# CederGroupHub/chgnet

Hardware: NVIDIA H100
Metric: structures_per_sec_EFS (higher is better)
Workload: dtype f32

## Files before the change

chgnet_b200/_lib.py:

```python
from __future__ import annotations

import ctypes
import os
from ctypes import c_char_p, c_float, c_int32, c_int64, c_void_p

import torch
from torch import Tensor

_HERE = os.path.dirname(os.path.abspath(__file__))
LIB_PATH = os.path.join(_HERE, "libchgnet_b200.so")

P, I, F, I64 = c_void_p, c_int32, c_float, c_int64

SIGNATURES: dict[str, list] = {
    "chg_embed_atoms": [P, P, I, P, P],
    "chg_edge_geometry": [P, P, P, P, P, P, I, P, P, P, P],
    "chg_bond_basis_embed": [P, P, I, P, P, I, F, F, I, P, P, P, P, P, P],
    "chg_bond_basis_bwd": [P, P, I, P, P, I, F, F, I, P, P, P, P, P, P, P],
    "chg_angle_basis_embed": [P, P, P, I, P, I, P, P, P, P],
    "chg_angle_basis_bwd": [P, P, P, I, P, I, P, P, P, P, P],
    "chg_linear": [P, P, I, I, P, P, P, P, I, P, P],
    "chg_gather_rows": [P, P, I, I, P, P],
    "chg_scatter_rows": [P, P, I, I, P, P],
    "chg_atom_conv_fwd": [P, P, P, P, P, P, I, P, P, P, P, P, P, P],
    "chg_atom_conv_bwd": [P, P, P, P, P, P, I, P, P, P, P, P, P, P, P, P],
    "chg_segment_sum": [P, I, P, P, I, I, I, P, I, P],
    "chg_atom_conv_fused": [P, P, P, P, P, P, P, I, I, P, P, P, P, P, P, P],
    "chg_bond_conv_fused": [P, P, P, P, P, P, P, P, I, I, P, P, P, P, P, P, P, P],
    "chg_bond_conv_fwd": [P, P, P, P, P, P, P, I, P, P, P, P, P, P, P],
    "chg_bond_conv_bwd": [P, P, P, P, P, I, P, P, P, P, P, P, P, P, P],
    "chg_angle_update_fwd": [P, P, P, P, P, P, P, I, P, P, P, P],
    "chg_angle_update_bwd": [P, P, I, P, P, P, P],
    "chg_readout": [P, P, P, I, P, P, P, P, I, P, F, P, P, P, P, P, P, P],
    "chg_magmom": [P, I, P, F, P, P],
    "chg_force_virial": [P, P, P, P, P, P, P, P, P, P, I, P, P, P],
    "chg_wgrad": [P, P, I, P, I, P, I, P, I, I, P, I, P, P, P],
    "chg_colsum": [P, I, P, I, P, I, I, P, P],
    "chg_readout_bwd": [P, I, P, P, P, P, I, P, P, P, P, P, P, P, P],
    "chg_magmom_bwd": [P, I, P, F, P, P, P, P],
    "chg_loss_terms": [P, P, I, I, F, P, P, P],
    "chg_adam_step": [P, P, P, P, I64, F, F, F, F, F, I, P],
    "chg_edge_tangent": [P, P, P, P, P, P, P, P, I, P, P, P],
    "chg_bond_basis_tangent": [P, P, P, I, P, P, I, F, F, I, P, P, P, P, P, P],
    "chg_bond_basis_bwd2": [P, P, P, I, P, P, I, F, F, I, P, P, P, P, P, P],
    "chg_angle_basis_tangent": [P, P, P, P, I, P, I, P, P, P, P],
    "chg_angle_basis_bwd2": [P, P, P, P, I, P, I, P, P, P, P],
    "chg_atom_conv_tan": [P, P, P, P, P, P, P, I, P, P, P, P, P, P, P, P],
    "chg_atom_conv_bwd2": [P, P, P, P, P, P, P, P, P, I, P, P, P, P, P, P, P, P, P],
    "chg_bond_conv_tan": [P, P, P, P, P, P, P, P, I, P, P, P, P, P, P, P, P],
    "chg_bond_conv_bwd2": [P, P, P, P, P, P, P, P, P, I, P, P, P, P, P, P, P, P, P, P],
    "chg_angle_update_tan": [P, P, P, P, P, P, P, I, P, P, P, P, P],
    "chg_angle_update_bwd2": [P, P, P, P, I, P, P, P, P],
    "chg_readout_bwd2": [P, P, I, P, P, P, P, I, P, P, P, P, P, P, P, P, P, P, P, P],
    "chg_bond_basis_hvp": [P, P, P, I, P, P, I, F, F, I, P, P, P, P, P, P],
    "chg_angle_basis_hvp": [P, P, P, P, I, P, I, P, P, P, P],
    "chg_edge_tangent_bwd": [P, P, P, P, P, P, P, P, P, P, I, P, P],
    "chg_edge_tangent_bwd_virial": [P, P, P, P, P, P, P, P, P, P, P, P, I, P, P, P],
    "chg_dynamical_matrices": [P, P, P, P, P, I, I, P, I, P, P],
}

_lib = None


class ChgnetB200Error(RuntimeError):
    pass


def load_library(path: str | None = None) -> ctypes.CDLL:
    global _lib
    if _lib is not None and path is None:
        return _lib
    path = path or LIB_PATH
    if not os.path.exists(path):
        raise ChgnetB200Error(
            f"{path} not found: build it with `python -c 'import __graft_entry__ as g; g.build()'` "
            "(or `make -C chgnet_b200/csrc`). chgnet_b200 has no CPU or PyTorch fallback."
        )
    lib = ctypes.CDLL(path)
    lib.chg_last_error.restype = c_char_p
    lib.chg_last_error.argtypes = []
    lib.chg_abi_version.restype = c_int32
    lib.chg_abi_version.argtypes = []
    lib.chg_launch_count.restype = c_int64
    lib.chg_launch_count.argtypes = []
    lib.chg_set_option.restype = c_int32
    lib.chg_set_option.argtypes = [c_char_p, c_int32]
    lib.chg_wgrad_workspace_floats.restype = c_int64
    lib.chg_wgrad_workspace_floats.argtypes = [c_int32]
    lib.chg_gated_fused_workspace_floats.restype = c_int64
    lib.chg_gated_fused_workspace_floats.argtypes = [c_int32]
    for name, argtypes in SIGNATURES.items():
        fn = getattr(lib, name)
        fn.restype = c_int32
        fn.argtypes = argtypes
    _lib = lib
    return lib


def _p(t: Tensor | None):
    if t is None:
        return None
    return t.data_ptr()


class CudaKernels:

    name = "cuda"

    def __init__(self, device: torch.device | str | int | None = None) -> None:
        self.lib = load_library()
        if not torch.cuda.is_available():
            raise ChgnetB200Error("chgnet_b200 needs a CUDA device (H100 / sm_90a); none is visible")
        dev = torch.device("cuda", torch.cuda.current_device()) if device is None else torch.device(device)
        if dev.type != "cuda":
            raise ChgnetB200Error(f"chgnet_b200 kernels run on CUDA devices only (got {dev})")
        self.device_index = torch.cuda.current_device() if dev.index is None else dev.index

    def _stream(self):
        return torch.cuda.current_stream(self.device_index).cuda_stream

    def _call(self, name: str, *args) -> None:
        if torch.cuda.current_device() != self.device_index:
            with torch.cuda.device(self.device_index):
                return self._call(name, *args)
        rc = getattr(self.lib, name)(*args, self._stream())
        if rc != 0:
            raise ChgnetB200Error(f"{name} failed ({rc}): {self.lib.chg_last_error().decode()}")

    @staticmethod
    def _chk(*tensors: Tensor | None) -> None:
        for t in tensors:
            if t is not None and (not t.is_cuda or not t.is_contiguous()):
                raise ChgnetB200Error("kernel arguments must be contiguous CUDA tensors")

    def set_option(self, name: str, value: int) -> None:
        if self.lib.chg_set_option(name.encode(), int(value)) != 0:
            raise ChgnetB200Error(self.lib.chg_last_error().decode())

    @property
    def launches(self) -> int:
        return int(self.lib.chg_launch_count())

    def embed_atoms(self, z, emb, x):
        self._chk(z, emb, x)
        self._call("chg_embed_atoms", _p(z), _p(emb), z.shape[0], _p(x))

    def edge_geometry(self, frac, lattice, owner, center, nbr, image, rvec, dist, rhat):
        self._chk(frac, lattice, owner, center, nbr, image, rvec, dist, rhat)
        self._call("chg_edge_geometry", _p(frac), _p(lattice), _p(owner), _p(center), _p(nbr), _p(image),
                   center.shape[0], _p(rvec), _p(dist), _p(rhat))

    def bond_basis_embed(self, dist, u2d, freq_ag, freq_bg, rc_ag, rc_bg, p, w3t, e0, wag, wbg, basis_out=None):
        self._chk(dist, u2d, freq_ag, freq_bg, w3t, e0, wag, wbg, basis_out)
        self._call("chg_bond_basis_embed", _p(dist), _p(u2d), u2d.shape[0], _p(freq_ag), _p(freq_bg),
                   freq_ag.shape[0], float(rc_ag), float(rc_bg), int(p), _p(w3t), _p(e0), _p(wag), _p(wbg),
                   _p(basis_out))

    def bond_basis_bwd(self, dist, u2d, freq_ag, freq_bg, rc_ag, rc_bg, p, w3, g_e0, g_wag, g_wbg, g_dist,
                       g_freq=None):
        self._chk(dist, u2d, freq_ag, freq_bg, w3, g_e0, g_wag, g_wbg, g_dist, g_freq)
        self._call("chg_bond_basis_bwd", _p(dist), _p(u2d), u2d.shape[0], _p(freq_ag), _p(freq_bg),
                   freq_ag.shape[0], float(rc_ag), float(rc_bg), int(p), _p(w3), _p(g_e0), _p(g_wag), _p(g_wbg),
                   _p(g_dist), _p(g_freq))

    def angle_basis_embed(self, rhat, ang_di, ang_dj, freq, wt, a0, basis_out=None):
        self._chk(rhat, ang_di, ang_dj, freq, wt, a0, basis_out)
        self._call("chg_angle_basis_embed", _p(rhat), _p(ang_di), _p(ang_dj), ang_di.shape[0], _p(freq),
                   freq.shape[0], _p(wt), _p(a0), _p(basis_out))

    def angle_basis_bwd(self, rhat, ang_di, ang_dj, freq, w, g_a0, g_rhat, g_freq=None):
        self._chk(rhat, ang_di, ang_dj, freq, w, g_a0, g_rhat, g_freq)
        self._call("chg_angle_basis_bwd", _p(rhat), _p(ang_di), _p(ang_dj), ang_di.shape[0], _p(freq),
                   freq.shape[0], _p(w), _p(g_a0), _p(g_rhat), _p(g_freq))

    def linear(self, x, wt, bias, residual, y, x_rows=None, y_rows=None):
        self._chk(x, wt, bias, residual, y, x_rows, y_rows)
        m = x_rows.shape[0] if x_rows is not None else x.shape[0]
        self._call("chg_linear", _p(x), _p(x_rows), m, x.shape[1], _p(wt), _p(bias), _p(residual), _p(y_rows),
                   wt.shape[1], _p(y))

    def gather_rows(self, src, idx, dst):
        self._chk(src, idx, dst)
        self._call("chg_gather_rows", _p(src), _p(idx), idx.shape[0], src.shape[1], _p(dst))

    def scatter_rows(self, src, idx, dst):
        self._chk(src, idx, dst)
        self._call("chg_scatter_rows", _p(src), _p(idx), idx.shape[0], src.shape[1], _p(dst))

    def atom_conv_fwd(self, pcn, pe, wag, center, nbr, d2u, w2t, b2, ln, msg, save_p, save_pre=None):
        self._chk(pcn, pe, wag, center, nbr, d2u, w2t, b2, ln, msg, save_p, save_pre)
        self._call("chg_atom_conv_fwd", _p(pcn), _p(pe), _p(wag), _p(center), _p(nbr), _p(d2u), center.shape[0],
                   _p(w2t), _p(b2), _p(ln), _p(msg), _p(save_p), _p(save_pre))

    def atom_conv_bwd(self, pcn, pe, wag, center, nbr, d2u, save_p, g_agg, w2, ln, g_pre, g_w, g_p=None, g_ln=None):
        self._chk(pcn, pe, wag, center, nbr, d2u, save_p, g_agg, w2, ln, g_pre, g_w, g_p, g_ln)
        self._call("chg_atom_conv_bwd", _p(pcn), _p(pe), _p(wag), _p(center), _p(nbr), _p(d2u), center.shape[0],
                   _p(save_p), _p(g_agg), _p(w2), _p(ln), _p(g_pre), _p(g_w), _p(g_p), _p(g_ln))

    def _fused_work(self, n_rows: int, device) -> Tensor:
        need = int(self.lib.chg_gated_fused_workspace_floats(int(n_rows)))
        ws = getattr(self, "_fws", None)
        if ws is None or ws.device != device or ws.numel() < need:
            ws = torch.empty(need, dtype=torch.float32, device=device)
            self._fws = ws
        return ws

    def atom_conv_fused(self, pcn, pe, wag, center, nbr, d2u, ptr_c, w2t, b2, ln, agg, save_p):
        self._chk(pcn, pe, wag, center, nbr, d2u, ptr_c, w2t, b2, ln, agg, save_p)
        self._call("chg_atom_conv_fused", _p(pcn), _p(pe), _p(wag), _p(center), _p(nbr), _p(d2u), _p(ptr_c), center.shape[0],
                   agg.shape[0], _p(w2t), _p(b2), _p(ln), _p(agg), _p(save_p), _p(self._fused_work(center.shape[0], agg.device)))

    def bond_conv_fused(self, pij, px, pa, wbg, ang_atom, ang_i, ang_j, ptr_i, w2t, b2, ln, agg, save_pre, save_p):
        self._chk(pij, px, pa, wbg, ang_atom, ang_i, ang_j, ptr_i, w2t, b2, ln, agg, save_pre, save_p)
        self._call("chg_bond_conv_fused", _p(pij), _p(px), _p(pa), _p(wbg), _p(ang_atom), _p(ang_i), _p(ang_j), _p(ptr_i),
                   ang_i.shape[0], agg.shape[0], _p(w2t), _p(b2), _p(ln), _p(agg), _p(save_pre), _p(save_p),
                   _p(self._fused_work(ang_i.shape[0], agg.device)))

    def segment_sum(self, data, perm, ptr, accumulate, out):
        self._chk(data, perm, ptr)
        if not out.is_cuda or out.stride(1) != 1:
            raise ChgnetB200Error("segment_sum output must be a CUDA tensor with unit column stride")
        n_items = data.shape[0] if perm is None else perm.shape[0]
        self._call("chg_segment_sum", _p(data), data.shape[1], _p(perm), _p(ptr), ptr.shape[0] - 1, n_items,
                   int(accumulate), _p(out), out.stride(0))

    def bond_conv_fwd(self, pij, px, pa, wbg, ang_atom, ang_i, ang_j, w2t, b2, ln, upd, save_pre, save_p):
        self._chk(pij, px, pa, wbg, ang_atom, ang_i, ang_j, w2t, b2, ln, upd, save_pre, save_p)
        self._call("chg_bond_conv_fwd", _p(pij), _p(px), _p(pa), _p(wbg), _p(ang_atom), _p(ang_i), _p(ang_j),
                   ang_i.shape[0], _p(w2t), _p(b2), _p(ln), _p(upd), _p(save_pre), _p(save_p))

    def bond_conv_bwd(self, save_pre, save_p, wbg, ang_i, ang_j, g_agg, w2, ln, g_pre, gw_i, gw_j, g_p=None,
                      g_ln=None):
        self._chk(save_pre, save_p, wbg, ang_i, ang_j, g_agg, w2, ln, g_pre, gw_i, gw_j, g_p, g_ln)
        self._call("chg_bond_conv_bwd", _p(save_pre), _p(save_p), _p(wbg), _p(ang_i), _p(ang_j), ang_i.shape[0],
                   _p(g_agg), _p(w2), _p(ln), _p(g_pre), _p(gw_i), _p(gw_j), _p(g_p), _p(g_ln))

    def angle_update_fwd(self, pij, px, pa, ang, ang_atom, ang_i, ang_j, ln, ang_new, save_p):
        self._chk(pij, px, pa, ang, ang_atom, ang_i, ang_j, ln, ang_new, save_p)
        self._call("chg_angle_update_fwd", _p(pij), _p(px), _p(pa), _p(ang), _p(ang_atom), _p(ang_i), _p(ang_j),
                   ang_i.shape[0], _p(ln), _p(ang_new), _p(save_p))

    def angle_update_bwd(self, save_p, g_ang_in, ln, g_pre, g_ln=None):
        self._chk(save_p, g_ang_in, ln, g_pre, g_ln)
        self._call("chg_angle_update_bwd", _p(save_p), _p(g_ang_in), save_p.shape[0], _p(ln), _p(g_pre), _p(g_ln))

    @staticmethod
    def _chk_rows(*tensors: Tensor | None) -> None:
        for t in tensors:
            if t is not None and (not t.is_cuda or t.stride(-1) != 1):
                raise ChgnetB200Error("kernel arguments must be CUDA tensors with unit column stride")

    def _workspace(self, n_out: int, device) -> Tensor:
        ws = getattr(self, "_ws", None)
        if ws is None or ws.device != device:
            need = max(int(self.lib.chg_wgrad_workspace_floats(n)) for n in (64, 128, 256))
            ws = torch.empty(need, dtype=torch.float32, device=device)
            self._ws = ws
        return ws

    def wgrad(self, x, g, out, colsum=None, x_rows=None, g_rows=None, x_silu=False, x2=None):
        self._chk_rows(x, g, out, x2)
        self._chk(colsum, x_rows, g_rows)
        if x2 is not None and x2.stride(0) != x.stride(0):
            raise ChgnetB200Error("wgrad: x2 must have the row stride of x")
        m = x_rows.shape[0] if x_rows is not None else (g_rows.shape[0] if g_rows is not None else x.shape[0])
        self._call("chg_wgrad", _p(x), _p(x2), x.stride(0), _p(x_rows), int(bool(x_silu)), _p(g), g.stride(0), _p(g_rows), m,
                   out.shape[1], _p(out), out.stride(0), _p(colsum), _p(self._workspace(out.shape[1], x.device)))

    def colsum(self, a, out, b=None, rowscale=None):
        self._chk_rows(a, b)
        self._chk(out, rowscale)
        self._call("chg_colsum", _p(a), a.stride(0), _p(b), b.stride(0) if b is not None else 0, _p(rowscale),
                   a.shape[0], a.shape[1], _p(out))

    def readout_bwd(self, x, ln, mlp_wt, mlp_w, mlp_b, w_last, seed, g_x, h_all, gz_all, g_h0, xhat):
        self._chk(x, ln, mlp_wt, mlp_w, mlp_b, w_last, seed, g_x, h_all, gz_all, g_h0, xhat)
        self._call("chg_readout_bwd", _p(x), x.shape[0], _p(ln), _p(mlp_wt), _p(mlp_w), _p(mlp_b), mlp_wt.shape[0],
                   _p(w_last), _p(seed), _p(g_x), _p(h_all), _p(gz_all), _p(g_h0), _p(xhat))

    def magmom_bwd(self, x, w, b, g_m, g_x, g_lin):
        self._chk(x, w, g_m, g_x, g_lin)
        self._call("chg_magmom_bwd", _p(x), x.shape[0], _p(w), float(b), _p(g_m), _p(g_x), _p(g_lin))

    def loss_terms(self, pred, target, kind, delta, g_pred, sums):
        self._chk(pred, target, g_pred, sums)
        self._call("chg_loss_terms", _p(pred), _p(target), pred.numel(), int(kind), float(delta), _p(g_pred), _p(sums))

    def edge_tangent(self, rvec, dist, rhat, center, nbr, owner, u_atom, w_graph, ddist, drhat):
        self._chk(rvec, dist, rhat, center, nbr, owner, u_atom, w_graph, ddist, drhat)
        self._call("chg_edge_tangent", _p(rvec), _p(dist), _p(rhat), _p(center), _p(nbr), _p(owner), _p(u_atom),
                   _p(w_graph), center.shape[0], _p(ddist), _p(drhat))

    def bond_basis_tangent(self, dist, ddist, u2d, freq_ag, freq_bg, rc_ag, rc_bg, p, w3t, e0d, wagd, wbgd, tbasis):
        self._chk(dist, ddist, u2d, freq_ag, freq_bg, w3t, e0d, wagd, wbgd, tbasis)
        self._call("chg_bond_basis_tangent", _p(dist), _p(ddist), _p(u2d), u2d.shape[0], _p(freq_ag), _p(freq_bg),
                   freq_ag.shape[0], float(rc_ag), float(rc_bg), int(p), _p(w3t), _p(e0d), _p(wagd), _p(wbgd), _p(tbasis))

    def bond_basis_bwd2(self, dist, ddist, u2d, freq_ag, freq_bg, rc_ag, rc_bg, p, w3, lam_e0, lam_wag, lam_wbg, g_freq):
        self._chk(dist, ddist, u2d, freq_ag, freq_bg, w3, lam_e0, lam_wag, lam_wbg, g_freq)
        self._call("chg_bond_basis_bwd2", _p(dist), _p(ddist), _p(u2d), u2d.shape[0], _p(freq_ag), _p(freq_bg),
                   freq_ag.shape[0], float(rc_ag), float(rc_bg), int(p), _p(w3), _p(lam_e0), _p(lam_wag), _p(lam_wbg),
                   _p(g_freq))

    def angle_basis_tangent(self, rhat, drhat, ang_di, ang_dj, freq, wt, a0d, tbasis):
        self._chk(rhat, drhat, ang_di, ang_dj, freq, wt, a0d, tbasis)
        self._call("chg_angle_basis_tangent", _p(rhat), _p(drhat), _p(ang_di), _p(ang_dj), ang_di.shape[0], _p(freq),
                   freq.shape[0], _p(wt), _p(a0d), _p(tbasis))

    def angle_basis_bwd2(self, rhat, drhat, ang_di, ang_dj, freq, w, lam_a0, g_freq):
        self._chk(rhat, drhat, ang_di, ang_dj, freq, w, lam_a0, g_freq)
        self._call("chg_angle_basis_bwd2", _p(rhat), _p(drhat), _p(ang_di), _p(ang_dj), ang_di.shape[0], _p(freq),
                   freq.shape[0], _p(w), _p(lam_a0), _p(g_freq))

    def bond_basis_hvp(self, dist, ddist, u2d, freq_ag, freq_bg, rc_ag, rc_bg, p, w3, lam_e0, lam_wag, lam_wbg, g_dist):
        self._chk(dist, ddist, u2d, freq_ag, freq_bg, w3, lam_e0, lam_wag, lam_wbg, g_dist)
        self._call("chg_bond_basis_hvp", _p(dist), _p(ddist), _p(u2d), u2d.shape[0], _p(freq_ag), _p(freq_bg),
                   freq_ag.shape[0], float(rc_ag), float(rc_bg), int(p), _p(w3), _p(lam_e0), _p(lam_wag), _p(lam_wbg),
                   _p(g_dist))

    def angle_basis_hvp(self, rhat, drhat, ang_di, ang_dj, freq, w, lam_a0, g_rhat):
        self._chk(rhat, drhat, ang_di, ang_dj, freq, w, lam_a0, g_rhat)
        self._call("chg_angle_basis_hvp", _p(rhat), _p(drhat), _p(ang_di), _p(ang_dj), ang_di.shape[0], _p(freq),
                   freq.shape[0], _p(w), _p(lam_a0), _p(g_rhat))

    def edge_tangent_bwd(self, dist, rhat, ddist, drhat, lam_dist, lam_rhat, d2u, u2d, center, nbr, force):
        self._chk(dist, rhat, ddist, drhat, lam_dist, lam_rhat, d2u, u2d, center, nbr, force)
        self._call("chg_edge_tangent_bwd", _p(dist), _p(rhat), _p(ddist), _p(drhat), _p(lam_dist), _p(lam_rhat), _p(d2u),
                   _p(u2d), _p(center), _p(nbr), center.shape[0], _p(force))

    def edge_tangent_bwd_virial(self, rvec, dist, rhat, ddist, drhat, lam_dist, lam_rhat, d2u, u2d, center, nbr, owner,
                                force, virial):
        self._chk(rvec, dist, rhat, ddist, drhat, lam_dist, lam_rhat, d2u, u2d, center, nbr, owner, force, virial)
        self._call("chg_edge_tangent_bwd_virial", _p(rvec), _p(dist), _p(rhat), _p(ddist), _p(drhat), _p(lam_dist),
                   _p(lam_rhat), _p(d2u), _p(u2d), _p(center), _p(nbr), _p(owner), center.shape[0], _p(force), _p(virial))

    def dynamical_matrices(self, fc, img_ptr, img_vec, s2p, inv_sqrt_m, qpoints, dyn):
        self._chk(fc, img_ptr, img_vec, s2p, inv_sqrt_m, qpoints, dyn)
        if dyn.dtype != torch.complex128 or fc.dtype != torch.float64 or qpoints.dtype != torch.float64:
            raise ChgnetB200Error("dynamical_matrices: fc and qpoints must be float64, dyn complex128")
        self._call("chg_dynamical_matrices", _p(fc), _p(img_ptr), _p(img_vec), _p(s2p), _p(inv_sqrt_m), fc.shape[0],
                   fc.shape[1], _p(qpoints), qpoints.shape[0], _p(dyn))

    def atom_conv_tan(self, pcn_d, pe_d, wag, wag_d, center, nbr, d2u, save_pre, save_p, w2t, ln, msg_d, pre_d, p_d):
        self._chk(pcn_d, pe_d, wag, wag_d, center, nbr, d2u, save_pre, save_p, w2t, ln, msg_d, pre_d, p_d)
        self._call("chg_atom_conv_tan", _p(pcn_d), _p(pe_d), _p(wag), _p(wag_d), _p(center), _p(nbr), _p(d2u),
                   center.shape[0], _p(save_pre), _p(save_p), _p(w2t), _p(ln), _p(msg_d), _p(pre_d), _p(p_d))

    def atom_conv_bwd2(self, save_pre, save_p, pre_d, p_d, g_p_lam, wag, wag_d, center, d2u, lam_agg, bar_agg, w2, ln,
                       bar_pre, bar_w, u_out, g_ln):
        self._chk(save_pre, save_p, pre_d, p_d, g_p_lam, wag, wag_d, center, d2u, lam_agg, bar_agg, w2, ln, bar_pre,
                  bar_w, u_out, g_ln)
        self._call("chg_atom_conv_bwd2", _p(save_pre), _p(save_p), _p(pre_d), _p(p_d), _p(g_p_lam), _p(wag), _p(wag_d),
                   _p(center), _p(d2u), center.shape[0], _p(lam_agg), _p(bar_agg), _p(w2), _p(ln), _p(bar_pre), _p(bar_w),
                   _p(u_out), _p(g_ln))

    def bond_conv_tan(self, pij_d, px_d, pa_d, wbg, wbg_d, ang_atom, ang_i, ang_j, save_pre, save_p, w2t, ln, upd_d,
                      pre_d, p_d):
        self._chk(pij_d, px_d, pa_d, wbg, wbg_d, ang_atom, ang_i, ang_j, save_pre, save_p, w2t, ln, upd_d, pre_d, p_d)
        self._call("chg_bond_conv_tan", _p(pij_d), _p(px_d), _p(pa_d), _p(wbg), _p(wbg_d), _p(ang_atom), _p(ang_i),
                   _p(ang_j), ang_i.shape[0], _p(save_pre), _p(save_p), _p(w2t), _p(ln), _p(upd_d), _p(pre_d), _p(p_d))

    def bond_conv_bwd2(self, save_pre, save_p, pre_d, p_d, g_p_lam, wbg, wbg_d, ang_i, ang_j, lam_agg, bar_agg, w2, ln,
                       bar_pre, bar_wi, bar_wj, u_out, g_ln):
        self._chk(save_pre, save_p, pre_d, p_d, g_p_lam, wbg, wbg_d, ang_i, ang_j, lam_agg, bar_agg, w2, ln, bar_pre,
                  bar_wi, bar_wj, u_out, g_ln)
        self._call("chg_bond_conv_bwd2", _p(save_pre), _p(save_p), _p(pre_d), _p(p_d), _p(g_p_lam), _p(wbg), _p(wbg_d),
                   _p(ang_i), _p(ang_j), ang_i.shape[0], _p(lam_agg), _p(bar_agg), _p(w2), _p(ln), _p(bar_pre),
                   _p(bar_wi), _p(bar_wj), _p(u_out), _p(g_ln))

    def angle_update_tan(self, pij_d, px_d, pa_d, ang_d, ang_atom, ang_i, ang_j, save_p, ln, ang_new_d, p_d):
        self._chk(pij_d, px_d, pa_d, ang_d, ang_atom, ang_i, ang_j, save_p, ln, ang_new_d, p_d)
        self._call("chg_angle_update_tan", _p(pij_d), _p(px_d), _p(pa_d), _p(ang_d), _p(ang_atom), _p(ang_i), _p(ang_j),
                   ang_i.shape[0], _p(save_p), _p(ln), _p(ang_new_d), _p(p_d))

    def angle_update_bwd2(self, save_p, p_d, lam_ang, bar_ang, ln, bar_pre, g_ln):
        self._chk(save_p, p_d, lam_ang, bar_ang, ln, bar_pre, g_ln)
        self._call("chg_angle_update_bwd2", _p(save_p), _p(p_d), _p(lam_ang), _p(bar_ang), save_p.shape[0], _p(ln),
                   _p(bar_pre), _p(g_ln))

    def readout_bwd2(self, x, xd, ln, mlp_wt, mlp_w, mlp_b, w_last, seed, bar_x, h_all, hd_all, gz_all, zbar_all,
                     g_h0, hbar0, xhat, xhatd):
        self._chk(x, xd, ln, mlp_wt, mlp_w, mlp_b, w_last, seed, bar_x, h_all, hd_all, gz_all, zbar_all, g_h0, hbar0,
                  xhat, xhatd)
        self._call("chg_readout_bwd2", _p(x), _p(xd), x.shape[0], _p(ln), _p(mlp_wt), _p(mlp_w), _p(mlp_b),
                   mlp_wt.shape[0], _p(w_last), _p(seed), _p(bar_x), _p(h_all), _p(hd_all), _p(gz_all), _p(zbar_all),
                   _p(g_h0), _p(hbar0), _p(xhat), _p(xhatd))

    def adam_step(self, p, g, m, v, lr, beta1, beta2, eps, weight_decay, step):
        self._chk(p, g, m, v)
        self._call("chg_adam_step", _p(p), _p(g), _p(m), _p(v), p.numel(), float(lr), float(beta1), float(beta2),
                   float(eps), float(weight_decay), int(step))

    def readout(self, x, z, owner, ln, mlp_wt, mlp_w, mlp_b, w_last, b_last, atom_ref, site_e, h_out, e_graph,
                e_ref, g_x):
        self._chk(x, z, owner, ln, mlp_wt, mlp_w, mlp_b, w_last, atom_ref, site_e, h_out, e_graph, e_ref, g_x)
        self._call("chg_readout", _p(x), _p(z), _p(owner), x.shape[0], _p(ln), _p(mlp_wt), _p(mlp_w), _p(mlp_b),
                   mlp_wt.shape[0], _p(w_last), float(b_last), _p(atom_ref), _p(site_e), _p(h_out), _p(e_graph),
                   _p(e_ref), _p(g_x))

# ... 9 lines not shown
```

chgnet_b200/csrc/gated.cu:

```cuda
#include <cstdlib>

#include "gated_common.cuh"

namespace chg {
namespace {

using namespace gated;

template <int MODE>
struct FwdSmem {
  static constexpr bool HAS_W2 = MODE != ANGLE;
  static constexpr int W2_OFF = 0;
  static constexpr int TILE_OFF = W2_OFF + (HAS_W2 ? 64 * 128 : 0);
  static constexpr int TILE_FLOATS = HAS_W2 ? TM * HS : 0;
  static constexpr int B2_OFF = TILE_OFF + TILE_FLOATS;
  static constexpr int LN_OFF = B2_OFF + 128;
  static constexpr int IDX_OFF = LN_OFF + 256;
  static constexpr int TOTAL_BYTES = (IDX_OFF + 3 * TM) * 4;
};

template <int MODE>
__global__ void __launch_bounds__(NTHR, 2) gated_fwd_kernel(const FwdArgs a) {
  using L = FwdSmem<MODE>;
  extern __shared__ __align__(16) float smem[];
  float* s_w2t = smem + L::W2_OFF;
  float* s_tile = smem + L::TILE_OFF;
  float* s_b2 = smem + L::B2_OFF;
  float* s_ln = smem + L::LN_OFF;
  int* s_idx = reinterpret_cast<int*>(smem + L::IDX_OFF);

  const int tid = threadIdx.x;
  const int tx = tid & 15, ty = tid >> 4;
  const int r0 = ty * 4, c0 = tx * 4;
  const bool use_ln = a.ln != nullptr;

  if (L::HAS_W2) {
    copy_to_smem(s_w2t, a.w2t, 64 * 128, tid);
    if (tid < 128) s_b2[tid] = a.b2[tid];
  }
  if (use_ln) s_ln[tid] = a.ln[tid];

  const int n_tiles = (a.n_rows + TM - 1) / TM;
  for (int tile = blockIdx.x; tile < n_tiles; tile += gridDim.x) {
    const int base = tile * TM;
    __syncthreads();
    if (tid < TM) {
      const int r = min(base + tid, a.n_rows - 1);
      s_idx[tid] = a.idx0[r];
      s_idx[TM + tid] = a.idx1[r];
      s_idx[2 * TM + tid] = a.idx2[r];
    }
    __syncthreads();

    float acc[4][8];
#pragma unroll
    for (int i = 0; i < 4; ++i)
#pragma unroll
      for (int j = 0; j < 8; ++j) acc[i][j] = 0.f;
    gather_pre<TM>(acc, a.p_a, a.p_b, a.p_c, s_idx, base, a.n_rows, r0, c0);

    if (L::HAS_W2) {
      if (a.save_pre != nullptr) {
#pragma unroll
        for (int i = 0; i < 4; ++i) {
          const int g = base + r0 + i;
          if (g < a.n_rows) {
            stg4(a.save_pre + (size_t)g * 128 + c0, make_float4(acc[i][0], acc[i][1], acc[i][2], acc[i][3]));
            stg4(a.save_pre + (size_t)g * 128 + 64 + c0, make_float4(acc[i][4], acc[i][5], acc[i][6], acc[i][7]));
          }
        }
      }
#pragma unroll
      for (int i = 0; i < 4; ++i) {
        sts4(s_tile + (r0 + i) * HS + c0,
             make_float4(silu_f(acc[i][0]), silu_f(acc[i][1]), silu_f(acc[i][2]), silu_f(acc[i][3])));
        sts4(s_tile + (r0 + i) * HS + 64 + c0,
             make_float4(silu_f(acc[i][4]), silu_f(acc[i][5]), silu_f(acc[i][6]), silu_f(acc[i][7])));
      }
      __syncthreads();
      const float4 bc = lds4(s_b2 + c0), bg = lds4(s_b2 + 64 + c0);
#pragma unroll
      for (int i = 0; i < 4; ++i) {
        acc[i][0] = bc.x; acc[i][1] = bc.y; acc[i][2] = bc.z; acc[i][3] = bc.w;
        acc[i][4] = bg.x; acc[i][5] = bg.y; acc[i][6] = bg.z; acc[i][7] = bg.w;
      }
      gemm_blockdiag(acc, s_tile, s_w2t, s_w2t + 64, 128, r0, c0);
    }

    float4 g1, b1, g2, b2v;
    if (use_ln) {
      g1 = lds4(s_ln + c0);
      b1 = lds4(s_ln + 64 + c0);
      g2 = lds4(s_ln + 128 + c0);
      b2v = lds4(s_ln + 192 + c0);
    }
#pragma unroll
    for (int i = 0; i < 4; ++i) {
      const int row = r0 + i;
      const int g = base + row;
      const bool valid = g < a.n_rows;
      if (a.save_p != nullptr && valid) {
        stg4(a.save_p + (size_t)g * 128 + c0, make_float4(acc[i][0], acc[i][1], acc[i][2], acc[i][3]));
        stg4(a.save_p + (size_t)g * 128 + 64 + c0, make_float4(acc[i][4], acc[i][5], acc[i][6], acc[i][7]));
      }
      float y1[4] = {acc[i][0], acc[i][1], acc[i][2], acc[i][3]};
      float y2[4] = {acc[i][4], acc[i][5], acc[i][6], acc[i][7]};
      if (use_ln) {
        float xh[4], rstd;
        ln_stats(y1, xh, rstd);
#pragma unroll
        for (int j = 0; j < 4; ++j) y1[j] = fmaf(xh[j], f4at(g1, j), f4at(b1, j));
        ln_stats(y2, xh, rstd);
#pragma unroll
        for (int j = 0; j < 4; ++j) y2[j] = fmaf(xh[j], f4at(g2, j), f4at(b2v, j));
      }
      float4 o;
#pragma unroll
      for (int j = 0; j < 4; ++j) f4at(o, j) = silu_f(y1[j]) * sigmoid_f(y2[j]);
      if (MODE == ATOM) {
        o = o * ldg4(a.wgt + (size_t)s_idx[2 * TM + row] * 64 + c0);
      } else if (MODE == BOND) {
        o = o * ldg4(a.wgt + (size_t)s_idx[row] * 64 + c0) * ldg4(a.wgt + (size_t)s_idx[TM + row] * 64 + c0);
      } else {
        o = o + ldg4(a.feat + (size_t)min(g, a.n_rows - 1) * 64 + c0);
      }
      if (valid) stg4(a.out + (size_t)g * 64 + c0, o);
    }
  }
}

template <int MODE>
struct BwdSmem {
  static constexpr bool HAS_W2 = MODE != ANGLE;
  static constexpr int W2_OFF = 0;
  static constexpr int TILE_OFF = W2_OFF + (HAS_W2 ? 128 * 64 : 0);
  static constexpr int LN_OFF = TILE_OFF + (HAS_W2 ? TM * HS : 0);
  static constexpr int IDX_OFF = LN_OFF + 256;
  static constexpr int TOTAL_BYTES = (IDX_OFF + 3 * TM) * 4;
};

template <int MODE, bool TRAIN>
__global__ void __launch_bounds__(NTHR, 2) gated_bwd_kernel(const BwdArgs a) {
  using L = BwdSmem<MODE>;
  extern __shared__ __align__(16) float smem[];
  float* s_w2 = smem + L::W2_OFF;
  float* s_g = smem + L::TILE_OFF;
  float* s_ln = smem + L::LN_OFF;
  int* s_idx = reinterpret_cast<int*>(smem + L::IDX_OFF);

  const int tid = threadIdx.x;
  const int tx = tid & 15, ty = tid >> 4;
  const int r0 = ty * 4, c0 = tx * 4;
  const bool use_ln = a.ln != nullptr;

  if (L::HAS_W2) copy_to_smem(s_w2, a.w2, 128 * 64, tid);
  if (use_ln) s_ln[tid] = a.ln[tid];
  float ln_acc[16];
#pragma unroll
  for (int j = 0; j < 16; ++j) ln_acc[j] = 0.f;

  const int n_tiles = (a.n_rows + TM - 1) / TM;
  for (int tile = blockIdx.x; tile < n_tiles; tile += gridDim.x) {
    const int base = tile * TM;
    __syncthreads();
    if (MODE != ANGLE && tid < TM) {
      const int r = min(base + tid, a.n_rows - 1);
      s_idx[tid] = a.idx0[r];
      s_idx[TM + tid] = a.idx1[r];
      if (MODE == ATOM) s_idx[2 * TM + tid] = a.idx2[r];
    }
    __syncthreads();

    float4 g1, g2, b1, b2v;
    if (use_ln) {
      g1 = lds4(s_ln + c0);
      b1 = lds4(s_ln + 64 + c0);
      g2 = lds4(s_ln + 128 + c0);
      b2v = lds4(s_ln + 192 + c0);
    }
#pragma unroll
    for (int i = 0; i < 4; ++i) {
      const int row = r0 + i;
      const int g = base + row;
      const bool valid = g < a.n_rows;
      const int r = min(g, a.n_rows - 1);
      const float4 pc4 = ldg4(a.save_p + (size_t)r * 128 + c0);
      const float4 pg4 = ldg4(a.save_p + (size_t)r * 128 + 64 + c0);
      float y1[4] = {pc4.x, pc4.y, pc4.z, pc4.w};
      float y2[4] = {pg4.x, pg4.y, pg4.z, pg4.w};
      float xh1[4], xh2[4], rstd1 = 1.f, rstd2 = 1.f;
      if (use_ln) {
        ln_stats(y1, xh1, rstd1);
        ln_stats(y2, xh2, rstd2);
#pragma unroll
        for (int j = 0; j < 4; ++j) {
          y1[j] = fmaf(xh1[j], f4at(g1, j), f4at(b1, j));
          y2[j] = fmaf(xh2[j], f4at(g2, j), f4at(b2v, j));
        }
      }
      float s1[4], core[4], gate[4];
      float4 o;
#pragma unroll
      for (int j = 0; j < 4; ++j) {
        s1[j] = sigmoid_f(y1[j]);
        core[j] = y1[j] * s1[j];
        gate[j] = sigmoid_f(y2[j]);
        f4at(o, j) = core[j] * gate[j];
      }
      float4 go;
      if (MODE == ATOM) {
        const float4 gm = ldg4(a.g_in + (size_t)s_idx[row] * 64 + c0);
        const float4 w = ldg4(a.wgt + (size_t)s_idx[2 * TM + row] * 64 + c0);
        if (valid) stg4(a.g_w0 + (size_t)g * 64 + c0, gm * o);
        go = gm * w;
      } else if (MODE == BOND) {
        const float4 gm = ldg4(a.g_in + (size_t)s_idx[row] * 64 + c0);
        const float4 wi = ldg4(a.wgt + (size_t)s_idx[row] * 64 + c0);
        const float4 wj = ldg4(a.wgt + (size_t)s_idx[TM + row] * 64 + c0);
        const float4 gmo = gm * o;
        if (valid) {
          stg4(a.g_w0 + (size_t)g * 64 + c0, gmo * wj);
          stg4(a.g_w1 + (size_t)g * 64 + c0, gmo * wi);
        }
        go = gm * wi * wj;
      } else {
        go = a.g_in != nullptr ? ldg4(a.g_in + (size_t)r * 64 + c0) : make_float4(0.f, 0.f, 0.f, 0.f);
      }
      float gy1[4], gy2[4];
#pragma unroll
      for (int j = 0; j < 4; ++j) {
        const float gj = f4at(go, j);
        gy1[j] = gj * gate[j] * (s1[j] * fmaf(y1[j], 1.f - s1[j], 1.f));
        gy2[j] = gj * core[j] * gate[j] * (1.f - gate[j]);
      }
      if (use_ln) {
        if (TRAIN && valid) {
#pragma unroll
          for (int j = 0; j < 4; ++j) {
            ln_acc[j] = fmaf(gy1[j], xh1[j], ln_acc[j]);
            ln_acc[4 + j] += gy1[j];
            ln_acc[8 + j] = fmaf(gy2[j], xh2[j], ln_acc[8 + j]);
            ln_acc[12 + j] += gy2[j];
          }
        }
        float gx[4], sa = 0.f, sb = 0.f;
#pragma unroll
        for (int j = 0; j < 4; ++j) {
          gx[j] = gy1[j] * f4at(g1, j);
          sa += gx[j];
          sb = fmaf(gx[j], xh1[j], sb);
        }
        sa = sum16(sa) * (1.f / 64.f);
        sb = sum16(sb) * (1.f / 64.f);
#pragma unroll
        for (int j = 0; j < 4; ++j) gy1[j] = rstd1 * (gx[j] - sa - xh1[j] * sb);
        sa = 0.f, sb = 0.f;
#pragma unroll
        for (int j = 0; j < 4; ++j) {
          gx[j] = gy2[j] * f4at(g2, j);
          sa += gx[j];
          sb = fmaf(gx[j], xh2[j], sb);
        }
        sa = sum16(sa) * (1.f / 64.f);
        sb = sum16(sb) * (1.f / 64.f);
#pragma unroll
        for (int j = 0; j < 4; ++j) gy2[j] = rstd2 * (gx[j] - sa - xh2[j] * sb);
      }
      const float4 gpc = make_float4(gy1[0], gy1[1], gy1[2], gy1[3]);
      const float4 gpg = make_float4(gy2[0], gy2[1], gy2[2], gy2[3]);
      if (TRAIN && L::HAS_W2 && valid && a.g_p != nullptr) {
        stg4(a.g_p + (size_t)g * 128 + c0, gpc);
        stg4(a.g_p + (size_t)g * 128 + 64 + c0, gpg);
      }
      if (L::HAS_W2) {
        sts4(s_g + row * HS + c0, gpc);
        sts4(s_g + row * HS + 64 + c0, gpg);
      } else if (valid) {
        stg4(a.g_pre + (size_t)g * 128 + c0, gpc);
        stg4(a.g_pre + (size_t)g * 128 + 64 + c0, gpg);
      }
    }

    if (L::HAS_W2) {
      __syncthreads();
      float acc[4][8];
#pragma unroll
      for (int i = 0; i < 4; ++i)
#pragma unroll
        for (int j = 0; j < 8; ++j) acc[i][j] = 0.f;
      gemm_blockdiag(acc, s_g, s_w2, s_w2 + 64 * 64, 64, r0, c0);
      float pre[4][8];
      if (MODE == ATOM) {
#pragma unroll
        for (int i = 0; i < 4; ++i)
#pragma unroll
          for (int j = 0; j < 8; ++j) pre[i][j] = 0.f;
        gather_pre<TM>(pre, a.p_a, a.p_b, nullptr, s_idx, base, a.n_rows, r0, c0);
      } else {
#pragma unroll
        for (int i = 0; i < 4; ++i) {
          const int r = min(base + r0 + i, a.n_rows - 1);
          const float4 vc = ldg4(a.save_pre + (size_t)r * 128 + c0);
          const float4 vg = ldg4(a.save_pre + (size_t)r * 128 + 64 + c0);
          pre[i][0] = vc.x; pre[i][1] = vc.y; pre[i][2] = vc.z; pre[i][3] = vc.w;
          pre[i][4] = vg.x; pre[i][5] = vg.y; pre[i][6] = vg.z; pre[i][7] = vg.w;
        }
      }
#pragma unroll
      for (int i = 0; i < 4; ++i) {
        const int g = base + r0 + i;
#pragma unroll
        for (int j = 0; j < 8; ++j) acc[i][j] *= dsilu_f(pre[i][j]);
        if (g < a.n_rows) {
          stg4(a.g_pre + (size_t)g * 128 + c0, make_float4(acc[i][0], acc[i][1], acc[i][2], acc[i][3]));
          stg4(a.g_pre + (size_t)g * 128 + 64 + c0, make_float4(acc[i][4], acc[i][5], acc[i][6], acc[i][7]));
        }
      }
    }
  }
  if (TRAIN && use_ln && a.g_ln != nullptr) {
    __syncthreads();
    float* s_red = smem;
#pragma unroll
    for (int which = 0; which < 4; ++which)
#pragma unroll
      for (int j = 0; j < 4; ++j) s_red[ty * 256 + which * 64 + c0 + j] = ln_acc[which * 4 + j];
    __syncthreads();
    float tot = 0.f;
#pragma unroll
    for (int r = 0; r < 16; ++r) tot += s_red[r * 256 + tid];
    atomicAdd(a.g_ln + tid, (double)tot);
  }
}

constexpr int TM2 = 128;

struct Smem2 {
  static constexpr int W_OFF = 0;
  static constexpr int TILE_OFF = W_OFF + 64 * 128;
  static constexpr int B2_OFF = TILE_OFF + TM2 * HS;
  static constexpr int LN_OFF = B2_OFF + 128;
  static constexpr int IDX_OFF = LN_OFF + 256;
  static constexpr int TOTAL_BYTES = (IDX_OFF + 3 * TM2) * 4;
};

__device__ __forceinline__ void gemm_half_8x8(float (&acc)[8][8], const float* __restrict__ sT,
                                              const float* __restrict__ sB, int ldb, int row0, int cg) {
#pragma unroll
  for (int i = 0; i < 8; ++i)
#pragma unroll
    for (int j = 0; j < 8; ++j) acc[i][j] = 0.f;
#pragma unroll 2
  for (int k2 = 0; k2 < 32; ++k2) {
    float2 a[8];
#pragma unroll
    for (int i = 0; i < 8; ++i) a[i] = *reinterpret_cast<const float2*>(sT + (row0 + i) * HS + k2 * 2);
#pragma unroll
    for (int kk = 0; kk < 2; ++kk) {
      const float4 b0 = lds4(sB + (k2 * 2 + kk) * ldb + cg * 4);
      const float4 b1 = lds4(sB + (k2 * 2 + kk) * ldb + 32 + cg * 4);
#pragma unroll
      for (int i = 0; i < 8; ++i) {
        const float v = kk == 0 ? a[i].x : a[i].y;
        acc[i][0] = fmaf(v, b0.x, acc[i][0]);
        acc[i][1] = fmaf(v, b0.y, acc[i][1]);
        acc[i][2] = fmaf(v, b0.z, acc[i][2]);
        acc[i][3] = fmaf(v, b0.w, acc[i][3]);
        acc[i][4] = fmaf(v, b1.x, acc[i][4]);
        acc[i][5] = fmaf(v, b1.y, acc[i][5]);
        acc[i][6] = fmaf(v, b1.z, acc[i][6]);
        acc[i][7] = fmaf(v, b1.w, acc[i][7]);
      }
    }
  }
}

template <bool FWD>
__device__ __forceinline__ void tile_gemm_inplace(float* s_tile, const float* s_w, int tid) {
  const int half = tid >> 7, u = tid & 127;
  const int cg = u & 7, row0 = (u >> 3) * 8;
  const float* sB = FWD ? s_w + half * 64 : s_w + half * 64 * 64;
  float acc[8][8];
  gemm_half_8x8(acc, s_tile + half * 64, sB, FWD ? 128 : 64, row0, cg);
  __syncthreads();
#pragma unroll
  for (int i = 0; i < 8; ++i) {
    float* dst = s_tile + (row0 + i) * HS + half * 64 + cg * 4;
    sts4(dst, make_float4(acc[i][0], acc[i][1], acc[i][2], acc[i][3]));
    sts4(dst + 32, make_float4(acc[i][4], acc[i][5], acc[i][6], acc[i][7]));
  }
  __syncthreads();
}

template <int MODE>
__global__ void __launch_bounds__(NTHR, 2) gated2_fwd_kernel(const FwdArgs a) {
  extern __shared__ __align__(16) float smem[];
  float* s_w = smem + Smem2::W_OFF;
  float* s_tile = smem + Smem2::TILE_OFF;
  float* s_b2 = smem + Smem2::B2_OFF;
  float* s_ln = smem + Smem2::LN_OFF;
  int* s_idx = reinterpret_cast<int*>(smem + Smem2::IDX_OFF);

  const int tid = threadIdx.x;
  const int tx = tid & 15, ty = tid >> 4;
  const int c0 = tx * 4;
  const bool use_ln = a.ln != nullptr;
  copy_to_smem(s_w, a.w2t, 64 * 128, tid);
  if (tid < 128) s_b2[tid] = a.b2[tid];
  if (use_ln) s_ln[tid] = a.ln[tid];

  const int n_tiles = (a.n_rows + TM2 - 1) / TM2;
  for (int tile = blockIdx.x; tile < n_tiles; tile += gridDim.x) {
    const int base = tile * TM2;
    __syncthreads();
    if (tid < TM2) {
      const int r = min(base + tid, a.n_rows - 1);
      s_idx[tid] = a.idx0[r];
      s_idx[TM2 + tid] = a.idx1[r];
      s_idx[2 * TM2 + tid] = a.idx2[r];
    }
    __syncthreads();

#pragma unroll 1
    for (int it = 0; it < 2; ++it) {
      const int r0 = it * 64 + ty * 4;
      float acc[4][8];
#pragma unroll
      for (int i = 0; i < 4; ++i)
#pragma unroll
        for (int j = 0; j < 8; ++j) acc[i][j] = 0.f;
      gather_pre<TM2>(acc, a.p_a, a.p_b, a.p_c, s_idx, base, a.n_rows, r0, c0);
#pragma unroll
      for (int i = 0; i < 4; ++i) {
        const int g = base + r0 + i;
// ... 209 lines not shown
                           hc.w * dsilu_f(pre[i][3])));
          stg4(a.g_pre + (size_t)g * 128 + 64 + c0,
               make_float4(hg.x * dsilu_f(pre[i][4]), hg.y * dsilu_f(pre[i][5]), hg.z * dsilu_f(pre[i][6]),
                           hg.w * dsilu_f(pre[i][7])));
        }
      }
    }
  }
}

template <int MODE>
int launch_fwd(const FwdArgs& a, cudaStream_t stream) {
  if (a.n_rows == 0) return CHG_OK;
  constexpr int smem = FwdSmem<MODE>::TOTAL_BYTES;
  static int slots = 0;
  if (slots == 0) {
    CHG_CUDA(cudaFuncSetAttribute(gated_fwd_kernel<MODE>, cudaFuncAttributeMaxDynamicSharedMemorySize, smem));
    slots = resident_ctas(gated_fwd_kernel<MODE>, smem);
  }
  const int n_tiles = (a.n_rows + TM - 1) / TM;
  gated_fwd_kernel<MODE><<<min(n_tiles, slots), NTHR, smem, stream>>>(a);
  CHG_LAUNCH_END();
}

template <int MODE, bool TRAIN>
int launch_bwd_t(const BwdArgs& a, cudaStream_t stream) {
  if (a.n_rows == 0) return CHG_OK;
  constexpr int smem = TRAIN ? (BwdSmem<MODE>::TOTAL_BYTES > 16 * 256 * 4 ? BwdSmem<MODE>::TOTAL_BYTES : 16 * 256 * 4)
                             : BwdSmem<MODE>::TOTAL_BYTES;
  static int slots = 0;
  if (slots == 0) {
    CHG_CUDA(cudaFuncSetAttribute(gated_bwd_kernel<MODE, TRAIN>, cudaFuncAttributeMaxDynamicSharedMemorySize, smem));
    slots = resident_ctas(gated_bwd_kernel<MODE, TRAIN>, smem);
  }
  const int n_tiles = (a.n_rows + TM - 1) / TM;
  gated_bwd_kernel<MODE, TRAIN><<<min(n_tiles, slots), NTHR, smem, stream>>>(a);
  CHG_LAUNCH_END();
}

template <int MODE>
int launch_bwd(const BwdArgs& a, cudaStream_t stream) {
  if (a.g_p != nullptr || a.g_ln != nullptr) return launch_bwd_t<MODE, true>(a, stream);
  return launch_bwd_t<MODE, false>(a, stream);
}

template <typename KernelT, typename ArgsT>
int launch2(KernelT kernel, const ArgsT& a, int& slots, cudaStream_t stream) {
  if (a.n_rows == 0) return CHG_OK;
  if (slots == 0) {
    CHG_CUDA(cudaFuncSetAttribute(kernel, cudaFuncAttributeMaxDynamicSharedMemorySize, Smem2::TOTAL_BYTES));
    slots = resident_ctas(kernel, Smem2::TOTAL_BYTES);
  }
  const int n_tiles = (a.n_rows + TM2 - 1) / TM2;
  kernel<<<min(n_tiles, slots), NTHR, Smem2::TOTAL_BYTES, stream>>>(a);
  CHG_LAUNCH_END();
}

}
}

using namespace chg;
using namespace chg::gated;

extern "C" int chg_atom_conv_fwd(const float* pcn, const float* pe, const float* wag, const int32_t* center,
                                 const int32_t* nbr, const int32_t* d2u, int32_t n_edges, const float* w2t,
                                 const float* b2, const float* ln, float* msg, float* save_p, float* save_pre,
                                 void* stream) {
  CHG_CHECK_ARG(n_edges >= 0, "negative size");
  if (n_edges == 0) return CHG_OK;
  CHG_CHECK_ARG(pcn && pe && wag && center && nbr && d2u && w2t && b2 && msg, "null pointer");
  FwdArgs a{pcn, pe, nullptr, nullptr, wag, center, nbr, d2u, n_edges, w2t, b2, ln, msg, save_pre, save_p};
  const bool train = save_pre != nullptr;
  if (gated_impl() == 1 && !train) return atom_conv_fwd_tc(a, as_stream(stream));
  if (gated_impl() == 2 && !train) {
    static int slots = 0;
    return launch2(gated2_fwd_kernel<ATOM>, a, slots, as_stream(stream));
  }
  return launch_fwd<ATOM>(a, as_stream(stream));
}

extern "C" int chg_atom_conv_bwd(const float* pcn, const float* pe, const float* wag, const int32_t* center,
                                 const int32_t* nbr, const int32_t* d2u, int32_t n_edges, const float* save_p,
                                 const float* g_agg, const float* w2, const float* ln, float* g_pre, float* g_w,
                                 float* g_p, double* g_ln, void* stream) {
  CHG_CHECK_ARG(n_edges >= 0, "negative size");
  if (n_edges == 0) return CHG_OK;
  CHG_CHECK_ARG(pcn && pe && wag && center && nbr && d2u && save_p && g_agg && w2 && g_pre && g_w, "null pointer");
  BwdArgs a{pcn, pe, wag, center, nbr, d2u, n_edges, nullptr, save_p, g_agg, w2, ln, g_pre, g_w, nullptr, g_p, g_ln};
  const bool train = g_p != nullptr || g_ln != nullptr;
  if (gated_impl() == 3 && !train && n_edges >= ws_min_rows()) return atom_conv_bwd_ws(a, as_stream(stream));
  if (gated_impl() == 1 && !train) return atom_conv_bwd_tc(a, as_stream(stream));
  if (gated_impl() == 2 && !train) {
    static int slots = 0;
    return launch2(gated2_bwd_kernel<ATOM>, a, slots, as_stream(stream));
  }
  return launch_bwd<ATOM>(a, as_stream(stream));
}

extern "C" int chg_bond_conv_fwd(const float* pij, const float* px, const float* pa, const float* wbg,
                                 const int32_t* ang_atom, const int32_t* ang_i, const int32_t* ang_j,
                                 int32_t n_angles, const float* w2t, const float* b2, const float* ln, float* upd,
                                 float* save_pre, float* save_p, void* stream) {
  CHG_CHECK_ARG(n_angles >= 0, "negative size");
  if (n_angles == 0) return CHG_OK;
  CHG_CHECK_ARG(pij && px && pa && wbg && ang_atom && ang_i && ang_j && w2t && b2 && upd, "null pointer");
  FwdArgs a{pij, px, pa, nullptr, wbg, ang_i, ang_j, ang_atom, n_angles, w2t, b2, ln, upd, save_pre, save_p};
  if (gated_impl() == 1) return bond_conv_fwd_tc(a, as_stream(stream));
  if (gated_impl() == 2) {
    static int slots = 0;
    return launch2(gated2_fwd_kernel<BOND>, a, slots, as_stream(stream));
  }
  return launch_fwd<BOND>(a, as_stream(stream));
}

extern "C" int chg_bond_conv_bwd(const float* save_pre, const float* save_p, const float* wbg, const int32_t* ang_i,
                                 const int32_t* ang_j, int32_t n_angles, const float* g_agg, const float* w2,
                                 const float* ln, float* g_pre, float* gw_i, float* gw_j, float* g_p, double* g_ln,
                                 void* stream) {
  CHG_CHECK_ARG(n_angles >= 0, "negative size");
  if (n_angles == 0) return CHG_OK;
  CHG_CHECK_ARG(save_pre && save_p && wbg && ang_i && ang_j && g_agg && w2 && g_pre && gw_i && gw_j, "null pointer");
  BwdArgs a{nullptr, nullptr, wbg, ang_i, ang_j, nullptr, n_angles, save_pre, save_p, g_agg, w2, ln,
            g_pre, gw_i, gw_j, g_p, g_ln};
  const bool train = g_p != nullptr || g_ln != nullptr;
  if (gated_impl() == 3 && !train && n_angles >= ws_min_rows()) return bond_conv_bwd_ws(a, as_stream(stream));
  if (gated_impl() == 1 && !train) return bond_conv_bwd_tc(a, as_stream(stream));
  if (gated_impl() == 2 && !train) {
    static int slots = 0;
    return launch2(gated2_bwd_kernel<BOND>, a, slots, as_stream(stream));
  }
  return launch_bwd<BOND>(a, as_stream(stream));
}

extern "C" int chg_angle_update_fwd(const float* pij, const float* px, const float* pa, const float* ang,
                                    const int32_t* ang_atom, const int32_t* ang_i, const int32_t* ang_j,
                                    int32_t n_angles, const float* ln, float* ang_new, float* save_p, void* stream) {
  CHG_CHECK_ARG(n_angles >= 0, "negative size");
  if (n_angles == 0) return CHG_OK;
  CHG_CHECK_ARG(pij && px && pa && ang && ang_atom && ang_i && ang_j && ang_new, "null pointer");
  FwdArgs a{pij, px, pa, ang, nullptr, ang_i, ang_j, ang_atom, n_angles, nullptr, nullptr, ln, ang_new,
            nullptr, save_p};
  return launch_fwd<ANGLE>(a, as_stream(stream));
}

extern "C" int chg_angle_update_bwd(const float* save_p, const float* g_ang_in, int32_t n_angles, const float* ln,
                                    float* g_pre, double* g_ln, void* stream) {
  CHG_CHECK_ARG(n_angles >= 0, "negative size");
  if (n_angles == 0) return CHG_OK;
  CHG_CHECK_ARG(save_p && g_pre, "null pointer");
  BwdArgs a{nullptr, nullptr, nullptr, nullptr, nullptr, nullptr, n_angles, nullptr, save_p, g_ang_in,
            nullptr, ln, g_pre, nullptr, nullptr, nullptr, g_ln};
  return launch_bwd<ANGLE>(a, as_stream(stream));
}
```

chgnet_b200/csrc/gated_common.cuh:

```cuda
#pragma once
#include "common.cuh"

namespace chg {
namespace gated {

constexpr int HS = 132;
constexpr float LN_EPS = 1e-5f;
}
int ws_min_rows();
namespace gated {

enum Mode { ATOM = 0, BOND = 1, ANGLE = 2 };

struct FwdArgs {
  const float* p_a;
  const float* p_b;
  const float* p_c;
  const float* feat;
  const float* wgt;
  const int32_t* idx0;
  const int32_t* idx1;
  const int32_t* idx2;
  int32_t n_rows;
  const float* w2t;
  const float* b2;
  const float* ln;
  float* out;
  float* save_pre;
  float* save_p;
};

struct BwdArgs {
  const float* p_a;
  const float* p_b;
  const float* wgt;
  const int32_t* idx0;
  const int32_t* idx1;
  const int32_t* idx2;
  int32_t n_rows;
  const float* save_pre;
  const float* save_p;
  const float* g_in;
  const float* w2;
  const float* ln;
  float* g_pre;
  float* g_w0;
  float* g_w1;
  float* g_p;
  double* g_ln;
};

__device__ __forceinline__ void ln_stats(const float (&v)[4], float (&xhat)[4], float& rstd) {
  const float mean = sum16(v[0] + v[1] + v[2] + v[3]) * (1.f / 64.f);
  float d[4], ss = 0.f;
#pragma unroll
  for (int j = 0; j < 4; ++j) {
    d[j] = v[j] - mean;
    ss = fmaf(d[j], d[j], ss);
  }
  const float var = sum16(ss) * (1.f / 64.f);
  rstd = 1.f / sqrtf(var + LN_EPS);
#pragma unroll
  for (int j = 0; j < 4; ++j) xhat[j] = d[j] * rstd;
}

template <int TMV>
__device__ __forceinline__ void gather_pre(float (&acc)[4][8], const float* __restrict__ p_a,
                                           const float* __restrict__ p_b, const float* __restrict__ p_c,
                                           const int* s_idx, int base, int n_rows, int r0, int c0) {
#pragma unroll
  for (int i = 0; i < 4; ++i) {
    const int row = r0 + i;
    const float* s0 = p_a + (size_t)s_idx[row] * 256 + c0;
    const float* s1 = p_a + (size_t)s_idx[TMV + row] * 256 + 128 + c0;
    const float* s2 = p_b + (size_t)s_idx[2 * TMV + row] * 128 + c0;
    float4 vc = ldg4(s0) + ldg4(s1) + ldg4(s2);
    float4 vg = ldg4(s0 + 64) + ldg4(s1 + 64) + ldg4(s2 + 64);
    if (p_c != nullptr) {
      const float* s3 = p_c + (size_t)min(base + row, n_rows - 1) * 128 + c0;
      vc = vc + ldg4(s3);
      vg = vg + ldg4(s3 + 64);
    }
    acc[i][0] += vc.x; acc[i][1] += vc.y; acc[i][2] += vc.z; acc[i][3] += vc.w;
    acc[i][4] += vg.x; acc[i][5] += vg.y; acc[i][6] += vg.z; acc[i][7] += vg.w;
  }
}


#ifdef __CUDACC__
constexpr int TM = 64;
constexpr int NTHR = 256;

__device__ __forceinline__ void copy_to_smem(float* dst, const float* src, int n_floats, int tid) {
  for (int i = tid * 4; i < n_floats; i += NTHR * 4) sts4(dst + i, ldg4(src + i));
}

__device__ __forceinline__ void gemm_blockdiag(float (&acc)[4][8], const float* __restrict__ sT,
                                               const float* __restrict__ sBc, const float* __restrict__ sBg,
                                               int ldb, int r0, int c0) {
#pragma unroll 2
  for (int k4 = 0; k4 < 16; ++k4) {
    float4 hc[4], hg[4];
#pragma unroll
    for (int i = 0; i < 4; ++i) {
      hc[i] = lds4(sT + (r0 + i) * HS + k4 * 4);
      hg[i] = lds4(sT + (r0 + i) * HS + 64 + k4 * 4);
    }
#pragma unroll
    for (int kk = 0; kk < 4; ++kk) {
      const float4 wc = lds4(sBc + (k4 * 4 + kk) * ldb + c0);
      const float4 wg = lds4(sBg + (k4 * 4 + kk) * ldb + c0);
#pragma unroll
      for (int i = 0; i < 4; ++i) {
        const float a = f4at(hc[i], kk);
        const float g = f4at(hg[i], kk);
        acc[i][0] = fmaf(a, wc.x, acc[i][0]);
        acc[i][1] = fmaf(a, wc.y, acc[i][1]);
        acc[i][2] = fmaf(a, wc.z, acc[i][2]);
        acc[i][3] = fmaf(a, wc.w, acc[i][3]);
        acc[i][4] = fmaf(g, wg.x, acc[i][4]);
        acc[i][5] = fmaf(g, wg.y, acc[i][5]);
        acc[i][6] = fmaf(g, wg.z, acc[i][6]);
        acc[i][7] = fmaf(g, wg.w, acc[i][7]);
      }
    }
  }
}


template <typename KernelT>
inline int resident_ctas(KernelT kernel, int smem_bytes) {
  int per_sm = 0;
  if (cudaOccupancyMaxActiveBlocksPerMultiprocessor(&per_sm, kernel, NTHR, smem_bytes) != cudaSuccess || per_sm < 1)
    per_sm = 1;
  return per_sm * sm_count();
}

#endif

int atom_conv_fwd_tc(const FwdArgs& a, cudaStream_t stream);
int bond_conv_fwd_tc(const FwdArgs& a, cudaStream_t stream);
int atom_conv_bwd_tc(const BwdArgs& a, cudaStream_t stream);
int bond_conv_bwd_tc(const BwdArgs& a, cudaStream_t stream);

int atom_conv_bwd_ws(const BwdArgs& a, cudaStream_t stream);
int bond_conv_bwd_ws(const BwdArgs& a, cudaStream_t stream);

int atom_conv_fused_ws(const float* pcn, const float* pe, const float* wag, const int32_t* center, const int32_t* nbr,
                       const int32_t* d2u, const int32_t* ptr_c, int n_edges, int n_atoms, const float* w2t, const float* b2,
                       const float* ln, float* agg, float* save_p, float* parts, cudaStream_t stream);
int bond_conv_fused_ws(const float* pij, const float* px, const float* pa, const float* wbg, const int32_t* ang_atom,
                       const int32_t* ang_i, const int32_t* ang_j, const int32_t* ptr_i, int n_angles, int n_slots,
                       const float* w2t, const float* b2, const float* ln, float* agg, float* save_pre, float* save_p,
                       float* parts, cudaStream_t stream);

}
}
```

chgnet_b200/csrc/gated_ws.cu:

```cuda
#include "gated_common.cuh"
#include "tc.cuh"

namespace chg {
namespace gated {
namespace {

constexpr int WS_THREADS = 512;
constexpr int TR = 128;
constexpr int HALF_BYTES = TR * 64 * 4;
constexpr int IMG_BYTES = 64 * 64 * 4;
constexpr int STRIP = 16;

struct WsSmem {
  static constexpr int IMG_OFF = 0;
  static constexpr int HS_OFF = 4 * IMG_BYTES;
  static constexpr int O_OFF = HS_OFF + 2 * HALF_BYTES;
  static constexpr int GIDX_OFF = O_OFF + HALF_BYTES;
  static constexpr int EIDX_OFF = GIDX_OFF + 2 * 3 * TR * 4;
  static constexpr int B2_OFF = EIDX_OFF + 4 * TR * 4;
  static constexpr int LN_OFF = B2_OFF + 128 * 4;
  static constexpr int TOTAL = LN_OFF + 256 * 4;
};

struct WsBars {
  uint64_t a_full[2], a_empty[2];
};

struct FusedArgs {
  const float* p_a;
  const float* p_b;
  const float* p_c;
  const float* wgt;
  const int32_t* idx0;
  const int32_t* idx1;
  const int32_t* idx2;
  const int32_t* ptr;
  int32_t n_rows, n_seg;
  const float* w2t;
  const float* b2;
  const float* ln;
  float* out;
  float* parts;
  float* save_pre;
  float* save_p;
};

__device__ __forceinline__ void prefetch_l2(const void* p) { asm volatile("prefetch.global.L2 [%0];" ::"l"(p)); }
__device__ __forceinline__ int swz(int r, int c) { return r * 256 + ((c ^ (r & 7)) << 4); }

__device__ __forceinline__ void build_image_ws(uint8_t* hi, uint8_t* lo, const float* __restrict__ src, int ld, int col0,
                                               int tid) {
  for (int i = tid; i < 4096; i += (int)blockDim.x) {
    const int kk = i >> 6, n = i & 63;
    uint32_t h, l;
    tc::split_tf32(__ldg(src + (size_t)kk * ld + col0 + n), h, l);
    const uint32_t off = tc::kmajor_offset(n, kk, 64);
    *reinterpret_cast<uint32_t*>(hi + off) = h;
    *reinterpret_cast<uint32_t*>(lo + off) = l;
  }
}

__device__ __forceinline__ float quad_sum(float v) {
  v += __shfl_xor_sync(0xffffffffu, v, 1);
  v += __shfl_xor_sync(0xffffffffu, v, 2);
  return v;
}
__device__ __forceinline__ void bias_ln_frag(float (&d)[32], const float* s_b2, const float* s_gamma, const float* s_beta,
                                             bool use_ln, float* save_rows, int row0, int n_rows) {
#pragma unroll
  for (int i = 0; i < 32; ++i) d[i] += s_b2[tc::frag_col(i)];
  if (save_rows != nullptr) {
#pragma unroll
    for (int i = 0; i < 32; i += 2) {
      const int g = row0 + tc::frag_row(i);
      if (g < n_rows) *reinterpret_cast<float2*>(save_rows + (size_t)g * 128 + tc::frag_col(i)) = make_float2(d[i], d[i + 1]);
    }
  }
  if (!use_ln) return;
#pragma unroll
  for (int h = 0; h < 2; ++h) {
    float s1 = 0.f;
#pragma unroll
    for (int i = 0; i < 32; ++i)
      if (((i >> 1) & 1) == h) s1 += d[i];
    const float mean = quad_sum(s1) * (1.f / 64.f);
    float s2 = 0.f;
#pragma unroll
    for (int i = 0; i < 32; ++i)
      if (((i >> 1) & 1) == h) s2 = fmaf(d[i] - mean, d[i] - mean, s2);
    const float rstd = 1.f / sqrtf(quad_sum(s2) * (1.f / 64.f) + LN_EPS);
#pragma unroll
    for (int i = 0; i < 32; ++i)
      if (((i >> 1) & 1) == h) d[i] = fmaf((d[i] - mean) * rstd, s_gamma[tc::frag_col(i)], s_beta[tc::frag_col(i)]);
  }
}

template <int MODE>
__global__ void __launch_bounds__(WS_THREADS, 1) gated_ws_fwd_kernel(const FusedArgs a) {
  extern __shared__ __align__(1024) uint8_t smem_raw[];
  uint8_t* s_img = smem_raw + WsSmem::IMG_OFF;
  uint8_t* s_hs = smem_raw + WsSmem::HS_OFF;
  uint8_t* s_o = smem_raw + WsSmem::O_OFF;
  int* s_gidx = reinterpret_cast<int*>(smem_raw + WsSmem::GIDX_OFF);
  int* s_eidx = reinterpret_cast<int*>(smem_raw + WsSmem::EIDX_OFF);
  float* s_b2 = reinterpret_cast<float*>(smem_raw + WsSmem::B2_OFF);
  float* s_ln = reinterpret_cast<float*>(smem_raw + WsSmem::LN_OFF);
  __shared__ __align__(8) WsBars bars;

  const int tid = threadIdx.x, warp = tid >> 5, lane = tid & 31;
  const bool use_ln = a.ln != nullptr;
  const int n_tiles = (a.n_rows + TR - 1) / TR;

  build_image_ws(s_img, s_img + IMG_BYTES, a.w2t, 128, 0, tid);
  build_image_ws(s_img + 2 * IMG_BYTES, s_img + 3 * IMG_BYTES, a.w2t, 128, 64, tid);
  if (tid < 128) s_b2[tid] = a.b2[tid];
  if (tid < 256) s_ln[tid] = use_ln ? a.ln[tid] : 0.f;
  if (tid == 0) {
    for (int i = 0; i < 2; ++i) {
      tc::mbar_init(&bars.a_full[i], 128);
      tc::mbar_init(&bars.a_empty[i], 256);
    }
    tc::mbar_fence_init();
  }
  tc::fence_async_smem();
  __syncthreads();

  if (warp >= 8) {
    const int half = (warp - 8) >> 2;
    const int gt = tid - 256 - half * 128;
    const int tx = gt & 15, ty = gt >> 4;
    int* gi = s_gidx + half * 3 * TR;
    uint8_t* stage = s_hs + half * HALF_BYTES;
    const int col = half * 64 + tx * 4;
    constexpr int PB = 4;
    int tl = 0;
    for (int tile = blockIdx.x; tile < n_tiles; tile += gridDim.x, ++tl) {
      const int base = tile * TR;
      {
        const int r = min(base + gt, a.n_rows - 1);
        gi[gt] = a.idx0[r];
        gi[TR + gt] = a.idx1[r];
        gi[2 * TR + gt] = a.idx2[r];
      }
      tc::wg_barrier(1 + half, 128);
      {
        const int nt = tile + gridDim.x;
        if (nt < n_tiles) {
          const int r = min(nt * TR + gt, a.n_rows - 1);
          const float* row = MODE == BOND ? a.p_c + (size_t)r * 128 + half * 64 : a.p_b + (size_t)__ldg(a.idx2 + r) * 128 + half * 64;
          prefetch_l2(row);
          prefetch_l2(row + 32);
        }
      }
#pragma unroll 1
      for (int b = 0; b < 16 / PB; ++b) {
        float4 v[PB];
#pragma unroll
        for (int i = 0; i < PB; ++i) {
          const int row = ty + 8 * (b * PB + i);
          const float* s0 = a.p_a + (size_t)gi[row] * 256 + col;
          const float* s1 = a.p_a + (size_t)gi[TR + row] * 256 + 128 + col;
          const float* s2 = a.p_b + (size_t)gi[2 * TR + row] * 128 + col;
          v[i] = ldg4(s0) + ldg4(s1) + ldg4(s2);
          if (MODE == BOND) v[i] = v[i] + ldg4(a.p_c + (size_t)min(base + row, a.n_rows - 1) * 128 + col);
        }
        if (b == 0) tc::mbar_wait(&bars.a_empty[half], (tl & 1) ^ 1);
#pragma unroll
        for (int i = 0; i < PB; ++i) {
          const int row = ty + 8 * (b * PB + i);
          if (a.save_pre != nullptr && base + row < a.n_rows) stg4(a.save_pre + (size_t)(base + row) * 128 + col, v[i]);
          *reinterpret_cast<float4*>(stage + swz(row, tx)) =
              make_float4(silu_f(v[i].x), silu_f(v[i].y), silu_f(v[i].z), silu_f(v[i].w));
        }
      }
      tc::wg_barrier(1 + half, 128);
      tc::mbar_arrive(&bars.a_full[half]);
    }
  } else {
    const int cw = warp >> 2;
    const int t = tid & 127;
    const int row0 = cw * 64;
    int* s_seg = s_eidx;
    int* s_wrow = s_eidx + TR;
    int* s_sa = s_eidx + 2 * TR;
    int* s_sb = s_eidx + 3 * TR;
    const uint32_t img = tc::smem_u32(s_img);
    int tl = 0;
    for (int tile = blockIdx.x; tile < n_tiles; tile += gridDim.x, ++tl) {
      const int base = tile * TR;
      {
        const int r = min(base + t, a.n_rows - 1);
        if (cw == 0) {
          const int seg = a.idx0[r];
          s_seg[t] = seg;
          s_sa[t] = __ldg(a.ptr + seg);
          s_sb[t] = __ldg(a.ptr + seg + 1);
        } else {
          const int wr = MODE == BOND ? a.idx1[r] : a.idx2[r];
          s_wrow[t] = wr;
          prefetch_l2(a.wgt + (size_t)wr * 64);
          prefetch_l2(a.wgt + (size_t)wr * 64 + 32);
        }
      }
      float dc[32], dg[32];
#pragma unroll
      for (int i = 0; i < 32; ++i) dc[i] = dg[i] = 0.f;
      tc::mbar_wait(&bars.a_full[0], tl & 1);
      tc::wg_gemm_k64<64>(dc, [&](int r, int k) { return *reinterpret_cast<const float*>(s_hs + swz(row0 + r, k >> 2) + (k & 3) * 4); },
                          img, img + IMG_BYTES, 2048);
      tc::mbar_arrive(&bars.a_empty[0]);
      tc::mbar_wait(&bars.a_full[1], tl & 1);
      tc::wg_gemm_k64<64>(dg, [&](int r, int k) { return *reinterpret_cast<const float*>(s_hs + HALF_BYTES + swz(row0 + r, k >> 2) + (k & 3) * 4); },
                          img + 2 * IMG_BYTES, img + 3 * IMG_BYTES, 2048);
      tc::mbar_arrive(&bars.a_empty[1]);
      float* save = a.save_p != nullptr ? a.save_p + (size_t)base * 128 : nullptr;
      bias_ln_frag(dc, s_b2, s_ln, s_ln + 64, use_ln, save, row0, a.n_rows - base);
      bias_ln_frag(dg, s_b2 + 64, s_ln + 128, s_ln + 192, use_ln, save != nullptr ? save + 64 : nullptr, row0, a.n_rows - base);
#pragma unroll
      for (int i = 0; i < 32; i += 2) {
        const int r = row0 + tc::frag_row(i), c = tc::frag_col(i);
        *reinterpret_cast<float2*>(s_o + swz(r, c >> 2) + (c & 3) * 4) =
            make_float2(silu_f(dc[i]) * sigmoid_f(dg[i]), silu_f(dc[i + 1]) * sigmoid_f(dg[i + 1]));
      }
      tc::wg_barrier(3, 256);

      const int strip_lo = base + warp * STRIP;
      const int strip_hi = min(strip_lo + STRIP, a.n_rows);
      if (strip_lo < a.n_rows) {
        float2 w[STRIP];
#pragma unroll
        for (int i = 0; i < STRIP; ++i) {
          const int rr = warp * STRIP + i;
          const float2 w0 = __ldg(reinterpret_cast<const float2*>(a.wgt + (size_t)s_wrow[rr] * 64) + lane);
          if (MODE == ATOM) {
            w[i] = w0;
          } else {
            const float2 wi = __ldg(reinterpret_cast<const float2*>(a.wgt + (size_t)s_seg[rr] * 64) + lane);
            w[i] = make_float2(wi.x * w0.x, wi.y * w0.y);
          }
        }
        float2 acc = make_float2(0.f, 0.f);
        int cur_row = warp * STRIP;
        auto emit = [&](int row0_, const float2& v) {
          const int seg = s_seg[row0_], sa = s_sa[row0_], sb = s_sb[row0_];
          float* dst;
          if (sa >= strip_lo && sb <= strip_hi) {
            dst = a.out + (size_t)seg * 64;
          } else {
            dst = a.parts + ((size_t)(strip_lo / STRIP) * 2 + (sa < strip_lo ? 0 : 1)) * 64;
          }
          *reinterpret_cast<float2*>(dst + lane * 2) = v;
        };
#pragma unroll
        for (int i = 0; i < STRIP; ++i) {
          const int rr = warp * STRIP + i;
          if (strip_lo + i < strip_hi) {
            if (s_seg[rr] != s_seg[cur_row]) {
              emit(cur_row, acc);
              cur_row = rr;
              acc = make_float2(0.f, 0.f);
            }
            const float2 o = *reinterpret_cast<const float2*>(s_o + swz(rr, lane >> 1) + (lane & 1) * 8);
            acc.x = fmaf(o.x, w[i].x, acc.x);
            acc.y = fmaf(o.y, w[i].y, acc.y);
          }
        }
        emit(cur_row, acc);
      }
      tc::wg_barrier(3, 256);
    }
  }
}

__global__ void seg_stitch_kernel(const int32_t* __restrict__ ptr, int n_seg, const float* __restrict__ parts,
                                  float* __restrict__ out) {
  const int idx = blockIdx.x * blockDim.x + threadIdx.x;
  const int s = idx >> 4, l = idx & 15;
  if (s >= n_seg) return;
  const int a = ptr[s], b = ptr[s + 1];
  if (a >= b) {
    stg4(out + (size_t)s * 64 + l * 4, make_float4(0.f, 0.f, 0.f, 0.f));
    return;
  }
  const int k0 = a / STRIP, k1 = (b - 1) / STRIP;
  if (k0 == k1) return;
  float4 acc = ldg4(parts + ((size_t)k0 * 2 + 1) * 64 + l * 4);
  for (int k = k0 + 1; k <= k1; ++k) acc = acc + ldg4(parts + ((size_t)k * 2) * 64 + l * 4);
  stg4(out + (size_t)s * 64 + l * 4, acc);
}

template <int MODE>
int launch_fused(const FusedArgs& a, cudaStream_t stream) {
  if (a.n_seg == 0) return CHG_OK;
  if (a.n_rows > 0) {
    static bool attr_set = false;
    if (!attr_set) {
      CHG_CUDA(cudaFuncSetAttribute(gated_ws_fwd_kernel<MODE>, cudaFuncAttributeMaxDynamicSharedMemorySize, WsSmem::TOTAL));
      attr_set = true;
    }
    const int n_tiles = (a.n_rows + TR - 1) / TR;
    gated_ws_fwd_kernel<MODE><<<min(n_tiles, sm_count()), WS_THREADS, WsSmem::TOTAL, stream>>>(a);
    cudaError_t e = cudaGetLastError();
    if (e != cudaSuccess) {
      set_error("gated_ws_fwd_kernel: launch failed: %s", cudaGetErrorString(e));
      return CHG_ERR_CUDA;
    }
    count_launch();
  }
  seg_stitch_kernel<<<(a.n_seg * 16 + 255) / 256, 256, 0, stream>>>(a.ptr, a.n_seg, a.parts, a.out);
  CHG_LAUNCH_END();
}

}

int atom_conv_fused_ws(const float* pcn, const float* pe, const float* wag, const int32_t* center, const int32_t* nbr,
                       const int32_t* d2u, const int32_t* ptr_c, int n_edges, int n_atoms, const float* w2t, const float* b2,
                       const float* ln, float* agg, float* save_p, float* parts, cudaStream_t stream) {
  FusedArgs a{pcn, pe, nullptr, wag, center, nbr, d2u, ptr_c, n_edges, n_atoms, w2t, b2, ln, agg, parts, nullptr, save_p};
  return launch_fused<ATOM>(a, stream);
}

int bond_conv_fused_ws(const float* pij, const float* px, const float* pa, const float* wbg, const int32_t* ang_atom,
                       const int32_t* ang_i, const int32_t* ang_j, const int32_t* ptr_i, int n_angles, int n_slots,
                       const float* w2t, const float* b2, const float* ln, float* agg, float* save_pre, float* save_p,
                       float* parts, cudaStream_t stream) {
  FusedArgs a{pij, px, pa, wbg, ang_i, ang_j, ang_atom, ptr_i, n_angles, n_slots, w2t, b2, ln, agg, parts, save_pre, save_p};
  return launch_fused<BOND>(a, stream);
}

}
}

using namespace chg;

extern "C" int64_t chg_gated_fused_workspace_floats(int32_t n_rows) {
  if (n_rows < 0) return -1;
  const int64_t msg = (int64_t)n_rows * 64, parts = ((int64_t)n_rows + 15) / 16 * 128;
  return (msg > parts ? msg : parts) + 64;
}

extern "C" int chg_atom_conv_fused(const float* pcn, const float* pe, const float* wag, const int32_t* center,
                                   const int32_t* nbr, const int32_t* d2u, const int32_t* ptr_c, int32_t n_edges,
                                   int32_t n_atoms, const float* w2t, const float* b2, const float* ln, float* agg,
                                   float* save_p, float* work, void* stream) {
  CHG_CHECK_ARG(n_edges >= 0 && n_atoms >= 0, "negative size");
  if (n_atoms == 0) return CHG_OK;
  CHG_CHECK_ARG(ptr_c && agg, "null pointer");
  CHG_CHECK_ARG(n_edges == 0 || (pcn && pe && wag && center && nbr && d2u && w2t && b2 && work), "null pointer");
  if (gated_impl() == 3 && n_edges >= ws_min_rows())
    return gated::atom_conv_fused_ws(pcn, pe, wag, center, nbr, d2u, ptr_c, n_edges, n_atoms, w2t, b2, ln, agg, save_p, work,
                                     as_stream(stream));
  const int rc = chg_atom_conv_fwd(pcn, pe, wag, center, nbr, d2u, n_edges, w2t, b2, ln, work, save_p, nullptr, stream);
  if (rc != CHG_OK) return rc;
  return chg_segment_sum(work, 64, nullptr, ptr_c, n_atoms, n_edges, 0, agg, 64, stream);
}

extern "C" int chg_bond_conv_fused(const float* pij, const float* px, const float* pa, const float* wbg,
                                   const int32_t* ang_atom, const int32_t* ang_i, const int32_t* ang_j,
                                   const int32_t* ptr_i, int32_t n_angles, int32_t n_slots, const float* w2t,
                                   const float* b2, const float* ln, float* agg, float* save_pre, float* save_p,
                                   float* work, void* stream) {
  CHG_CHECK_ARG(n_angles >= 0 && n_slots >= 0, "negative size");
  if (n_slots == 0) return CHG_OK;
  CHG_CHECK_ARG(ptr_i && agg, "null pointer");
  CHG_CHECK_ARG(n_angles == 0 || (pij && px && pa && wbg && ang_atom && ang_i && ang_j && w2t && b2 && work), "null pointer");
  if (gated_impl() == 3 && n_angles >= ws_min_rows())
    return gated::bond_conv_fused_ws(pij, px, pa, wbg, ang_atom, ang_i, ang_j, ptr_i, n_angles, n_slots, w2t, b2, ln, agg,
                                     save_pre, save_p, work, as_stream(stream));
  const int rc = chg_bond_conv_fwd(pij, px, pa, wbg, ang_atom, ang_i, ang_j, n_angles, w2t, b2, ln, work, save_pre, save_p, stream);
  if (rc != CHG_OK) return rc;
  return chg_segment_sum(work, 64, nullptr, ptr_i, n_slots, n_angles, 0, agg, 64, stream);
}

namespace chg {
namespace gated {
namespace {

struct WsBwdSmem {
  static constexpr int IMG_OFF = 0;
  static constexpr int T1_OFF = 4 * IMG_BYTES;
  static constexpr int T2_OFF = T1_OFF + 2 * HALF_BYTES;
  static constexpr int PIDX_OFF = T2_OFF + 2 * HALF_BYTES;
  static constexpr int FIDX_OFF = PIDX_OFF + 3 * TR * 4;
  static constexpr int LN_OFF = FIDX_OFF + 3 * TR * 4;
  static constexpr int TOTAL = LN_OFF + 256 * 4;
};

struct WsBwdBars {
  uint64_t a_full, a_empty;
};

template <int MODE>
__global__ void __launch_bounds__(WS_THREADS, 1) gated_ws_bwd_kernel(const BwdArgs a) {
  extern __shared__ __align__(1024) uint8_t smem_raw[];
  uint8_t* s_img = smem_raw + WsBwdSmem::IMG_OFF;
  uint8_t* s_t1 = smem_raw + WsBwdSmem::T1_OFF;
  uint8_t* s_t2 = smem_raw + WsBwdSmem::T2_OFF;
  int* s_pidx = reinterpret_cast<int*>(smem_raw + WsBwdSmem::PIDX_OFF);
  int* s_fidx = reinterpret_cast<int*>(smem_raw + WsBwdSmem::FIDX_OFF);
  float* s_ln = reinterpret_cast<float*>(smem_raw + WsBwdSmem::LN_OFF);
  __shared__ __align__(8) WsBwdBars bars;

  const int tid = threadIdx.x, warp = tid >> 5;
  const bool use_ln = a.ln != nullptr;
  const int n_tiles = (a.n_rows + TR - 1) / TR;

  build_image_ws(s_img, s_img + IMG_BYTES, a.w2, 64, 0, tid);
  build_image_ws(s_img + 2 * IMG_BYTES, s_img + 3 * IMG_BYTES, a.w2 + 64 * 64, 64, 0, tid);
  if (tid < 256) s_ln[tid] = use_ln ? a.ln[tid] : 0.f;
  if (tid == 0) {
    tc::mbar_init(&bars.a_full, 256);
    tc::mbar_init(&bars.a_empty, 256);
    tc::mbar_fence_init();
  }
  tc::fence_async_smem();
  __syncthreads();

  if (warp < 8) {
    const int t = tid;
    const int tx = t & 15, ty = t >> 4;
    const int c0 = tx * 4;
    int tl = 0;
    for (int tile = blockIdx.x; tile < n_tiles; tile += gridDim.x, ++tl) {
      const int base = tile * TR;
      if (t < TR) {
        const int r = min(base + t, a.n_rows - 1);
        s_pidx[t] = a.idx0[r];
        s_pidx[TR + t] = a.idx1[r];
        if (MODE == ATOM) s_pidx[2 * TR + t] = a.idx2[r];
      }
      tc::wg_barrier(1, 256);
      {
        const int nt = tile + gridDim.x;
        if (nt < n_tiles) {
          const int r = min(nt * TR + (t & 127), a.n_rows - 1);
          const float* row = a.save_p + (size_t)r * 128 + (t >> 7) * 64;
          prefetch_l2(row);
          prefetch_l2(row + 32);
        }
      }
      float4 g1, g2, b1, b2v;
      if (use_ln) {
        g1 = lds4(s_ln + c0);
        b1 = lds4(s_ln + 64 + c0);
        g2 = lds4(s_ln + 128 + c0);
        b2v = lds4(s_ln + 192 + c0);
      }
      tc::mbar_wait(&bars.a_empty, (tl & 1) ^ 1);
#pragma unroll 2
      for (int pass = 0; pass < 8; ++pass) {
        const int row = pass * 16 + ty;
        const int g = base + row;
        const bool valid = g < a.n_rows;
        const int r = min(g, a.n_rows - 1);
        const float4 pc4 = ldg4(a.save_p + (size_t)r * 128 + c0);
        const float4 pg4 = ldg4(a.save_p + (size_t)r * 128 + 64 + c0);
        float4 gm, wv;
        if (MODE == ATOM) {
          gm = ldg4(a.g_in + (size_t)s_pidx[row] * 64 + c0);
          wv = ldg4(a.wgt + (size_t)s_pidx[2 * TR + row] * 64 + c0);
        } else {
          gm = ldg4(a.g_in + (size_t)s_pidx[row] * 64 + c0);
          wv = ldg4(a.wgt + (size_t)s_pidx[row] * 64 + c0);
        }
        float y1[4] = {pc4.x, pc4.y, pc4.z, pc4.w};
        float y2[4] = {pg4.x, pg4.y, pg4.z, pg4.w};
        float xh1[4], xh2[4], rstd1 = 1.f, rstd2 = 1.f;
        if (use_ln) {
          ln_stats(y1, xh1, rstd1);
          ln_stats(y2, xh2, rstd2);
#pragma unroll
          for (int j = 0; j < 4; ++j) {
            y1[j] = fmaf(xh1[j], f4at(g1, j), f4at(b1, j));
            y2[j] = fmaf(xh2[j], f4at(g2, j), f4at(b2v, j));
          }
        }
        float s1[4], core[4], gate[4];
        float4 o;
#pragma unroll
        for (int j = 0; j < 4; ++j) {
          s1[j] = sigmoid_f(y1[j]);
          core[j] = y1[j] * s1[j];
          gate[j] = sigmoid_f(y2[j]);
          f4at(o, j) = core[j] * gate[j];
        }
        float4 go;
        if (MODE == ATOM) {
          if (valid) stg4(a.g_w0 + (size_t)g * 64 + c0, gm * o);
          go = gm * wv;
        } else {
          const float4 wj = ldg4(a.wgt + (size_t)s_pidx[TR + row] * 64 + c0);
          const float4 gmo = gm * o;
          if (valid) {
            stg4(a.g_w0 + (size_t)g * 64 + c0, gmo * wj);
            stg4(a.g_w1 + (size_t)g * 64 + c0, gmo * wv);
          }
          go = gm * wv * wj;
        }
        float gy1[4], gy2[4];
#pragma unroll
        for (int j = 0; j < 4; ++j) {
          const float gj = f4at(go, j);
          gy1[j] = gj * gate[j] * (s1[j] * fmaf(y1[j], 1.f - s1[j], 1.f));
          gy2[j] = gj * core[j] * gate[j] * (1.f - gate[j]);
        }
        if (use_ln) {
          float gx[4], sa = 0.f, sb = 0.f;
#pragma unroll
          for (int j = 0; j < 4; ++j) {
            gx[j] = gy1[j] * f4at(g1, j);
            sa += gx[j];
            sb = fmaf(gx[j], xh1[j], sb);
          }
          sa = sum16(sa) * (1.f / 64.f);
          sb = sum16(sb) * (1.f / 64.f);
#pragma unroll
          for (int j = 0; j < 4; ++j) gy1[j] = rstd1 * (gx[j] - sa - xh1[j] * sb);
          sa = 0.f, sb = 0.f;
#pragma unroll
          for (int j = 0; j < 4; ++j) {
            gx[j] = gy2[j] * f4at(g2, j);
            sa += gx[j];
            sb = fmaf(gx[j], xh2[j], sb);
          }
          sa = sum16(sa) * (1.f / 64.f);
          sb = sum16(sb) * (1.f / 64.f);
#pragma unroll
          for (int j = 0; j < 4; ++j) gy2[j] = rstd2 * (gx[j] - sa - xh2[j] * sb);
        }
        *reinterpret_cast<float4*>(s_t1 + swz(row, tx)) = make_float4(gy1[0], gy1[1], gy1[2], gy1[3]);
        *reinterpret_cast<float4*>(s_t1 + HALF_BYTES + swz(row, tx)) = make_float4(gy2[0], gy2[1], gy2[2], gy2[3]);
      }
      tc::wg_barrier(1, 256);
      tc::mbar_arrive(&bars.a_full);
    }
  } else {
    const int t = tid - 256;
    const int tx = t & 15, ty = t >> 4;
    const int c0 = tx * 4;
    const int crow = t & 127, chalf = t >> 7;
    const int row0 = ((warp - 8) >> 2) * 64;
    const uint32_t img = tc::smem_u32(s_img);
    int tl = 0;
    for (int tile = blockIdx.x; tile < n_tiles; tile += gridDim.x, ++tl) {
      const int base = tile * TR;
      if (MODE == ATOM && t < TR) {
        const int r = min(base + t, a.n_rows - 1);
        s_fidx[t] = a.idx0[r];
        s_fidx[TR + t] = a.idx1[r];
        s_fidx[2 * TR + t] = a.idx2[r];
      }
      {
        const int r = min(base + crow, a.n_rows - 1);
        const float* row = MODE == ATOM ? a.p_b + (size_t)__ldg(a.idx2 + r) * 128 + chalf * 64 : a.save_pre + (size_t)r * 128 + chalf * 64;
        prefetch_l2(row);
        prefetch_l2(row + 32);
      }
      tc::mbar_wait(&bars.a_full, tl & 1);
#pragma unroll 1
      for (int half = 0; half < 2; ++half) {
        float d[32];
#pragma unroll
        for (int i = 0; i < 32; ++i) d[i] = 0.f;
        const uint8_t* src = s_t1 + half * HALF_BYTES;
        tc::wg_gemm_k64<64>(d, [&](int r, int k) { return *reinterpret_cast<const float*>(src + swz(row0 + r, k >> 2) + (k & 3) * 4); },
                            img + half * 2 * IMG_BYTES, img + (half * 2 + 1) * IMG_BYTES, 2048);
        uint8_t* dst = s_t2 + half * HALF_BYTES;
#pragma unroll
        for (int i = 0; i < 32; i += 2) {
          const int r = row0 + tc::frag_row(i), c = tc::frag_col(i);
          *reinterpret_cast<float2*>(dst + swz(r, c >> 2) + (c & 3) * 4) = make_float2(d[i], d[i + 1]);
        }
      }
      tc::mbar_arrive(&bars.a_empty);
      tc::wg_barrier(2, 256);
#pragma unroll 2
      for (int pass = 0; pass < 8; ++pass) {
        const int row = pass * 16 + ty;
        const int g = base + row;
        float4 vc, vg;
        if (MODE == ATOM) {
          const float* s0 = a.p_a + (size_t)s_fidx[row] * 256 + c0;
          const float* s1 = a.p_a + (size_t)s_fidx[TR + row] * 256 + 128 + c0;
          const float* s2 = a.p_b + (size_t)s_fidx[2 * TR + row] * 128 + c0;
          vc = ldg4(s0) + ldg4(s1) + ldg4(s2);
          vg = ldg4(s0 + 64) + ldg4(s1 + 64) + ldg4(s2 + 64);
        } else {
          const int r = min(g, a.n_rows - 1);
          vc = ldg4(a.save_pre + (size_t)r * 128 + c0);
          vg = ldg4(a.save_pre + (size_t)r * 128 + 64 + c0);
        }
        const float4 hc = *reinterpret_cast<const float4*>(s_t2 + swz(row, tx));
        const float4 hg = *reinterpret_cast<const float4*>(s_t2 + HALF_BYTES + swz(row, tx));
        if (g < a.n_rows) {
          stg4(a.g_pre + (size_t)g * 128 + c0,
               make_float4(hc.x * dsilu_f(vc.x), hc.y * dsilu_f(vc.y), hc.z * dsilu_f(vc.z), hc.w * dsilu_f(vc.w)));
          stg4(a.g_pre + (size_t)g * 128 + 64 + c0,
               make_float4(hg.x * dsilu_f(vg.x), hg.y * dsilu_f(vg.y), hg.z * dsilu_f(vg.z), hg.w * dsilu_f(vg.w)));
        }
      }
      tc::wg_barrier(2, 256);
    }
  }
}

template <int MODE>
int launch_ws_bwd(const BwdArgs& a, cudaStream_t stream) {
  if (a.n_rows == 0) return CHG_OK;
  static bool attr_set = false;
  if (!attr_set) {
    CHG_CUDA(cudaFuncSetAttribute(gated_ws_bwd_kernel<MODE>, cudaFuncAttributeMaxDynamicSharedMemorySize, WsBwdSmem::TOTAL));
    attr_set = true;
  }
  const int n_tiles = (a.n_rows + TR - 1) / TR;
  gated_ws_bwd_kernel<MODE><<<min(n_tiles, sm_count()), WS_THREADS, WsBwdSmem::TOTAL, stream>>>(a);
  CHG_LAUNCH_END();
}

}

int atom_conv_bwd_ws(const BwdArgs& a, cudaStream_t stream) { return launch_ws_bwd<ATOM>(a, stream); }
int bond_conv_bwd_ws(const BwdArgs& a, cudaStream_t stream) { return launch_ws_bwd<BOND>(a, stream); }

}
}
```

chgnet_b200/csrc/native_engine.cu:

```cuda
#include <cstdarg>
#include <cstdio>
#include <cstring>
#include <string>

#include "common.cuh"

namespace chg {
namespace {

constexpr size_t ALIGN = 256;
constexpr int64_t PAD = 16;

struct GatedW {
  const float *w2t = nullptr, *w2 = nullptr, *b2 = nullptr, *ln = nullptr;
  const float *a_t = nullptr, *b_t = nullptr, *c_t = nullptr, *bias1 = nullptr;
  const float *a_b = nullptr, *b_b = nullptr, *c_b = nullptr;
  const float *wo_t = nullptr, *wo = nullptr, *bo = nullptr;
};
struct Weights {
  const float *emb, *freq_ag, *freq_bg, *freq_ang, *w3t, *w3, *wang_t, *wang;
  GatedW atom[CHG_MAX_CONV], bond[CHG_MAX_CONV], angle[CHG_MAX_CONV];
  const float *readout_ln, *mlp_wt, *mlp_w, *mlp_b, *w_last, *w_mag, *atom_ref;
};

// ... 128 lines not shown
  void reset_tmp() { top_used = 0; }
};

struct Ctx {
  Arena ar;
  cudaStream_t stream = nullptr;
  std::string* trace = nullptr;
  int rc = CHG_OK;
  float* f(bool keep, size_t n) { return static_cast<float*>(keep ? ar.keep(n * 4) : ar.tmp(n * 4)); }
  bool go(const char* name) {
    if (trace != nullptr) {
      trace->append(name);
      trace->push_back('\n');
    }
    return !ar.dry && !ar.overflow && rc == CHG_OK;
  }
  void zero(void* p, size_t bytes) {
    if (!ar.dry && !ar.overflow && rc == CHG_OK && bytes > 0 && cudaMemsetAsync(p, 0, bytes, stream) != cudaSuccess) {
      set_error("chg_forward: cudaMemsetAsync failed");
      rc = CHG_ERR_CUDA;
    }
  }
};

#define RUN(c, name, call) \
  do {                     \
    if ((c).go(name)) (c).rc = (call); \
  } while (0)

int run_schedule(const chg_hparams& hp, const Weights& W, const chg_batch& b, const chg_outputs& o, Ctx& c) {
  const int N = b.n_atoms, Ed = b.n_edges, Eu = b.n_bonds, A = b.n_angles, B = b.n_graphs, Es = b.n_short;
  const bool has_ang = A > 0;
  const bool grad = o.force != nullptr || o.virial != nullptr;
  const int n_conv = hp.n_conv;
  void* st = c.stream;
  auto lin = [&](const float* x, const int32_t* xr, int m, int k, const float* wt, const float* bias, const float* res,
                 const int32_t* yr, int n, float* y) { RUN(c, "linear", chg_linear(x, xr, m, k, wt, bias, res, yr, n, y, st)); };
  auto seg = [&](const float* data, int width, const int32_t* perm, const int32_t* ptr, int rows, int items, int acc,
                 float* out, int ld) { RUN(c, "segment_sum", chg_segment_sum(data, width, perm, ptr, rows, items, acc, out, ld, st)); };

  float* x = c.f(true, (size_t)N * 64);
  RUN(c, "embed_atoms", chg_embed_atoms(b.z, W.emb, N, x, st));
  float *rvec = c.f(true, (size_t)Ed * 3), *dist = c.f(true, Ed), *rhat = c.f(true, (size_t)Ed * 3);
  RUN(c, "edge_geometry", chg_edge_geometry(b.frac, b.lattice, b.owner, b.center, b.nbr, b.image, Ed, rvec, dist, rhat, st));
  float *e = c.f(true, (size_t)Eu * 64), *wag = c.f(true, (size_t)Eu * 64), *wbg = c.f(true, (size_t)Eu * 64);
  RUN(c, "bond_basis_embed", chg_bond_basis_embed(dist, b.u2d, Eu, W.freq_ag, W.freq_bg, hp.num_radial, hp.atom_graph_cutoff,
                                                  hp.bond_graph_cutoff, hp.cutoff_coeff, W.w3t, e, wag, wbg, nullptr, st));
  float *ang = nullptr, *ang_alt = nullptr, *wbg_s = nullptr;
  if (has_ang) {
    ang = c.f(true, (size_t)A * 64);
    ang_alt = c.f(true, (size_t)A * 64);
    RUN(c, "angle_basis_embed", chg_angle_basis_embed(rhat, b.ang_di, b.ang_dj, A, W.freq_ang, (hp.num_angular - 1) / 2,
                                                      W.wang_t, ang, nullptr, st));
    wbg_s = c.f(true, (size_t)Es * 64);
    RUN(c, "gather_rows", chg_gather_rows(wbg, b.short_ids, Es, 64, wbg_s, st));
  }
  struct SavedAtom { float *pcn, *pe, *p; } sa[CHG_MAX_CONV];
  struct SavedBond { float *pre, *p; } sb[CHG_MAX_CONV];
  float* sang[CHG_MAX_CONV];

  auto atom_conv = [&](int t, const float* xin, float* xout) {
    const GatedW& g = W.atom[t];
    float* pcn = c.f(grad, (size_t)N * 256);
    float* pe = c.f(grad, (size_t)Eu * 128);
    lin(xin, nullptr, N, 64, g.a_t, nullptr, nullptr, nullptr, 256, pcn);
    lin(e, nullptr, Eu, 64, g.b_t, g.bias1, nullptr, nullptr, 128, pe);
    float* save_p = grad ? c.f(true, (size_t)Ed * 128) : nullptr;
    float* agg = c.f(false, (size_t)N * 64);
    float* work = c.f(false, (size_t)chg_gated_fused_workspace_floats(Ed));
    RUN(c, "atom_conv_fused", chg_atom_conv_fused(pcn, pe, wag, b.center, b.nbr, b.d2u, b.ptr_c, Ed, N, g.w2t, g.b2, g.ln, agg, save_p,
                                                  work, st));
    sa[t] = SavedAtom{pcn, pe, save_p};
    lin(agg, nullptr, N, 64, g.wo_t, g.bo, xin, nullptr, 64, xout);
    c.ar.reset_tmp();
  };

  float* x_mag = nullptr;
  for (int t = 0; t < n_conv - 1; ++t) {
    float* xn = (t == n_conv - 2 && o.atom_fea != nullptr) ? o.atom_fea : c.f(true, (size_t)N * 64);
    atom_conv(t, x, xn);
    x = xn;
    if (has_ang) {
      const GatedW& g = W.bond[t];
      float* pij = c.f(false, (size_t)Es * 256);
      float* px = c.f(false, (size_t)N * 128);
      float* pa = c.f(false, (size_t)A * 128);
      lin(e, b.short_ids, Es, 64, g.a_t, g.bias1, nullptr, nullptr, 256, pij);
      lin(x, nullptr, N, 64, g.b_t, nullptr, nullptr, nullptr, 128, px);
      lin(ang, nullptr, A, 64, g.c_t, nullptr, nullptr, nullptr, 128, pa);
      float* s_pre = grad ? c.f(true, (size_t)A * 128) : nullptr;
      float* s_p = grad ? c.f(true, (size_t)A * 128) : nullptr;
      float* agg = c.f(false, (size_t)Es * 64);
      float* work = c.f(false, (size_t)chg_gated_fused_workspace_floats(A));
      RUN(c, "bond_conv_fused", chg_bond_conv_fused(pij, px, pa, wbg_s, b.ang_atom, b.ang_is, b.ang_js, b.ptr_is, A, Es, g.w2t, g.b2,
                                                    g.ln, agg, s_pre, s_p, work, st));
      lin(agg, nullptr, Es, 64, g.wo_t, g.bo, e, b.short_ids, 64, e);
      sb[t] = SavedBond{s_pre, s_p};
      c.ar.reset_tmp();
      if (t < n_conv - 2) {
        const GatedW& ga = W.angle[t];
        pij = c.f(false, (size_t)Es * 256);
        px = c.f(false, (size_t)N * 128);
        pa = c.f(false, (size_t)A * 128);
        lin(e, b.short_ids, Es, 64, ga.a_t, ga.bias1, nullptr, nullptr, 256, pij);
        lin(x, nullptr, N, 64, ga.b_t, nullptr, nullptr, nullptr, 128, px);
        lin(ang, nullptr, A, 64, ga.c_t, nullptr, nullptr, nullptr, 128, pa);
        float* s_pa = grad ? c.f(true, (size_t)A * 128) : nullptr;
        RUN(c, "angle_update_fwd", chg_angle_update_fwd(pij, px, pa, ang, b.ang_atom, b.ang_is, b.ang_js, A, ga.ln, ang_alt, s_pa, st));
        sang[t] = s_pa;
        float* sw = ang;
        ang = ang_alt;
        ang_alt = sw;
        c.ar.reset_tmp();
      }
    }
    if (t == n_conv - 2) {
      x_mag = x;
      if (o.magmom != nullptr) RUN(c, "magmom", chg_magmom(x, N, W.w_mag, hp.b_mag, o.magmom, st));
    }
  }
  if (n_conv == 1 && o.magmom != nullptr) c.zero(o.magmom, (size_t)N * 4);
  (void)x_mag;
  {
    float* xn = c.f(true, (size_t)N * 64);
    atom_conv(n_conv - 1, x, xn);
    x = xn;
  }

  float* h_out = o.crystal_fea != nullptr ? c.f(false, (size_t)N * 64) : nullptr;
  float* g_x = grad ? c.f(true, (size_t)N * 64) : nullptr;
  c.zero(o.energy, (size_t)B * 8);
  c.zero(o.e_ref, (size_t)B * 8);
  RUN(c, "readout", chg_readout(x, b.z, b.owner, N, W.readout_ln, W.mlp_wt, W.mlp_w, W.mlp_b, hp.n_readout_hidden, W.w_last,
                                hp.b_last, W.atom_ref, o.site_e, h_out, o.energy, o.e_ref, g_x, st));
  if (o.crystal_fea != nullptr) seg(h_out, 64, nullptr, b.graph_ptr, B, N, 0, o.crystal_fea, 64);
  c.ar.reset_tmp();
  if (!grad) return c.rc;

  float* g_e = c.f(true, (size_t)Eu * 64);
  bool g_e_live = false;
  float* g_wag = c.f(true, (size_t)Eu * 64);
  c.zero(g_wag, (size_t)Eu * 256);
  float* g_wbg = has_ang ? c.f(true, (size_t)Es * 64) : nullptr;
  if (has_ang) c.zero(g_wbg, (size_t)Es * 256);
  float* g_a = has_ang ? c.f(true, (size_t)A * 64) : nullptr;
  bool g_a_live = false;

  auto atom_bwd = [&](int t) {
    const GatedW& g = W.atom[t];
    float* g_agg = c.f(false, (size_t)N * 64);
    lin(g_x, nullptr, N, 64, g.wo, nullptr, nullptr, nullptr, 64, g_agg);
    float* g_pre = c.f(false, (size_t)Ed * 128);
    float* g_w = c.f(false, (size_t)Ed * 64);
    RUN(c, "atom_conv_bwd", chg_atom_conv_bwd(sa[t].pcn, sa[t].pe, wag, b.center, b.nbr, b.d2u, Ed, sa[t].p, g_agg, g.w2, g.ln,
                                              g_pre, g_w, nullptr, nullptr, st));
    float* sp = c.f(false, (size_t)N * 256);
    seg(g_pre, 128, nullptr, b.ptr_c, N, Ed, 0, sp, 256);
    seg(g_pre, 128, b.perm_n, b.ptr_n, N, Ed, 0, sp + 128, 256);
    lin(sp, nullptr, N, 256, g.a_b, nullptr, g_x, nullptr, 64, g_x);
    float* spe = c.f(false, (size_t)Eu * 128);
    seg(g_pre, 128, b.perm_u, b.ptr_u, Eu, Ed, 0, spe, 128);
    lin(spe, nullptr, Eu, 128, g.b_b, nullptr, g_e_live ? g_e : nullptr, nullptr, 64, g_e);
    g_e_live = true;
    seg(g_w, 64, b.perm_u, b.ptr_u, Eu, Ed, 1, g_wag, 64);
    c.ar.reset_tmp();
  };
  auto angle_scatter = [&](const float* g_pre, const GatedW& g) {
    float* sp = c.f(false, (size_t)Es * 256);
    seg(g_pre, 128, nullptr, b.ptr_is, Es, A, 0, sp, 256);
    seg(g_pre, 128, b.perm_js, b.ptr_js, Es, A, 0, sp + 128, 256);
    lin(sp, nullptr, Es, 256, g.a_b, nullptr, g_e, b.short_ids, 64, g_e);
    float* spx = c.f(false, (size_t)N * 128);
    seg(g_pre, 128, b.perm_x, b.ptr_x, N, A, 0, spx, 128);
    lin(spx, nullptr, N, 128, g.b_b, nullptr, g_x, nullptr, 64, g_x);
  };

  atom_bwd(n_conv - 1);
  for (int t = n_conv - 2; t >= 0; --t) {
    if (has_ang) {
      if (t < n_conv - 2) {
        const GatedW& ga = W.angle[t];
        float* g_pre = c.f(false, (size_t)A * 128);
        RUN(c, "angle_update_bwd", chg_angle_update_bwd(sang[t], g_a_live ? g_a : nullptr, A, ga.ln, g_pre, nullptr, st));
        lin(g_pre, nullptr, A, 128, ga.c_b, nullptr, g_a_live ? g_a : nullptr, nullptr, 64, g_a);
        g_a_live = true;
        angle_scatter(g_pre, ga);
        c.ar.reset_tmp();
      }
      const GatedW& g = W.bond[t];
      float* g_agg = c.f(false, (size_t)Es * 64);
      lin(g_e, b.short_ids, Es, 64, g.wo, nullptr, nullptr, nullptr, 64, g_agg);
      float* g_pre = c.f(false, (size_t)A * 128);
      float *gw_i = c.f(false, (size_t)A * 64), *gw_j = c.f(false, (size_t)A * 64);
      RUN(c, "bond_conv_bwd", chg_bond_conv_bwd(sb[t].pre, sb[t].p, wbg_s, b.ang_is, b.ang_js, A, g_agg, g.w2, g.ln, g_pre, gw_i,
                                                gw_j, nullptr, nullptr, st));
      lin(g_pre, nullptr, A, 128, g.c_b, nullptr, g_a_live ? g_a : nullptr, nullptr, 64, g_a);
      g_a_live = true;
      angle_scatter(g_pre, g);
      seg(gw_i, 64, nullptr, b.ptr_is, Es, A, 1, g_wbg, 64);
      seg(gw_j, 64, b.perm_js, b.ptr_js, Es, A, 1, g_wbg, 64);
      c.ar.reset_tmp();
    }
    atom_bwd(t);
  }

  float* g_dist = c.f(false, Eu);
  float* g_wbg_full = c.f(false, (size_t)Eu * 64);
  c.zero(g_wbg_full, (size_t)Eu * 256);
  if (has_ang) RUN(c, "scatter_rows", chg_scatter_rows(g_wbg, b.short_ids, Es, 64, g_wbg_full, st));
  RUN(c, "bond_basis_bwd", chg_bond_basis_bwd(dist, b.u2d, Eu, W.freq_ag, W.freq_bg, hp.num_radial, hp.atom_graph_cutoff,
                                              hp.bond_graph_cutoff, hp.cutoff_coeff, W.w3, g_e, g_wag, g_wbg_full, g_dist, nullptr, st));
  double* g_rhat = static_cast<double*>(c.ar.tmp((size_t)Ed * 3 * 8));
  c.zero(g_rhat, (size_t)Ed * 24);
  if (has_ang)
    RUN(c, "angle_basis_bwd", chg_angle_basis_bwd(rhat, b.ang_di, b.ang_dj, A, W.freq_ang, (hp.num_angular - 1) / 2, W.wang, g_a,
                                                  g_rhat, nullptr, st));
  c.zero(o.force, (size_t)N * 24);
  c.zero(o.virial, (size_t)B * 72);
  RUN(c, "force_virial", chg_force_virial(rvec, dist, rhat, g_rhat, g_dist, b.d2u, b.u2d, b.center, b.nbr, b.owner, Ed, o.force,
                                          o.virial, st));
  c.ar.reset_tmp();
  return c.rc;
}

}
}

using namespace chg;

extern "C" int64_t chg_packed_floats(const chg_hparams* hp) {
  if (!hp_ok(hp)) return -1;
  Weights w;
  return walk(*hp, nullptr, w);
}

extern "C" int chg_pack_weights_host(chg_hparams* hp, const chg_state_dict* sd, float* packed) {
  CHG_CHECK_ARG(hp_ok(hp), "bad hyper-parameters");
  CHG_CHECK_ARG(sd != nullptr && packed != nullptr, "null pointer");
  Weights w;
  const int64_t total = walk(*hp, packed, w);
  std::memset(packed, 0, sizeof(float) * total);
  const int R = hp->num_radial, NA = hp->num_angular, F = (NA - 1) / 2, L = hp->n_readout_hidden;
  copy_n(w.emb, sd->atom_embedding, 94 * 64);
  copy_n(w.freq_ag, sd->freq_ag, R);
  copy_n(w.freq_bg, sd->freq_bg, R);
  copy_n(w.freq_ang, sd->freq_ang, F);
  const float* three[3] = {sd->bond_embedding, sd->bond_weights_ag, sd->bond_weights_bg};
  for (int m = 0; m < 3; ++m) {
    copy_n(w.w3 + (size_t)m * 64 * R, three[m], 64 * R);
    for (int o = 0; o < 64; ++o)
      for (int k = 0; k < R; ++k) mut(w.w3t)[((size_t)m * R + k) * 64 + o] = three[m][(size_t)o * R + k];
  }
  copy_n(w.wang, sd->angle_embedding, 64 * NA);
  for (int o = 0; o < 64; ++o)
    for (int k = 0; k < NA; ++k) mut(w.wang_t)[(size_t)k * 64 + o] = sd->angle_embedding[(size_t)o * NA + k];
  for (int t = 0; t < hp->n_conv; ++t) {
    const GatedW& g = w.atom[t];
    const chg_gated_sd& s = sd->atom[t];
    pack_second(g, s);
    pack_ln(g, s);
    put_t(g.a_t, 256, 0, s.core_w1, 192, 0);
    put_t(g.a_t, 256, 64, s.gate_w1, 192, 0);
    put_t(g.a_t, 256, 128, s.core_w1, 192, 128);
    put_t(g.a_t, 256, 192, s.gate_w1, 192, 128);
    put_t(g.b_t, 128, 0, s.core_w1, 192, 64);
    put_t(g.b_t, 128, 64, s.gate_w1, 192, 64);
    copy_n(g.bias1, s.core_b1, 64);
    copy_n(g.bias1 + 64, s.gate_b1, 64);
    put_rows(g.a_b, 0, s.core_w1, 192, 0);
    put_rows(g.a_b, 1, s.gate_w1, 192, 0);
    put_rows(g.a_b, 2, s.core_w1, 192, 128);
    put_rows(g.a_b, 3, s.gate_w1, 192, 128);
    put_rows(g.b_b, 0, s.core_w1, 192, 64);
    put_rows(g.b_b, 1, s.gate_w1, 192, 64);
    pack_out(g, s);
  }
  for (int t = 0; t < hp->n_conv - 1; ++t) {
    for (int kind = 0; kind < 2; ++kind) {
      const GatedW& g = kind == 0 ? w.bond[t] : w.angle[t];
      const chg_gated_sd& s = kind == 0 ? sd->bond[t] : sd->angle[t];
      if (kind == 0) pack_second(g, s);
      pack_ln(g, s);
      put_t(g.a_t, 256, 0, s.core_w1, 256, 0);
      put_t(g.a_t, 256, 64, s.gate_w1, 256, 0);
      put_t(g.a_t, 256, 128, s.core_w1, 256, 64);
      put_t(g.a_t, 256, 192, s.gate_w1, 256, 64);
      copy_n(g.bias1, s.core_b1, 64);
      copy_n(g.bias1 + 64, s.gate_b1, 64);
      put_t(g.b_t, 128, 0, s.core_w1, 256, 192);
      put_t(g.b_t, 128, 64, s.gate_w1, 256, 192);
      put_t(g.c_t, 128, 0, s.core_w1, 256, 128);
      put_t(g.c_t, 128, 64, s.gate_w1, 256, 128);
      put_rows(g.a_b, 0, s.core_w1, 256, 0);
      put_rows(g.a_b, 1, s.gate_w1, 256, 0);
      put_rows(g.a_b, 2, s.core_w1, 256, 64);
      put_rows(g.a_b, 3, s.gate_w1, 256, 64);
      put_rows(g.b_b, 0, s.core_w1, 256, 192);
      put_rows(g.b_b, 1, s.gate_w1, 256, 192);
      put_rows(g.c_b, 0, s.core_w1, 256, 128);
      put_rows(g.c_b, 1, s.gate_w1, 256, 128);
      if (kind == 0) pack_out(g, s);
    }
  }
  if (w.readout_ln != nullptr) {
    copy_n(w.readout_ln, sd->readout_ln_w, 64);
    copy_n(w.readout_ln + 64, sd->readout_ln_b, 64);
  }
  for (int l = 0; l < L; ++l) {
    copy_n(w.mlp_w + (size_t)l * 4096, sd->mlp_w[l], 4096);
    put_t(w.mlp_wt + (size_t)l * 4096, 64, 0, sd->mlp_w[l], 64, 0);
    copy_n(w.mlp_b + (size_t)l * 64, sd->mlp_b[l], 64);
  }
  copy_n(w.w_last, sd->mlp_last_w, 64);
  copy_n(w.w_mag, sd->site_wise_w, 64);
  if (sd->atom_ref != nullptr) copy_n(w.atom_ref, sd->atom_ref, 94);
  hp->b_last = sd->mlp_last_b;
  hp->b_mag = sd->site_wise_b;
  return CHG_OK;
}

static int forward_impl(const chg_hparams* hp, const float* packed, const chg_batch* b, const chg_outputs* o, void* workspace,
                        size_t workspace_bytes, bool dry, std::string* trace, size_t* need, void* stream) {
  CHG_CHECK_ARG(hp_ok(hp), "bad hyper-parameters");
  CHG_CHECK_ARG(b != nullptr && o != nullptr, "null pointer");
  CHG_CHECK_ARG(b->n_atoms >= 0 && b->n_edges >= 0 && b->n_bonds >= 0 && b->n_angles >= 0 && b->n_graphs >= 1 && b->n_short >= 0,
                "negative size");
  Weights w;
  walk(*hp, const_cast<float*>(packed), w);
  Ctx c;
  c.ar.base = static_cast<char*>(workspace);
  c.ar.cap = dry ? (size_t)-1 / 4 : workspace_bytes / ALIGN * ALIGN;
  c.ar.dry = dry;
  c.stream = as_stream(stream);
  c.trace = trace;
  const int rc = run_schedule(*hp, w, *b, *o, c);
  if (need != nullptr) *need = c.ar.peak + ALIGN;
  if (!dry && c.ar.overflow) {
    set_error("chg_forward: workspace too small (%zu bytes given, %zu needed; ask chg_forward_plan)", workspace_bytes,
              c.ar.peak + ALIGN);
    return CHG_ERR_ARG;
  }
  return rc;
}

extern "C" int chg_forward_plan(const chg_hparams* hp, const chg_batch* sizes, const chg_outputs* wanted,
                                size_t* workspace_bytes, char* trace, size_t trace_cap) {
  std::string tr;
  const int rc = forward_impl(hp, nullptr, sizes, wanted, nullptr, 0, true, trace != nullptr ? &tr : nullptr, workspace_bytes, nullptr);
  if (trace != nullptr && trace_cap > 0) {
    const size_t n = tr.size() < trace_cap - 1 ? tr.size() : trace_cap - 1;
    std::memcpy(trace, tr.data(), n);
    trace[n] = 0;
// ... 13 lines not shown
```

chgnet_b200/engine.py:

```python
from __future__ import annotations

from dataclasses import dataclass, field

import torch
from torch import Tensor

from chgnet_b200.batch import DeviceBatch
from chgnet_b200.weights import PackedWeights

EV_A3_TO_GPA = 160.21766208


@dataclass
class EngineOutput:
    energy: Tensor
    e_ref: Tensor
    site_e: Tensor
    magmom: Tensor | None = None
    atom_fea: Tensor | None = None
    crystal_fea: Tensor | None = None
    force: Tensor | None = None
    virial: Tensor | None = None
    extras: dict = field(default_factory=dict)

# ... 331 lines not shown

        def atom_bwd2(t, bar_xout, bar_e):
            gp, sv, la, tt = pw.atom[t], saved_atom[t], rec["atom"][t], t_atom[t]
            if G is not None:
                G[f"atom.{t}.wo_t"] = wsum(sv["agg"], bar_xout, 64, tt["agg_d"], la["g_xout"])
                if gp.extra["bo"] is not None:
                    G[f"atom.{t}.bo"] = self._colsum(b, bar_xout)
            bar_agg = self._lin(b, bar_xout, gp.extra["wo"])
            bar_pre, bar_w, u, g_ln = self._new(b, Ed, 128), self._new(b, Ed, 64), self._new(b, Ed, 128), ln_acc()
            K.atom_conv_bwd2(sv["pre"], sv["p"], tt["pre_d"], tt["p_d"], la["g_p"], wag, wag_d, b.center, b.d2u,
                             la["g_agg"], bar_agg, gp.w2, gp.ln, bar_pre, bar_w, u, g_ln)
            w2_grads(f"atom.{t}", sv["pre"], u, tt["pre_d"], la["g_p"], g_ln)
            sp = self._new(b, N, 256)
            K.segment_sum(bar_pre, None, b.ptr_c, 0, sp[:, :128])
            K.segment_sum(bar_pre, b.perm_n, b.ptr_n, 0, sp[:, 128:])
            spe = self._seg(b, bar_pre, b.perm_u, b.ptr_u, Eu)
            if G is not None:
                G[f"atom.{t}.wcn_t"] = wsum(sv["x"], sp, 256, tt["x_d"], la["sp"])
                we_bar, G[f"atom.{t}.b1"] = self._wgrad(b, sv["e"], spe, 128, colsum=True)
                G[f"atom.{t}.we_t"] = we_bar + self._wgrad(b, tt["e_d"], la["spe"], 128)
            K.segment_sum(bar_w, b.perm_u, b.ptr_u, 1, bar_wag)
            return acc(bar_xout, sp, gp.extra["wcn_b"]), acc(bar_e, spe, gp.extra["we_b"])

        def angle_scatter2(bar_pre, bar_x, bar_e, ex, key, sv, la, tt):
            sp = self._new(b, Es, 256)
            K.segment_sum(bar_pre, None, b.ptr_is, 0, sp[:, :128])
            K.segment_sum(bar_pre, b.perm_js, b.ptr_js, 0, sp[:, 128:])
            if bar_e is None:
                bar_e = self._zeros(b, Eu, 64)
            K.linear(sp, ex["wij_b"], None, bar_e, bar_e, None, sid)
            spx = self._seg(b, bar_pre, b.perm_x, b.ptr_x, N)
            if G is not None:
                G[f"{key}.wij_t"] = wsum(sv["e"], sp, 256, tt["e_d"], la["sp"], x_rows=sid)
                G[f"{key}.wx_t"] = wsum(sv["x"], spx, 128, tt["x_d"], la["spx"])
                w1a_bar, G[f"{key}.b1"] = self._wgrad(b, sv["ang"], bar_pre, 128, colsum=True)
                G[f"{key}.w1a_t"] = w1a_bar + self._wgrad(b, tt["ang_d"], la["g_pre"], 128)
            return acc(bar_x, spx, ex["wx_b"]), bar_e

        bar_x, bar_e = atom_bwd2(n_conv - 1, bar_x, None)
        if train["seed_magmom"] is not None:
            g_lin = self._new(b, N)
            K.magmom_bwd(tr["x_mag"], pw.w_mag, pw.b_mag, train["seed_magmom"].to(dt).contiguous(), bar_x, g_lin)
            G["w_mag"] = self._colsum(b, tr["x_mag"], rowscale=g_lin)
            G["b_mag"] = g_lin.sum()
        for t in reversed(range(n_conv - 1)):
            if has_ang:
                if t < n_conv - 2:
                    ga, sva, la, tt = pw.angle[t], saved_angle[t], rec["angle"][t], t_angle[t]
                    bar_pre, g_ln = self._new(b, A, 128), ln_acc()
                    K.angle_update_bwd2(sva["p"], tt["p_d"], la["g_ang_in"], bar_a, ga.ln, bar_pre, g_ln)
                    if g_ln is not None:
                        G[f"angle.{t}.ln"] = g_ln.to(dt).view(4, 64)
                    bar_a = acc(bar_a, bar_pre, ga.extra["w1a_b"])
                    bar_x, bar_e = angle_scatter2(bar_pre, bar_x, bar_e, ga.extra, f"angle.{t}", sva, la, tt)
                gp, sv, la, tt = pw.bond[t], saved_bond[t], rec["bond"][t], t_bond[t]
                if bar_e is None:
                    bar_e = self._zeros(b, Eu, 64)
                if G is not None:
                    G[f"bond.{t}.wo_t"] = (self._wgrad(b, sv["agg"], bar_e, 64, g_rows=sid)
                                           + self._wgrad(b, tt["agg_d"], la["g_eout"], 64, g_rows=sid))
                    if gp.extra["bo"] is not None:
                        G[f"bond.{t}.bo"] = self._colsum(b, bar_e)
                bar_agg = self._lin(b, bar_e, gp.extra["wo"], x_rows=sid)
                bar_pre, u, g_ln = self._new(b, A, 128), self._new(b, A, 128), ln_acc()
                bw_i, bw_j = self._new(b, A, 64), self._new(b, A, 64)
                K.bond_conv_bwd2(sv["pre"], sv["p"], tt["pre_d"], tt["p_d"], la["g_p"], wbg_s, wbg_s_d, b.ang_is, b.ang_js,
                                 la["g_agg"], bar_agg, gp.w2, gp.ln, bar_pre, bw_i, bw_j, u, g_ln)
                w2_grads(f"bond.{t}", sv["pre"], u, tt["pre_d"], la["g_p"], g_ln)
                bar_a = acc(bar_a, bar_pre, gp.extra["w1a_b"])
                bar_x, bar_e = angle_scatter2(bar_pre, bar_x, bar_e, gp.extra, f"bond.{t}", sv, la, tt)
                K.segment_sum(bw_i, None, b.ptr_is, 1, bar_wbg)
                K.segment_sum(bw_j, b.perm_js, b.ptr_js, 1, bar_wbg)
            bar_x, bar_e = atom_bwd2(t, bar_x, bar_e)

        bar_wbg_full = self._zeros(b, Eu, 64)
        if has_ang:
            K.scatter_rows(bar_wbg, sid, bar_wbg_full)
        if G is None:
            return self._geometry_tail(st, ddist, drhat, bar_e, bar_wag, bar_wbg_full, bar_a, per_graph)

        R, NA = pw.freq_ag.shape[0], pw.wang.shape[1]
        order = torch.argsort(b.z.long(), stable=True).int()
        zptr = torch.zeros(95, dtype=torch.int32, device=b.z.device)
        zptr[1:] = torch.cumsum(torch.bincount(b.z.long() - 1, minlength=94), 0)
        G["emb"] = self._new(b, 94, 64)
        K.segment_sum(bar_x, order, zptr, 0, G["emb"])
        bb = tr["bb"]
        G["w3t"] = torch.stack([wsum(bb, bar_e, 64, tb, rec["g_e0"])[:R], wsum(bb, bar_wag, 64, tb, rec["g_wag"])[:R],
                                wsum(bb, bar_wbg_full, 64, tb, rec["g_wbg_full"])[32 : 32 + R]])
        g_freq = self._zeros(b, 2, R, dtype=torch.float64)
        K.bond_basis_bwd(dist, b.u2d, pw.freq_ag, pw.freq_bg, hp.atom_graph_cutoff, hp.bond_graph_cutoff,
                         hp.cutoff_coeff, pw.w3, bar_e, bar_wag, bar_wbg_full, self._new(b, Eu), g_freq)
        K.bond_basis_bwd2(dist, ddist, b.u2d, pw.freq_ag, pw.freq_bg, hp.atom_graph_cutoff, hp.bond_graph_cutoff,
                          hp.cutoff_coeff, pw.w3, rec["g_e0"], rec["g_wag"], rec["g_wbg_full"], g_freq)
        G["freq_ag"], G["freq_bg"] = g_freq[0].to(dt), g_freq[1].to(dt)
        if has_ang:
            G["wang_t"] = wsum(tr["fb"], bar_a, 64, tfb, rec["g_a0"])[:NA]
            g_fa = self._zeros(b, pw.freq_ang.shape[0], dtype=torch.float64)
            K.angle_basis_bwd(rhat, b.ang_di, b.ang_dj, pw.freq_ang, pw.wang, bar_a, None, g_fa)
            K.angle_basis_bwd2(rhat, drhat, b.ang_di, b.ang_dj, pw.freq_ang, pw.wang, rec["g_a0"], g_fa)
            G["freq_ang"] = g_fa.to(dt)

    def _geometry_tail(self, st, ddist, drhat, bar_e, bar_wag, bar_wbg_full, bar_a,
                       per_graph: bool = False) -> tuple[Tensor, Tensor]:
        pw, K, hp = self.pw, self.K, self.pw.hp
        b: DeviceBatch = st["b"]
        rec, dist, rvec, rhat = st["rec"], st["dist"], st["rvec"], st["rhat"]
        g_dist = self._new(b, b.n_bonds)
        K.bond_basis_bwd(dist, b.u2d, pw.freq_ag, pw.freq_bg, hp.atom_graph_cutoff, hp.bond_graph_cutoff,
                         hp.cutoff_coeff, pw.w3, bar_e, bar_wag, bar_wbg_full, g_dist)
        K.bond_basis_hvp(dist, ddist, b.u2d, pw.freq_ag, pw.freq_bg, hp.atom_graph_cutoff, hp.bond_graph_cutoff,
                         hp.cutoff_coeff, pw.w3, rec["g_e0"], rec["g_wag"], rec["g_wbg_full"], g_dist)
        g_rhat = self._zeros(b, b.n_edges, 3, dtype=torch.float64)
        if b.n_angles > 0:
            K.angle_basis_bwd(rhat, b.ang_di, b.ang_dj, pw.freq_ang, pw.wang, bar_a, g_rhat)
            K.angle_basis_hvp(rhat, drhat, b.ang_di, b.ang_dj, pw.freq_ang, pw.wang, rec["g_a0"], g_rhat)
        neg_hv = self._zeros(b, b.n_atoms, 3, dtype=torch.float64)
        virial = self._zeros(b, b.n_graphs, 9, dtype=torch.float64)
        K.force_virial(rvec, dist, rhat, g_rhat, g_dist, b.d2u, b.u2d, b.center, b.nbr, b.owner, neg_hv, virial)
        if per_graph:
            K.edge_tangent_bwd_virial(rvec, dist, rhat, ddist, drhat, rec["g_dist"], rec["g_rhat"], b.d2u, b.u2d,
                                      b.center, b.nbr, b.owner, neg_hv, virial)
        else:
            K.edge_tangent_bwd(dist, rhat, ddist, drhat, rec["g_dist"], rec["g_rhat"], b.d2u, b.u2d, b.center, b.nbr,
                               neg_hv)
        return neg_hv.neg_(), virial

    def _wgrad(self, b, x, g, n, *, x_rows=None, g_rows=None, x_silu=False, colsum=False):
        out = self._new(b, 64, n)
        cs = self._new(b, n) if colsum else None
        self.K.wgrad(x, g, out, cs, x_rows, g_rows, x_silu)
        return (out, cs) if colsum else out

    def _colsum(self, b, a, bmul=None, rowscale=None) -> Tensor:
        out = self._zeros(b, a.shape[1], dtype=torch.float64)
        self.K.colsum(a, out, bmul, rowscale)
        return out.to(self.pw.emb.dtype)

    def _reverse(self, st: dict, out: EngineOutput, train: dict | None, rec: dict | None = None) -> None:
        pw, K, hp = self.pw, self.K, self.pw.hp
        b: DeviceBatch = st["b"]
        N, Ed, Eu, A, B = b.n_atoms, b.n_edges, b.n_bonds, b.n_angles, b.n_graphs
        has_ang = A > 0
        n_conv = hp.n_conv
        Es, sid = b.n_short, b.short_ids
        wag, wbg_s, dist, rvec, rhat, tr = st["wag"], st["wbg_s"], st["dist"], st["rvec"], st["rhat"], st["tr"]
        saved_atom, saved_bond, saved_angle = st["saved_atom"], st["saved_bond"], st["saved_angle"]
        G = train["grads"] if train is not None else None
        use_ln = pw.atom[0].ln is not None

        def ln_acc():
            return self._zeros(b, 256, dtype=torch.float64) if (G is not None and use_ln) else None

        g_x = st["g_x"]
        if train is not None:
            L = pw.mlp_wt.shape[0]
            seed_atom = train["seed_energy"].to(pw.emb.dtype)[b.owner.long()].contiguous()
            g_x = self._new(b, N, 64)
            h_all, gz_all = self._new(b, L + 1, N, 64), self._new(b, L, N, 64)
            g_h0, xhat = self._new(b, N, 64), self._new(b, N, 64)
            K.readout_bwd(st["x_last"], pw.readout_ln, pw.mlp_wt, pw.mlp_w, pw.mlp_b, pw.w_last, seed_atom, g_x,
                          h_all, gz_all, g_h0, xhat)
            G["mlp_wt"] = torch.stack([self._wgrad(b, h_all[l], gz_all[l], 64) for l in range(L)])
            G["mlp_b"] = torch.stack([self._colsum(b, gz_all[l]) for l in range(L)])
            G["w_last"] = self._colsum(b, h_all[L], rowscale=seed_atom)
            G["b_last"] = seed_atom.sum()
            if pw.readout_ln is not None:
                G["readout_ln"] = torch.stack([self._colsum(b, g_h0, xhat), self._colsum(b, g_h0)])

        g_e = None
        g_wag = self._zeros(b, Eu, 64)
        g_wbg = self._zeros(b, Es, 64) if has_ang else None
        g_a = None

        def acc(dst: Tensor | None, x_in: Tensor, wt: Tensor) -> Tensor:
            return self._lin(b, x_in, wt, residual=dst)

        def w2_grads(key: str, pre: Tensor, g_p: Tensor, g_ln: Tensor | None) -> None:
            w2t, b2 = self._new(b, 64, 128), self._new(b, 128)
            K.wgrad(pre[:, :64], g_p[:, :64], w2t[:, :64], b2[:64], None, None, True)
            K.wgrad(pre[:, 64:], g_p[:, 64:], w2t[:, 64:], b2[64:], None, None, True)
            G[f"{key}.w2t"], G[f"{key}.b2"] = w2t, b2
            if g_ln is not None:
                G[f"{key}.ln"] = g_ln.to(w2t.dtype).view(4, 64)

        def atom_conv_bwd(t: int, g_xout: Tensor, g_e: Tensor | None) -> tuple[Tensor, Tensor]:
            gp, sv = pw.atom[t], saved_atom[t]
            g_agg = self._lin(b, g_xout, gp.extra["wo"])
            g_pre, g_w = self._new(b, Ed, 128), self._new(b, Ed, 64)
            if rec is not None:
                g_p = self._new(b, Ed, 128)
                K.atom_conv_bwd(sv["pcn"], sv["pe"], wag, b.center, b.nbr, b.d2u, sv["p"], g_agg, gp.w2, gp.ln,
                                g_pre, g_w, g_p, None)
                rec["atom"][t] = dict(g_xout=g_xout, g_agg=g_agg, g_p=g_p)
            elif G is None:
                K.atom_conv_bwd(sv["pcn"], sv["pe"], wag, b.center, b.nbr, b.d2u, sv["p"], g_agg, gp.w2, gp.ln,
                                g_pre, g_w)
            else:
                g_p, g_ln = self._new(b, Ed, 128), ln_acc()
                K.atom_conv_bwd(sv["pcn"], sv["pe"], wag, b.center, b.nbr, b.d2u, sv["p"], g_agg, gp.w2, gp.ln,
                                g_pre, g_w, g_p, g_ln)
                w2_grads(f"atom.{t}", sv["pre"], g_p, g_ln)
                G[f"atom.{t}.wo_t"] = self._wgrad(b, sv["agg"], g_xout, 64)
                if gp.extra["bo"] is not None:
                    G[f"atom.{t}.bo"] = self._colsum(b, g_xout)
            sp = self._new(b, N, 256)
            K.segment_sum(g_pre, None, b.ptr_c, 0, sp[:, :128])
            K.segment_sum(g_pre, b.perm_n, b.ptr_n, 0, sp[:, 128:])
            g_xin = acc(g_xout, sp, gp.extra["wcn_b"])
            spe = self._seg(b, g_pre, b.perm_u, b.ptr_u, Eu)
            if rec is not None:
                rec["atom"][t].update(sp=sp, spe=spe)
            if G is not None:
                G[f"atom.{t}.wcn_t"] = self._wgrad(b, sv["x"], sp, 256)
                G[f"atom.{t}.we_t"], G[f"atom.{t}.b1"] = self._wgrad(b, sv["e"], spe, 128, colsum=True)
            g_e = acc(g_e, spe, gp.extra["we_b"])
            K.segment_sum(g_w, b.perm_u, b.ptr_u, 1, g_wag)
            return g_xin, g_e

        def angle_scatter(g_pre: Tensor, g_x: Tensor, g_e: Tensor | None, ex: dict, key: str = "",
                          sv: dict | None = None) -> tuple[Tensor, Tensor]:
            sp = self._new(b, Es, 256)
            K.segment_sum(g_pre, None, b.ptr_is, 0, sp[:, :128])
            K.segment_sum(g_pre, b.perm_js, b.ptr_js, 0, sp[:, 128:])
            K.linear(sp, ex["wij_b"], None, g_e, g_e, None, sid)
            spx = self._seg(b, g_pre, b.perm_x, b.ptr_x, N)
            if rec is not None:
                rec[key.split(".")[0]][int(key.split(".")[1])].update(sp=sp, spx=spx, g_pre=g_pre)
            if G is not None:
                G[f"{key}.wij_t"] = self._wgrad(b, sv["e"], sp, 256, x_rows=sid)
                G[f"{key}.wx_t"] = self._wgrad(b, sv["x"], spx, 128)
                G[f"{key}.w1a_t"], G[f"{key}.b1"] = self._wgrad(b, sv["ang"], g_pre, 128, colsum=True)
            g_x = acc(g_x, spx, ex["wx_b"])
            return g_x, g_e

        g_x, g_e = atom_conv_bwd(n_conv - 1, g_x, None)
        if train is not None and train["seed_magmom"] is not None:
            g_lin = self._new(b, N)
            K.magmom_bwd(tr["x_mag"], pw.w_mag, pw.b_mag, train["seed_magmom"].to(pw.emb.dtype).contiguous(), g_x, g_lin)
            G["w_mag"] = self._colsum(b, tr["x_mag"], rowscale=g_lin)
            G["b_mag"] = g_lin.sum()
        for t in reversed(range(n_conv - 1)):
            if has_ang:
                if t < n_conv - 2:
                    ga = pw.angle[t]
                    g_pre = self._new(b, A, 128)
                    if rec is not None:
                        rec["angle"][t] = dict(g_ang_in=g_a)
                    if G is None:
                        K.angle_update_bwd(saved_angle[t]["p"], g_a, ga.ln, g_pre)
                    else:
                        g_ln = ln_acc()
                        K.angle_update_bwd(saved_angle[t]["p"], g_a, ga.ln, g_pre, g_ln)
                        if g_ln is not None:
                            G[f"angle.{t}.ln"] = g_ln.to(g_pre.dtype).view(4, 64)
                    g_a = acc(g_a, g_pre, ga.extra["w1a_b"])
                    g_x, g_e = angle_scatter(g_pre, g_x, g_e, ga.extra, f"angle.{t}", saved_angle[t])
                gp, sv = pw.bond[t], saved_bond[t]
                g_agg = self._lin(b, g_e, gp.extra["wo"], x_rows=sid)
                g_pre = self._new(b, A, 128)
                gw_i, gw_j = self._new(b, A, 64), self._new(b, A, 64)
                if rec is not None:
                    g_p = self._new(b, A, 128)
                    K.bond_conv_bwd(sv["pre"], sv["p"], wbg_s, b.ang_is, b.ang_js, g_agg, gp.w2, gp.ln, g_pre,
                                    gw_i, gw_j, g_p, None)
                    rec["bond"][t] = dict(g_eout=g_e.clone(), g_agg=g_agg, g_p=g_p)
                elif G is None:
                    K.bond_conv_bwd(sv["pre"], sv["p"], wbg_s, b.ang_is, b.ang_js, g_agg, gp.w2, gp.ln, g_pre,
                                    gw_i, gw_j)
                else:
                    g_p, g_ln = self._new(b, A, 128), ln_acc()
                    K.bond_conv_bwd(sv["pre"], sv["p"], wbg_s, b.ang_is, b.ang_js, g_agg, gp.w2, gp.ln, g_pre,
                                    gw_i, gw_j, g_p, g_ln)
                    w2_grads(f"bond.{t}", sv["pre"], g_p, g_ln)
                    G[f"bond.{t}.wo_t"] = self._wgrad(b, sv["agg"], g_e, 64, g_rows=sid)
                    if gp.extra["bo"] is not None:
                        G[f"bond.{t}.bo"] = self._colsum(b, g_e)
                g_a = acc(g_a, g_pre, gp.extra["w1a_b"])
                g_x, g_e = angle_scatter(g_pre, g_x, g_e, gp.extra, f"bond.{t}", sv)
                K.segment_sum(gw_i, None, b.ptr_is, 1, g_wbg)
                K.segment_sum(gw_j, b.perm_js, b.ptr_js, 1, g_wbg)
            g_x, g_e = atom_conv_bwd(t, g_x, g_e)

        g_dist = self._new(b, Eu)
        g_wbg_full = self._zeros(b, Eu, 64)
        if has_ang:
            K.scatter_rows(g_wbg, sid, g_wbg_full)
        if G is not None:
            R, NA = pw.freq_ag.shape[0], pw.wang.shape[1]
            order = torch.argsort(b.z.long(), stable=True).int()
            zptr = torch.zeros(95, dtype=torch.int32, device=b.z.device)
            zptr[1:] = torch.cumsum(torch.bincount(b.z.long() - 1, minlength=94), 0)
            G["emb"] = self._new(b, 94, 64)
            K.segment_sum(g_x, order, zptr, 0, G["emb"])
            G["w3t"] = torch.stack([self._wgrad(b, tr["bb"], g_e, 64)[:R], self._wgrad(b, tr["bb"], g_wag, 64)[:R],
                                    self._wgrad(b, tr["bb"], g_wbg_full, 64)[32 : 32 + R]])
            g_freq = self._zeros(b, 2, R, dtype=torch.float64)
            K.bond_basis_bwd(dist, b.u2d, pw.freq_ag, pw.freq_bg, hp.atom_graph_cutoff, hp.bond_graph_cutoff,
                             hp.cutoff_coeff, pw.w3, g_e, g_wag, g_wbg_full, g_dist, g_freq)
            G["freq_ag"], G["freq_bg"] = g_freq[0].to(g_e.dtype), g_freq[1].to(g_e.dtype)
            if has_ang:
                G["wang_t"] = self._wgrad(b, tr["fb"], g_a, 64)[:NA]
                g_fa = self._zeros(b, pw.freq_ang.shape[0], dtype=torch.float64)
                K.angle_basis_bwd(rhat, b.ang_di, b.ang_dj, pw.freq_ang, pw.wang, g_a, None, g_fa)
                G["freq_ang"] = g_fa.to(g_e.dtype)
            return
        if rec is not None:
            rec.update(g_e0=g_e, g_wag=g_wag, g_wbg_full=g_wbg_full, g_a0=g_a)
        K.bond_basis_bwd(dist, b.u2d, pw.freq_ag, pw.freq_bg, hp.atom_graph_cutoff, hp.bond_graph_cutoff,
                         hp.cutoff_coeff, pw.w3, g_e, g_wag, g_wbg_full, g_dist)
        g_rhat = self._zeros(b, Ed, 3, dtype=torch.float64)
        if has_ang:
            K.angle_basis_bwd(rhat, b.ang_di, b.ang_dj, pw.freq_ang, pw.wang, g_a, g_rhat)
        if rec is not None:
            rec.update(g_dist=g_dist, g_rhat=g_rhat)
        force = self._zeros(b, N, 3, dtype=torch.float64)
        virial = self._zeros(b, B, 9, dtype=torch.float64)
        K.force_virial(rvec, dist, rhat, g_rhat, g_dist, b.d2u, b.u2d, b.center, b.nbr, b.owner, force, virial)
        out.force, out.virial = force, virial
```

include/chgnet_b200.h:

```cpp
#ifndef CHGNET_B200_H
#define CHGNET_B200_H

#include <stdint.h>

#ifdef __cplusplus
extern "C" {
#endif

#define CHG_FEA 64
#define CHG_MAX_CONV 8
#define CHG_MAX_Z 94
#define CHG_OK 0
#define CHG_ERR_ARG (-1)
#define CHG_ERR_CUDA (-2)

const char* chg_last_error(void);
int chg_abi_version(void);
int64_t chg_launch_count(void);
int chg_set_option(const char* name, int32_t value);

int chg_embed_atoms(const int32_t* z, const float* emb, int32_t n_atoms, float* x, void* stream);

int chg_edge_geometry(const float* frac, const float* lattice, const int32_t* atom_owner,
                      const int32_t* center, const int32_t* nbr, const float* image,
                      int32_t n_edges, float* rvec, float* dist, float* rhat, void* stream);

int chg_bond_basis_embed(const float* dist, const int32_t* u2d, int32_t n_bonds,
                         const float* freq_ag, const float* freq_bg, int32_t n_radial,
                         float rc_ag, float rc_bg, int32_t p, const float* w3t,
                         float* e0, float* wag, float* wbg,
                         float* basis_out ,
                         void* stream);
int chg_bond_basis_bwd(const float* dist, const int32_t* u2d, int32_t n_bonds,
                       const float* freq_ag, const float* freq_bg, int32_t n_radial,
                       float rc_ag, float rc_bg, int32_t p, const float* w3,
                       const float* g_e0, const float* g_wag, const float* g_wbg,
                       float* g_dist,
                       double* g_freq ,
                       void* stream);

int chg_angle_basis_embed(const float* rhat, const int32_t* ang_di, const int32_t* ang_dj,
                          int32_t n_angles, const float* freq, int32_t n_freq,
                          const float* wt, float* a0,
                          float* basis_out ,
                          void* stream);
int chg_angle_basis_bwd(const float* rhat, const int32_t* ang_di, const int32_t* ang_dj,
                        int32_t n_angles, const float* freq, int32_t n_freq,
                        const float* w, const float* g_a0, double* g_rhat ,
                        double* g_freq , void* stream);

int chg_linear(const float* x, const int32_t* x_rows, int32_t m, int32_t k, const float* wt,
               const float* bias, const float* residual, const int32_t* y_rows, int32_t n_out,
               float* y, void* stream);
int chg_gather_rows(const float* src, const int32_t* idx, int32_t n, int32_t width, float* dst,
                    void* stream);
int chg_scatter_rows(const float* src, const int32_t* idx, int32_t n, int32_t width, float* dst,
                     void* stream);

int chg_atom_conv_fwd(const float* pcn, const float* pe, const float* wag,
                      const int32_t* center, const int32_t* nbr, const int32_t* d2u,
                      int32_t n_edges, const float* w2t, const float* b2, const float* ln,
                      float* msg, float* save_p, float* save_pre ,
                      void* stream);
int chg_atom_conv_bwd(const float* pcn, const float* pe, const float* wag,
                      const int32_t* center, const int32_t* nbr, const int32_t* d2u,
                      int32_t n_edges, const float* save_p, const float* g_agg,
                      const float* w2, const float* ln, float* g_pre, float* g_w,
                      float* g_p ,
                      double* g_ln , void* stream);

int chg_segment_sum(const float* data, int32_t width, const int32_t* perm,
                    const int32_t* ptr, int32_t n_rows,
                    int32_t n_items , int32_t accumulate,
                    float* out, int32_t out_ld , void* stream);

int64_t chg_gated_fused_workspace_floats(int32_t n_rows);
int chg_atom_conv_fused(const float* pcn, const float* pe, const float* wag, const int32_t* center,
                        const int32_t* nbr, const int32_t* d2u, const int32_t* ptr_c, int32_t n_edges,
                        int32_t n_atoms, const float* w2t, const float* b2, const float* ln, float* agg,
                        float* save_p, float* work, void* stream);
int chg_bond_conv_fused(const float* pij, const float* px, const float* pa, const float* wbg,
                        const int32_t* ang_atom, const int32_t* ang_i, const int32_t* ang_j,
                        const int32_t* ptr_i, int32_t n_angles, int32_t n_slots, const float* w2t,
                        const float* b2, const float* ln, float* agg, float* save_pre, float* save_p,
                        float* work, void* stream);

int chg_bond_conv_fwd(const float* pij, const float* px, const float* pa, const float* wbg,
                      const int32_t* ang_atom, const int32_t* ang_i, const int32_t* ang_j,
                      int32_t n_angles, const float* w2t, const float* b2, const float* ln,
                      float* upd, float* save_pre, float* save_p, void* stream);
int chg_bond_conv_bwd(const float* save_pre, const float* save_p, const float* wbg,
                      const int32_t* ang_i, const int32_t* ang_j, int32_t n_angles,
                      const float* g_agg, const float* w2, const float* ln, float* g_pre,
                      float* gw_i, float* gw_j, float* g_p ,
                      double* g_ln , void* stream);

int chg_angle_update_fwd(const float* pij, const float* px, const float* pa, const float* ang,
                         const int32_t* ang_atom, const int32_t* ang_i, const int32_t* ang_j,
                         int32_t n_angles, const float* ln, float* ang_new, float* save_p,
                         void* stream);
int chg_angle_update_bwd(const float* save_p, const float* g_ang_in, int32_t n_angles,
                         const float* ln, float* g_pre, double* g_ln ,
                         void* stream);

int chg_readout(const float* x, const int32_t* z, const int32_t* atom_owner, int32_t n_atoms,
                const float* ln, const float* mlp_wt, const float* mlp_w, const float* mlp_b,
                int32_t n_hidden, const float* w_last, float b_last, const float* atom_ref,
                float* site_e, float* h_out, double* e_graph, double* e_ref, float* g_x,
                void* stream);
int chg_magmom(const float* x, int32_t n_atoms, const float* w, float b, float* m, void* stream);

int chg_force_virial(const float* rvec, const float* dist, const float* rhat,
                     const double* g_rhat, const float* g_dist, const int32_t* d2u,
                     const int32_t* u2d, const int32_t* center, const int32_t* nbr,
                     const int32_t* atom_owner, int32_t n_edges, double* force,
                     double* virial, void* stream);

typedef struct {
  int32_t num_radial;
  int32_t num_angular;
  int32_t n_conv;
  int32_t cutoff_coeff;
  int32_t n_readout_hidden;
  int32_t use_ln;
  int32_t readout_ln;
  int32_t has_mlp_out_bias;
  float atom_graph_cutoff;
  float bond_graph_cutoff;
  float b_last;
  float b_mag;
} chg_hparams;

typedef struct {
  const float* core_w1; const float* core_b1; const float* gate_w1; const float* gate_b1;
  const float* core_w2; const float* core_b2; const float* gate_w2; const float* gate_b2;
  const float* ln1_w; const float* ln1_b; const float* ln2_w; const float* ln2_b;
  const float* out_w; const float* out_b;
} chg_gated_sd;
typedef struct {
  const float* atom_embedding;
  const float* freq_ag; const float* freq_bg; const float* freq_ang;
  const float* bond_embedding; const float* bond_weights_ag; const float* bond_weights_bg;
  const float* angle_embedding;
  chg_gated_sd atom[CHG_MAX_CONV];
  chg_gated_sd bond[CHG_MAX_CONV];
  chg_gated_sd angle[CHG_MAX_CONV];
  const float* readout_ln_w; const float* readout_ln_b;
  const float* mlp_w[4]; const float* mlp_b[4];
  const float* mlp_last_w; float mlp_last_b;
  const float* site_wise_w; float site_wise_b;
  const float* atom_ref;
} chg_state_dict;
int64_t chg_packed_floats(const chg_hparams* hp);
int chg_pack_weights_host(chg_hparams* hp, const chg_state_dict* sd, float* packed_host);

typedef struct {
  int32_t n_atoms, n_edges, n_bonds, n_angles, n_graphs, n_short;
  const int32_t* z; const float* frac; const int32_t* owner; const float* lattice;
  const int32_t* center; const int32_t* nbr; const float* image;
  const int32_t* d2u; const int32_t* u2d;
  const int32_t* ptr_c; const int32_t* perm_n; const int32_t* ptr_n; const int32_t* perm_u; const int32_t* ptr_u;
  const int32_t* ang_atom; const int32_t* ang_di; const int32_t* ang_dj; const int32_t* ang_is; const int32_t* ang_js;
  const int32_t* ptr_is; const int32_t* perm_js; const int32_t* ptr_js; const int32_t* perm_x; const int32_t* ptr_x;
  const int32_t* short_ids;
  const int32_t* graph_ptr;
} chg_batch;
typedef struct {
  double* energy; double* e_ref; float* site_e;
  float* magmom; float* atom_fea; float* crystal_fea;
  double* force; double* virial;
} chg_outputs;
int chg_forward_plan(const chg_hparams* hp, const chg_batch* sizes, const chg_outputs* wanted,
                     size_t* workspace_bytes, char* trace, size_t trace_cap);
int chg_forward(const chg_hparams* hp, const float* packed_weights, const chg_batch* batch,
                const chg_outputs* out, void* workspace , size_t workspace_bytes,
                void* stream);

typedef struct chg_graph chg_graph;
int chg_graph_build(const double* frac, const double* lattice, int32_t n_atoms, double r_atom, double r_bond,
                    chg_graph** out);
void chg_graph_sizes(const chg_graph* g, int64_t* n_edges, int64_t* n_bonds, int64_t* n_angles);
int chg_graph_export(const chg_graph* g, int32_t* atom_graph, float* image, int32_t* d2u, int32_t* u2d,
                     int32_t* bond_graph);
void chg_graph_free(chg_graph* g);

int chg_graph_build_many(int32_t n, const double* const* frac, const double* const* lattice, const int32_t* n_atoms,
                         double r_atom, double r_bond, chg_graph** out);
int chg_graph_views(int32_t n, chg_graph* const* graphs, int64_t* counts, uint64_t* ptrs, int32_t* n_isolated);
void chg_graph_free_many(int32_t n, chg_graph** graphs);

int64_t chg_graph_device_scratch_bytes(int32_t n_atoms, int32_t cap_edges);
int chg_graph_build_device(const double* frac, const double* lattice, int32_t n_atoms, double r_atom, double r_bond,
                           int32_t cap_edges, int32_t cap_angles, int32_t* center, int32_t* nbr, float* image,
                           int32_t* d2u, int32_t* u2d, int32_t* ptr_c, int32_t* ang_atom, int32_t* ang_i,
                           int32_t* ang_di, int32_t* ang_j, int32_t* ang_dj, void* scratch, int32_t* sizes_out,
                           void* stream);

int chg_md_kick_drift(double* x, double* v, const double* f, const double* inv_mass, int32_t n_atoms, double dt,
                      const double* inv_lattice, double* frac64, float* frac32, const double* x_ref,
                      double* max_disp2, void* stream);
int chg_md_kick(double* v, const double* f, const double* inv_mass, int32_t n_atoms, double dt, double* e_kin,
                void* stream);
int chg_fire_step(double* x, double* v, const double* f, int32_t n_atoms, double* state, const double* inv_lattice,
                  double* frac64, float* frac32, double dt_max, double max_step, void* stream);

typedef struct chg_csr_in {
  int32_t n_atoms, n_edges, n_bonds, n_angles, n_short, with_reverse;
  const int32_t *center, *nbr, *d2u, *ang_atom, *ang_i, *ang_j;
} chg_csr_in;
typedef struct chg_csr_out {
  int32_t *ptr_c, *perm_n, *ptr_n, *perm_u, *ptr_u, *ptr_i, *perm_j, *ptr_j, *perm_x, *ptr_x;
  int32_t *short_ids, *ang_is, *ang_js, *ptr_is, *ptr_js;
} chg_csr_out;
int64_t chg_build_csr_scratch_ints(int32_t n_atoms, int32_t n_edges, int32_t n_bonds, int32_t n_angles);
int chg_build_csr(const chg_csr_in* in, const chg_csr_out* out, int32_t* scratch, void* stream);
int chg_bond_graph_count(const int32_t* ang_i, const int32_t* ang_j, int32_t n_angles, int32_t n_bonds,
                         int32_t* scratch, int32_t* count_out, void* stream);

int chg_pack_batch_host(int32_t n_graphs, const int64_t* counts, const void* const* ptrs, int32_t* ibuf,
                        float* fbuf, int32_t* flags_out);

int chg_host_alloc(int64_t bytes, int32_t write_combined, void** out);
int chg_host_free(void* p);

int chg_pack_batch_wire(int32_t n_graphs, const int64_t* counts, const void* const* ptrs, int32_t* ibuf_host,
                        float* fbuf_host, int8_t* img_host, int32_t* ibuf_dev, float* fbuf_dev, int8_t* img_dev,
                        int32_t* flags_out, void* stream);


int64_t chg_wgrad_workspace_floats(int32_t n_out);
int chg_wgrad(const float* x, const float* x2 ,
              int32_t ldx, const int32_t* x_rows, int32_t x_silu, const float* g,
              int32_t ldg, const int32_t* g_rows, int32_t m, int32_t n_out, float* out, int32_t ldo,
              float* colsum, float* workspace, void* stream);
int chg_colsum(const float* a, int32_t lda, const float* bmul, int32_t ldb, const float* rowscale,
               int32_t m, int32_t n, double* out, void* stream);
int chg_readout_bwd(const float* x, int32_t n_atoms, const float* ln, const float* mlp_wt,
                    const float* mlp_w, const float* mlp_b, int32_t n_hidden, const float* w_last,
                    const float* seed, float* g_x, float* h_all, float* gz_all, float* g_h0,
                    float* xhat, void* stream);
int chg_magmom_bwd(const float* x, int32_t n_atoms, const float* w, float b, const float* g_m,
                   float* g_x, float* g_lin, void* stream);
int chg_loss_terms(const float* pred, const float* target, int32_t n, int32_t kind, float delta,
                   float* g_pred, double* sums, void* stream);
int chg_adam_step(float* p, const float* g, float* m, float* v, int64_t n, float lr, float beta1,
                  float beta2, float eps, float weight_decay, int32_t step, void* stream);

int chg_edge_tangent(const float* rvec, const float* dist, const float* rhat, const int32_t* center,
                     const int32_t* nbr, const int32_t* atom_owner, const float* u_atom ,
                     const float* w_graph , int32_t n_edges, float* ddist, float* drhat,
                     void* stream);
int chg_bond_basis_tangent(const float* dist, const float* ddist, const int32_t* u2d, int32_t n_bonds,
                           const float* freq_ag, const float* freq_bg, int32_t n_radial, float rc_ag,
                           float rc_bg, int32_t p, const float* w3t, float* e0d, float* wagd, float* wbgd,
                           float* tbasis, void* stream);
int chg_bond_basis_bwd2(const float* dist, const float* ddist, const int32_t* u2d, int32_t n_bonds,
// ... 64 lines not shown
```

Baseline: 10950.

## Fuse sorted-index segment sums into gated backward kernels' epilogues

Adds fused backward entry points for atom conv, bond conv and angle update that reduce g_pre (and gw_i for bond) into per-segment sums inside the kernel epilogue. They exploit that the first index array is sorted, writing partial sums at strip boundaries to a workspace. A small stitch kernel then combines those partials. This removes separate segment_sum launches and the re-read of the g_pre and gw_i buffers, and for bond conv it skips materializing gw_i. The cost is extra per-strip work and shared-memory traffic, plus a row-to-thread mapping change (contiguous strips of 8 rows) in the warp-specialized kernel that may alter its memory access pattern.

```diff
diff --git a/chgnet_b200/_lib.py b/chgnet_b200/_lib.py
--- a/chgnet_b200/_lib.py
+++ b/chgnet_b200/_lib.py
@@ -31,6 +31,9 @@
     "chg_bond_conv_bwd": [P, P, P, P, P, I, P, P, P, P, P, P, P, P, P],
     "chg_angle_update_fwd": [P, P, P, P, P, P, P, I, P, P, P, P],
     "chg_angle_update_bwd": [P, P, I, P, P, P, P],
+    "chg_atom_conv_bwd_fused": [P, P, P, P, P, P, P, I, I, P, P, P, P, P, P, P, I, P, P],
+    "chg_bond_conv_bwd_fused": [P, P, P, P, P, P, I, I, P, P, P, P, P, P, I, P, P, P],
+    "chg_angle_update_bwd_fused": [P, P, P, P, I, I, P, P, P, I, P, P],
     "chg_readout": [P, P, P, I, P, P, P, P, I, P, F, P, P, P, P, P, P, P],
     "chg_magmom": [P, I, P, F, P, P],
     "chg_force_virial": [P, P, P, P, P, P, P, P, P, P, I, P, P, P],
@@ -245,6 +248,31 @@
         self._call("chg_angle_update_bwd", _p(save_p), _p(g_ang_in), save_p.shape[0], _p(ln), _p(g_pre), _p(g_ln))
 
     @staticmethod
+    def _chk_sp(sp):
+        if not sp.is_cuda or sp.stride(1) != 1:
+            raise ChgnetB200Error("the segment-sum output must be a CUDA tensor with unit column stride")
+
+    def atom_conv_bwd_fused(self, pcn, pe, wag, center, nbr, d2u, ptr_c, save_p, g_agg, w2, ln, g_pre, g_w, sp):
+        self._chk(pcn, pe, wag, center, nbr, d2u, ptr_c, save_p, g_agg, w2, ln, g_pre, g_w)
+        self._chk_sp(sp)
+        self._call("chg_atom_conv_bwd_fused", _p(pcn), _p(pe), _p(wag), _p(center), _p(nbr), _p(d2u), _p(ptr_c),
+                   center.shape[0], sp.shape[0], _p(save_p), _p(g_agg), _p(w2), _p(ln), _p(g_pre), _p(g_w), _p(sp),
+                   sp.stride(0), _p(self._fused_work(center.shape[0], sp.device)))
+
+    def bond_conv_bwd_fused(self, save_pre, save_p, wbg, ang_i, ang_j, ptr_i, g_agg, w2, ln, g_pre, gw_j, sp, g_wbg):
+        self._chk(save_pre, save_p, wbg, ang_i, ang_j, ptr_i, g_agg, w2, ln, g_pre, gw_j, g_wbg)
+        self._chk_sp(sp)
+        self._call("chg_bond_conv_bwd_fused", _p(save_pre), _p(save_p), _p(wbg), _p(ang_i), _p(ang_j), _p(ptr_i),
+                   ang_i.shape[0], sp.shape[0], _p(g_agg), _p(w2), _p(ln), _p(g_pre), _p(gw_j), _p(sp), sp.stride(0),
+                   _p(g_wbg), _p(self._fused_work(ang_i.shape[0], sp.device)))
+
+    def angle_update_bwd_fused(self, save_p, g_ang_in, ang_i, ptr_i, ln, g_pre, sp):
+        self._chk(save_p, g_ang_in, ang_i, ptr_i, ln, g_pre)
+        self._chk_sp(sp)
+        self._call("chg_angle_update_bwd_fused", _p(save_p), _p(g_ang_in), _p(ang_i), _p(ptr_i), save_p.shape[0],
+                   sp.shape[0], _p(ln), _p(g_pre), _p(sp), sp.stride(0), _p(self._fused_work(save_p.shape[0], sp.device)))
+
+    @staticmethod
     def _chk_rows(*tensors: Tensor | None) -> None:
         for t in tensors:
             if t is not None and (not t.is_cuda or t.stride(-1) != 1):
diff --git a/chgnet_b200/csrc/gated.cu b/chgnet_b200/csrc/gated.cu
--- a/chgnet_b200/csrc/gated.cu
+++ b/chgnet_b200/csrc/gated.cu
@@ -159,17 +159,21 @@
 #pragma unroll
   for (int j = 0; j < 16; ++j) ln_acc[j] = 0.f;
 
+  const bool fuse = MODE == ANGLE && a.sum_pre.out != nullptr;
   const int n_tiles = (a.n_rows + TM - 1) / TM;
   for (int tile = blockIdx.x; tile < n_tiles; tile += gridDim.x) {
     const int base = tile * TM;
     __syncthreads();
-    if (MODE != ANGLE && tid < TM) {
+    if ((MODE != ANGLE || fuse) && tid < TM) {
       const int r = min(base + tid, a.n_rows - 1);
       s_idx[tid] = a.idx0[r];
-      s_idx[TM + tid] = a.idx1[r];
+      if (MODE != ANGLE) s_idx[TM + tid] = a.idx1[r];
       if (MODE == ATOM) s_idx[2 * TM + tid] = a.idx2[r];
     }
     __syncthreads();
+    const int strip_lo = base + r0, strip_hi = min(strip_lo + 4, a.n_rows);
+    StripSum<2> ss;
+    if (fuse && strip_lo < a.n_rows) ss.begin(a.idx0, strip_lo, strip_hi, a.n_rows, c0);
 
     float4 g1, g2, b1, b2v;
     if (use_ln) {
@@ -278,8 +282,13 @@
       } else if (valid) {
         stg4(a.g_pre + (size_t)g * 128 + c0, gpc);
         stg4(a.g_pre + (size_t)g * 128 + 64 + c0, gpg);
-      }
-    }
+        if (fuse) {
+          const float4 v[2] = {gpc, gpg};
+          ss.add(a.sum_pre, strip_lo / 4, s_idx[row], v);
+        }
+      }
+    }
+    if (fuse && strip_lo < a.n_rows) ss.flush(a.sum_pre, strip_lo / 4, true);
 
     if (L::HAS_W2) {
       __syncthreads();
@@ -795,3 +804,23 @@
             nullptr, ln, g_pre, nullptr, nullptr, nullptr, g_ln};
   return launch_bwd<ANGLE>(a, as_stream(stream));
 }
+
+extern "C" int chg_angle_update_bwd_fused(const float* save_p, const float* g_ang_in, const int32_t* ang_i,
+                                          const int32_t* ptr_i, int32_t n_angles, int32_t n_slots, const float* ln,
+                                          float* g_pre, float* sp, int32_t ld_sp, float* work, void* stream) {
+  CHG_CHECK_ARG(n_angles >= 0 && n_slots >= 0 && ld_sp >= 128, "bad size");
+  if (n_slots == 0) return CHG_OK;
+  CHG_CHECK_ARG(ptr_i && sp && work, "null pointer");
+  if (gated_impl() == 3 && n_angles >= ws_min_rows()) {
+    CHG_CHECK_ARG(save_p && ang_i && g_pre, "null pointer");
+    BwdArgs a{nullptr, nullptr, nullptr, ang_i, nullptr, nullptr, n_angles, nullptr, save_p, g_ang_in,
+              nullptr, ln, g_pre, nullptr, nullptr, nullptr, nullptr};
+    a.sum_pre = {sp, ld_sp, work, false};
+    const int rc = launch_bwd<ANGLE>(a, as_stream(stream));
+    if (rc != CHG_OK) return rc;
+    return seg_stitch(ptr_i, n_slots, 4, 128, work, sp, ld_sp, false, as_stream(stream));
+  }
+  const int rc = chg_angle_update_bwd(save_p, g_ang_in, n_angles, ln, g_pre, nullptr, stream);
+  if (rc != CHG_OK) return rc;
+  return chg_segment_sum(g_pre, 128, nullptr, ptr_i, n_slots, n_angles, 0, sp, ld_sp, stream);
+}
diff --git a/chgnet_b200/csrc/gated_common.cuh b/chgnet_b200/csrc/gated_common.cuh
--- a/chgnet_b200/csrc/gated_common.cuh
+++ b/chgnet_b200/csrc/gated_common.cuh
@@ -28,6 +28,13 @@
   float* out;
   float* save_pre;
   float* save_p;
+};
+
+struct SegSumOut {
+  float* out = nullptr;
+  int32_t ld = 0;
+  float* parts = nullptr;
+  bool acc = false;
 };
 
 struct BwdArgs {
@@ -48,6 +55,7 @@
   float* g_w1;
   float* g_p;
   double* g_ln;
+  SegSumOut sum_pre, sum_w;
 };
 
 __device__ __forceinline__ void ln_stats(const float (&v)[4], float (&xhat)[4], float& rstd) {
@@ -128,6 +136,50 @@
 }
 
 
+__device__ __forceinline__ size_t part_slot(int strip, int slot) { return (size_t)strip * 2 + slot - 1; }
+
+template <int NV>
+struct StripSum {
+  float4 s[NV];
+  int id;
+  bool first;
+  const int32_t* idx0;
+  int lo, hi, n_rows, c0;
+
+  __device__ __forceinline__ void begin(const int32_t* idx0_, int lo_, int hi_, int n_rows_, int c0_) {
+    idx0 = idx0_;
+    lo = lo_;
+    hi = hi_;
+    n_rows = n_rows_;
+    c0 = c0_;
+    id = -1;
+    first = true;
+  }
+  __device__ __forceinline__ void flush(const SegSumOut& o, int strip, bool last) {
+    const bool before = first && lo > 0 && __ldg(idx0 + lo - 1) == id;
+    const bool after = last && hi < n_rows && __ldg(idx0 + hi) == id;
+    const int width = 64 * NV;
+    float* dst = before || after ? o.parts + part_slot(strip, before ? 0 : 1) * width : o.out + (size_t)id * o.ld;
+    const bool add = o.acc && !before && !after;
+#pragma unroll
+    for (int v = 0; v < NV; ++v) {
+      float4* p = reinterpret_cast<float4*>(dst + 64 * v + c0);
+      *p = add ? *p + s[v] : s[v];
+    }
+    first = false;
+  }
+  __device__ __forceinline__ void add(const SegSumOut& o, int strip, int row_id, const float4 (&v)[NV]) {
+    if (row_id != id) {
+      if (id >= 0) flush(o, strip, false);
+      id = row_id;
+#pragma unroll
+      for (int k = 0; k < NV; ++k) s[k] = make_float4(0.f, 0.f, 0.f, 0.f);
+    }
+#pragma unroll
+    for (int k = 0; k < NV; ++k) s[k] = s[k] + v[k];
+  }
+};
+
 template <typename KernelT>
 inline int resident_ctas(KernelT kernel, int smem_bytes) {
   int per_sm = 0;
@@ -145,6 +197,9 @@
 
 int atom_conv_bwd_ws(const BwdArgs& a, cudaStream_t stream);
 int bond_conv_bwd_ws(const BwdArgs& a, cudaStream_t stream);
+
+int seg_stitch(const int32_t* ptr, int n_seg, int strip, int width, const float* parts, float* out, int ld, bool acc,
+               cudaStream_t stream);
 
 int atom_conv_fused_ws(const float* pcn, const float* pe, const float* wag, const int32_t* center, const int32_t* nbr,
                        const int32_t* d2u, const int32_t* ptr_c, int n_edges, int n_atoms, const float* w2t, const float* b2,
diff --git a/chgnet_b200/csrc/gated_ws.cu b/chgnet_b200/csrc/gated_ws.cu
--- a/chgnet_b200/csrc/gated_ws.cu
+++ b/chgnet_b200/csrc/gated_ws.cu
@@ -3,6 +3,7 @@
 
 namespace chg {
 namespace gated {
+constexpr int BWD_STRIP = 8;
 namespace {
 
 constexpr int WS_THREADS = 512;
@@ -247,7 +248,7 @@
           if (sa >= strip_lo && sb <= strip_hi) {
             dst = a.out + (size_t)seg * 64;
           } else {
-            dst = a.parts + ((size_t)(strip_lo / STRIP) * 2 + (sa < strip_lo ? 0 : 1)) * 64;
+            dst = a.parts + part_slot(strip_lo / STRIP, sa < strip_lo ? 0 : 1) * 64;
           }
           *reinterpret_cast<float2*>(dst + lane * 2) = v;
         };
@@ -272,21 +273,23 @@
   }
 }
 
-__global__ void seg_stitch_kernel(const int32_t* __restrict__ ptr, int n_seg, const float* __restrict__ parts,
-                                  float* __restrict__ out) {
+__global__ void seg_stitch_kernel(const int32_t* __restrict__ ptr, int n_seg, int strip, int width,
+                                  const float* __restrict__ parts, float* __restrict__ out, int ld, int acc) {
+  const int q = width >> 2;
   const int idx = blockIdx.x * blockDim.x + threadIdx.x;
-  const int s = idx >> 4, l = idx & 15;
+  const int s = idx / q, c = (idx - s * q) * 4;
   if (s >= n_seg) return;
   const int a = ptr[s], b = ptr[s + 1];
+  float* dst = out + (size_t)s * ld + c;
   if (a >= b) {
-    stg4(out + (size_t)s * 64 + l * 4, make_float4(0.f, 0.f, 0.f, 0.f));
+    if (!acc) stg4(dst, make_float4(0.f, 0.f, 0.f, 0.f));
     return;
   }
-  const int k0 = a / STRIP, k1 = (b - 1) / STRIP;
+  const int k0 = a / strip, k1 = (b - 1) / strip;
   if (k0 == k1) return;
-  float4 acc = ldg4(parts + ((size_t)k0 * 2 + 1) * 64 + l * 4);
-  for (int k = k0 + 1; k <= k1; ++k) acc = acc + ldg4(parts + ((size_t)k * 2) * 64 + l * 4);
-  stg4(out + (size_t)s * 64 + l * 4, acc);
+  float4 sum = ldg4(parts + part_slot(k0, 1) * width + c);
+  for (int k = k0 + 1; k <= k1; ++k) sum = sum + ldg4(parts + part_slot(k, 0) * width + c);
+  stg4(dst, acc ? *reinterpret_cast<const float4*>(dst) + sum : sum);
 }
 
 template <int MODE>
@@ -307,10 +310,17 @@
     }
     count_launch();
   }
-  seg_stitch_kernel<<<(a.n_seg * 16 + 255) / 256, 256, 0, stream>>>(a.ptr, a.n_seg, a.parts, a.out);
+  return seg_stitch(a.ptr, a.n_seg, STRIP, 64, a.parts, a.out, 64, false, stream);
+}
+
+}
+
+int seg_stitch(const int32_t* ptr, int n_seg, int strip, int width, const float* parts, float* out, int ld, bool acc,
+               cudaStream_t stream) {
+  if (n_seg == 0) return CHG_OK;
+  const int64_t threads = (int64_t)n_seg * (width / 4);
+  seg_stitch_kernel<<<(unsigned)((threads + 255) / 256), 256, 0, stream>>>(ptr, n_seg, strip, width, parts, out, ld, acc);
   CHG_LAUNCH_END();
-}
-
 }
 
 int atom_conv_fused_ws(const float* pcn, const float* pe, const float* wag, const int32_t* center, const int32_t* nbr,
@@ -420,6 +430,7 @@
     const int t = tid;
     const int tx = t & 15, ty = t >> 4;
     const int c0 = tx * 4;
+    const bool fuse_w = MODE == BOND && a.sum_w.out != nullptr;
     int tl = 0;
     for (int tile = blockIdx.x; tile < n_tiles; tile += gridDim.x, ++tl) {
       const int base = tile * TR;
@@ -446,10 +457,13 @@
         g2 = lds4(s_ln + 128 + c0);
         b2v = lds4(s_ln + 192 + c0);
       }
+      const int strip_lo = base + ty * BWD_STRIP, strip_hi = min(strip_lo + BWD_STRIP, a.n_rows);
+      StripSum<1> ssw;
+      if (fuse_w && strip_lo < a.n_rows) ssw.begin(a.idx0, strip_lo, strip_hi, a.n_rows, c0);
       tc::mbar_wait(&bars.a_empty, (tl & 1) ^ 1);
 #pragma unroll 2
-      for (int pass = 0; pass < 8; ++pass) {
-        const int row = pass * 16 + ty;
+      for (int pass = 0; pass < BWD_STRIP; ++pass) {
+        const int row = ty * BWD_STRIP + pass;
         const int g = base + row;
         const bool valid = g < a.n_rows;
         const int r = min(g, a.n_rows - 1);
@@ -492,7 +506,9 @@
           const float4 wj = ldg4(a.wgt + (size_t)s_pidx[TR + row] * 64 + c0);
           const float4 gmo = gm * o;
           if (valid) {
-            stg4(a.g_w0 + (size_t)g * 64 + c0, gmo * wj);
+            const float4 gwi[1] = {gmo * wj};
+            if (fuse_w) ssw.add(a.sum_w, strip_lo / BWD_STRIP, s_pidx[row], gwi);
+            else stg4(a.g_w0 + (size_t)g * 64 + c0, gwi[0]);
             stg4(a.g_w1 + (size_t)g * 64 + c0, gmo * wv);
           }
           go = gm * wv * wj;
@@ -531,6 +547,7 @@
         *reinterpret_cast<float4*>(s_t1 + swz(row, tx)) = make_float4(gy1[0], gy1[1], gy1[2], gy1[3]);
         *reinterpret_cast<float4*>(s_t1 + HALF_BYTES + swz(row, tx)) = make_float4(gy2[0], gy2[1], gy2[2], gy2[3]);
       }
+      if (fuse_w && strip_lo < a.n_rows) ssw.flush(a.sum_w, strip_lo / BWD_STRIP, true);
       tc::wg_barrier(1, 256);
       tc::mbar_arrive(&bars.a_full);
     }
@@ -539,16 +556,19 @@
     const int tx = t & 15, ty = t >> 4;
     const int c0 = tx * 4;
     const int crow = t & 127, chalf = t >> 7;
+    const bool fuse = a.sum_pre.out != nullptr;
     const int row0 = ((warp - 8) >> 2) * 64;
     const uint32_t img = tc::smem_u32(s_img);
     int tl = 0;
     for (int tile = blockIdx.x; tile < n_tiles; tile += gridDim.x, ++tl) {
       const int base = tile * TR;
-      if (MODE == ATOM && t < TR) {
+      if ((MODE == ATOM || fuse) && t < TR) {
         const int r = min(base + t, a.n_rows - 1);
         s_fidx[t] = a.idx0[r];
-        s_fidx[TR + t] = a.idx1[r];
-        s_fidx[2 * TR + t] = a.idx2[r];
+        if (MODE == ATOM) {
+          s_fidx[TR + t] = a.idx1[r];
+          s_fidx[2 * TR + t] = a.idx2[r];
+        }
       }
       {
         const int r = min(base + crow, a.n_rows - 1);
@@ -575,8 +595,8 @@
       tc::mbar_arrive(&bars.a_empty);
       tc::wg_barrier(2, 256);
 #pragma unroll 2
-      for (int pass = 0; pass < 8; ++pass) {
-        const int row = pass * 16 + ty;
+      for (int pass = 0; pass < BWD_STRIP; ++pass) {
+        const int row = ty * BWD_STRIP + pass;
         const int g = base + row;
         float4 vc, vg;
         if (MODE == ATOM) {
@@ -593,11 +613,27 @@
         const float4 hc = *reinterpret_cast<const float4*>(s_t2 + swz(row, tx));
         const float4 hg = *reinterpret_cast<const float4*>(s_t2 + HALF_BYTES + swz(row, tx));
         if (g < a.n_rows) {
-          stg4(a.g_pre + (size_t)g * 128 + c0,
-               make_float4(hc.x * dsilu_f(vc.x), hc.y * dsilu_f(vc.y), hc.z * dsilu_f(vc.z), hc.w * dsilu_f(vc.w)));
-          stg4(a.g_pre + (size_t)g * 128 + 64 + c0,
-               make_float4(hg.x * dsilu_f(vg.x), hg.y * dsilu_f(vg.y), hg.z * dsilu_f(vg.z), hg.w * dsilu_f(vg.w)));
-        }
+          const float4 v[2] = {
+              make_float4(hc.x * dsilu_f(vc.x), hc.y * dsilu_f(vc.y), hc.z * dsilu_f(vc.z), hc.w * dsilu_f(vc.w)),
+              make_float4(hg.x * dsilu_f(vg.x), hg.y * dsilu_f(vg.y), hg.z * dsilu_f(vg.z), hg.w * dsilu_f(vg.w))};
+          stg4(a.g_pre + (size_t)g * 128 + c0, v[0]);
+          stg4(a.g_pre + (size_t)g * 128 + 64 + c0, v[1]);
+          if (fuse) {
+            *reinterpret_cast<float4*>(s_t2 + swz(row, tx)) = v[0];
+            *reinterpret_cast<float4*>(s_t2 + HALF_BYTES + swz(row, tx)) = v[1];
+          }
+        }
+      }
+      const int strip_lo = base + ty * BWD_STRIP, strip_hi = min(strip_lo + BWD_STRIP, a.n_rows);
+      if (fuse && strip_lo < a.n_rows) {
+        StripSum<2> ss;
+        ss.begin(a.idx0, strip_lo, strip_hi, a.n_rows, c0);
+        for (int row = ty * BWD_STRIP; row < strip_hi - base; ++row) {
+          const float4 v[2] = {*reinterpret_cast<const float4*>(s_t2 + swz(row, tx)),
+                               *reinterpret_cast<const float4*>(s_t2 + HALF_BYTES + swz(row, tx))};
+          ss.add(a.sum_pre, strip_lo / BWD_STRIP, s_fidx[row], v);
+        }
+        ss.flush(a.sum_pre, strip_lo / BWD_STRIP, true);
       }
       tc::wg_barrier(2, 256);
     }
@@ -624,3 +660,52 @@
 
 }
 }
+
+extern "C" int chg_atom_conv_bwd_fused(const float* pcn, const float* pe, const float* wag, const int32_t* center,
+                                       const int32_t* nbr, const int32_t* d2u, const int32_t* ptr_c, int32_t n_edges,
+                                       int32_t n_atoms, const float* save_p, const float* g_agg, const float* w2,
+                                       const float* ln, float* g_pre, float* g_w, float* sp, int32_t ld_sp, float* work,
+                                       void* stream) {
+  CHG_CHECK_ARG(n_edges >= 0 && n_atoms >= 0 && ld_sp >= 128, "bad size");
+  if (n_atoms == 0) return CHG_OK;
+  CHG_CHECK_ARG(ptr_c && sp && work, "null pointer");
+  if (gated_impl() == 3 && n_edges >= ws_min_rows()) {
+    CHG_CHECK_ARG(pcn && pe && wag && center && nbr && d2u && save_p && g_agg && w2 && g_pre && g_w, "null pointer");
+    gated::BwdArgs a{pcn, pe, wag, center, nbr, d2u, n_edges, nullptr, save_p, g_agg, w2, ln, g_pre, g_w, nullptr, nullptr, nullptr};
+    a.sum_pre = {sp, ld_sp, work, false};
+    const int rc = gated::atom_conv_bwd_ws(a, as_stream(stream));
+    if (rc != CHG_OK) return rc;
+    return gated::seg_stitch(ptr_c, n_atoms, gated::BWD_STRIP, 128, work, sp, ld_sp, false, as_stream(stream));
+  }
+  const int rc = chg_atom_conv_bwd(pcn, pe, wag, center, nbr, d2u, n_edges, save_p, g_agg, w2, ln, g_pre, g_w, nullptr,
+                                   nullptr, stream);
+  if (rc != CHG_OK) return rc;
+  return chg_segment_sum(g_pre, 128, nullptr, ptr_c, n_atoms, n_edges, 0, sp, ld_sp, stream);
+}
+
+extern "C" int chg_bond_conv_bwd_fused(const float* save_pre, const float* save_p, const float* wbg, const int32_t* ang_i,
+                                       const int32_t* ang_j, const int32_t* ptr_i, int32_t n_angles, int32_t n_slots,
+                                       const float* g_agg, const float* w2, const float* ln, float* g_pre, float* gw_j,
+                                       float* sp, int32_t ld_sp, float* g_wbg, float* work, void* stream) {
+  CHG_CHECK_ARG(n_angles >= 0 && n_slots >= 0 && ld_sp >= 128, "bad size");
+  if (n_slots == 0) return CHG_OK;
+  CHG_CHECK_ARG(ptr_i && sp && g_wbg && work, "null pointer");
+  if (gated_impl() == 3 && n_angles >= ws_min_rows()) {
+    CHG_CHECK_ARG(save_pre && save_p && wbg && ang_i && ang_j && g_agg && w2 && g_pre && gw_j, "null pointer");
+    const int64_t n_strips = ((int64_t)n_angles + gated::BWD_STRIP - 1) / gated::BWD_STRIP;
+    float* parts_w = work + (n_strips > 0 ? 2 * n_strips - 2 : 0) * 128;
+    gated::BwdArgs a{nullptr, nullptr, wbg, ang_i, ang_j, nullptr, n_angles, save_pre, save_p, g_agg, w2, ln,
+                     g_pre, nullptr, gw_j, nullptr, nullptr};
+    a.sum_pre = {sp, ld_sp, work, false};
+    a.sum_w = {g_wbg, 64, parts_w, true};
+    int rc = gated::bond_conv_bwd_ws(a, as_stream(stream));
+    if (rc == CHG_OK) rc = gated::seg_stitch(ptr_i, n_slots, gated::BWD_STRIP, 128, work, sp, ld_sp, false, as_stream(stream));
+    if (rc == CHG_OK) rc = gated::seg_stitch(ptr_i, n_slots, gated::BWD_STRIP, 64, parts_w, g_wbg, 64, true, as_stream(stream));
+    return rc;
+  }
+  int rc = chg_bond_conv_bwd(save_pre, save_p, wbg, ang_i, ang_j, n_angles, g_agg, w2, ln, g_pre, work, gw_j, nullptr,
+                             nullptr, stream);
+  if (rc == CHG_OK) rc = chg_segment_sum(g_pre, 128, nullptr, ptr_i, n_slots, n_angles, 0, sp, ld_sp, stream);
+  if (rc == CHG_OK) rc = chg_segment_sum(work, 64, nullptr, ptr_i, n_slots, n_angles, 1, g_wbg, 64, stream);
+  return rc;
+}
diff --git a/chgnet_b200/csrc/native_engine.cu b/chgnet_b200/csrc/native_engine.cu
--- a/chgnet_b200/csrc/native_engine.cu
+++ b/chgnet_b200/csrc/native_engine.cu
@@ -304,10 +304,10 @@
     lin(g_x, nullptr, N, 64, g.wo, nullptr, nullptr, nullptr, 64, g_agg);
     float* g_pre = c.f(false, (size_t)Ed * 128);
     float* g_w = c.f(false, (size_t)Ed * 64);
-    RUN(c, "atom_conv_bwd", chg_atom_conv_bwd(sa[t].pcn, sa[t].pe, wag, b.center, b.nbr, b.d2u, Ed, sa[t].p, g_agg, g.w2, g.ln,
-                                              g_pre, g_w, nullptr, nullptr, st));
     float* sp = c.f(false, (size_t)N * 256);
-    seg(g_pre, 128, nullptr, b.ptr_c, N, Ed, 0, sp, 256);
+    float* work = c.f(false, (size_t)chg_gated_fused_workspace_floats(Ed));
+    RUN(c, "atom_conv_bwd\nsegment_sum", chg_atom_conv_bwd_fused(sa[t].pcn, sa[t].pe, wag, b.center, b.nbr, b.d2u, b.ptr_c, Ed, N, sa[t].p,
+                                                          g_agg, g.w2, g.ln, g_pre, g_w, sp, 256, work, st));
     seg(g_pre, 128, b.perm_n, b.ptr_n, N, Ed, 0, sp + 128, 256);
     lin(sp, nullptr, N, 256, g.a_b, nullptr, g_x, nullptr, 64, g_x);
     float* spe = c.f(false, (size_t)Eu * 128);
@@ -317,9 +317,7 @@
     seg(g_w, 64, b.perm_u, b.ptr_u, Eu, Ed, 1, g_wag, 64);
     c.ar.reset_tmp();
   };
-  auto angle_scatter = [&](const float* g_pre, const GatedW& g) {
-    float* sp = c.f(false, (size_t)Es * 256);
-    seg(g_pre, 128, nullptr, b.ptr_is, Es, A, 0, sp, 256);
+  auto angle_scatter = [&](const float* g_pre, float* sp, const GatedW& g) {
     seg(g_pre, 128, b.perm_js, b.ptr_js, Es, A, 0, sp + 128, 256);
     lin(sp, nullptr, Es, 256, g.a_b, nullptr, g_e, b.short_ids, 64, g_e);
     float* spx = c.f(false, (size_t)N * 128);
@@ -333,23 +331,27 @@
       if (t < n_conv - 2) {
         const GatedW& ga = W.angle[t];
         float* g_pre = c.f(false, (size_t)A * 128);
-        RUN(c, "angle_update_bwd", chg_angle_update_bwd(sang[t], g_a_live ? g_a : nullptr, A, ga.ln, g_pre, nullptr, st));
+        float* sp = c.f(false, (size_t)Es * 256);
+        float* work = c.f(false, (size_t)chg_gated_fused_workspace_floats(A));
+        RUN(c, "angle_update_bwd\nsegment_sum", chg_angle_update_bwd_fused(sang[t], g_a_live ? g_a : nullptr, b.ang_is, b.ptr_is, A, Es, ga.ln,
+                                                                    g_pre, sp, 256, work, st));
         lin(g_pre, nullptr, A, 128, ga.c_b, nullptr, g_a_live ? g_a : nullptr, nullptr, 64, g_a);
         g_a_live = true;
-        angle_scatter(g_pre, ga);
+        angle_scatter(g_pre, sp, ga);
         c.ar.reset_tmp();
       }
       const GatedW& g = W.bond[t];
       float* g_agg = c.f(false, (size_t)Es * 64);
       lin(g_e, b.short_ids, Es, 64, g.wo, nullptr, nullptr, nullptr, 64, g_agg);
       float* g_pre = c.f(false, (size_t)A * 128);
-      float *gw_i = c.f(false, (size_t)A * 64), *gw_j = c.f(false, (size_t)A * 64);
-      RUN(c, "bond_conv_bwd", chg_bond_conv_bwd(sb[t].pre, sb[t].p, wbg_s, b.ang_is, b.ang_js, A, g_agg, g.w2, g.ln, g_pre, gw_i,
-                                                gw_j, nullptr, nullptr, st));
+      float* gw_j = c.f(false, (size_t)A * 64);
+      float* sp = c.f(false, (size_t)Es * 256);
+      float* work = c.f(false, (size_t)chg_gated_fused_workspace_floats(A));
+      RUN(c, "bond_conv_bwd\nsegment_sum\nsegment_sum", chg_bond_conv_bwd_fused(sb[t].pre, sb[t].p, wbg_s, b.ang_is, b.ang_js, b.ptr_is, A, Es, g_agg, g.w2,
+                                                            g.ln, g_pre, gw_j, sp, 256, g_wbg, work, st));
       lin(g_pre, nullptr, A, 128, g.c_b, nullptr, g_a_live ? g_a : nullptr, nullptr, 64, g_a);
       g_a_live = true;
-      angle_scatter(g_pre, g);
-      seg(gw_i, 64, nullptr, b.ptr_is, Es, A, 1, g_wbg, 64);
+      angle_scatter(g_pre, sp, g);
       seg(gw_j, 64, b.perm_js, b.ptr_js, Es, A, 1, g_wbg, 64);
       c.ar.reset_tmp();
     }
diff --git a/chgnet_b200/engine.py b/chgnet_b200/engine.py
--- a/chgnet_b200/engine.py
+++ b/chgnet_b200/engine.py
@@ -507,6 +507,9 @@
         def ln_acc():
             return self._zeros(b, 256, dtype=torch.float64) if (G is not None and use_ln) else None
 
+        fuse_sums = rec is None and G is None
+        one_call = fuse_sums and hasattr(K, "atom_conv_bwd_fused")
+
         g_x = st["g_x"]
         if train is not None:
             L = pw.mlp_wt.shape[0]
@@ -543,12 +546,16 @@
             gp, sv = pw.atom[t], saved_atom[t]
             g_agg = self._lin(b, g_xout, gp.extra["wo"])
             g_pre, g_w = self._new(b, Ed, 128), self._new(b, Ed, 64)
+            sp = self._new(b, N, 256)
             if rec is not None:
                 g_p = self._new(b, Ed, 128)
                 K.atom_conv_bwd(sv["pcn"], sv["pe"], wag, b.center, b.nbr, b.d2u, sv["p"], g_agg, gp.w2, gp.ln,
                                 g_pre, g_w, g_p, None)
                 rec["atom"][t] = dict(g_xout=g_xout, g_agg=g_agg, g_p=g_p)
-            elif G is None:
+            elif one_call:
+                K.atom_conv_bwd_fused(sv["pcn"], sv["pe"], wag, b.center, b.nbr, b.d2u, b.ptr_c, sv["p"], g_agg, gp.w2,
+                                      gp.ln, g_pre, g_w, sp[:, :128])
+            elif fuse_sums:
                 K.atom_conv_bwd(sv["pcn"], sv["pe"], wag, b.center, b.nbr, b.d2u, sv["p"], g_agg, gp.w2, gp.ln,
                                 g_pre, g_w)
             else:
@@ -559,8 +566,8 @@
                 G[f"atom.{t}.wo_t"] = self._wgrad(b, sv["agg"], g_xout, 64)
                 if gp.extra["bo"] is not None:
                     G[f"atom.{t}.bo"] = self._colsum(b, g_xout)
-            sp = self._new(b, N, 256)
-            K.segment_sum(g_pre, None, b.ptr_c, 0, sp[:, :128])
+            if not one_call:
+                K.segment_sum(g_pre, None, b.ptr_c, 0, sp[:, :128])
             K.segment_sum(g_pre, b.perm_n, b.ptr_n, 0, sp[:, 128:])
             g_xin = acc(g_xout, sp, gp.extra["wcn_b"])
             spe = self._seg(b, g_pre, b.perm_u, b.ptr_u, Eu)
@@ -574,9 +581,10 @@
             return g_xin, g_e
 
         def angle_scatter(g_pre: Tensor, g_x: Tensor, g_e: Tensor | None, ex: dict, key: str = "",
-                          sv: dict | None = None) -> tuple[Tensor, Tensor]:
-            sp = self._new(b, Es, 256)
-            K.segment_sum(g_pre, None, b.ptr_is, 0, sp[:, :128])
+                          sv: dict | None = None, sp: Tensor | None = None) -> tuple[Tensor, Tensor]:
+            if sp is None:
+                sp = self._new(b, Es, 256)
+                K.segment_sum(g_pre, None, b.ptr_is, 0, sp[:, :128])
             K.segment_sum(g_pre, b.perm_js, b.ptr_js, 0, sp[:, 128:])
             K.linear(sp, ex["wij_b"], None, g_e, g_e, None, sid)
             spx = self._seg(b, g_pre, b.perm_x, b.ptr_x, N)
@@ -600,29 +608,45 @@
                 if t < n_conv - 2:
                     ga = pw.angle[t]
                     g_pre = self._new(b, A, 128)
+                    sp = None
                     if rec is not None:
                         rec["angle"][t] = dict(g_ang_in=g_a)
-                    if G is None:
                         K.angle_update_bwd(saved_angle[t]["p"], g_a, ga.ln, g_pre)
+                    elif one_call:
+                        sp = self._new(b, Es, 256)
+                        K.angle_update_bwd_fused(saved_angle[t]["p"], g_a, b.ang_is, b.ptr_is, ga.ln, g_pre, sp[:, :128])
+                    elif fuse_sums:
+                        sp = self._new(b, Es, 256)
+                        K.angle_update_bwd(saved_angle[t]["p"], g_a, ga.ln, g_pre)
+                        K.segment_sum(g_pre, None, b.ptr_is, 0, sp[:, :128])
                     else:
                         g_ln = ln_acc()
                         K.angle_update_bwd(saved_angle[t]["p"], g_a, ga.ln, g_pre, g_ln)
                         if g_ln is not None:
                             G[f"angle.{t}.ln"] = g_ln.to(g_pre.dtype).view(4, 64)
                     g_a = acc(g_a, g_pre, ga.extra["w1a_b"])
-                    g_x, g_e = angle_scatter(g_pre, g_x, g_e, ga.extra, f"angle.{t}", saved_angle[t])
+                    g_x, g_e = angle_scatter(g_pre, g_x, g_e, ga.extra, f"angle.{t}", saved_angle[t], sp)
                 gp, sv = pw.bond[t], saved_bond[t]
                 g_agg = self._lin(b, g_e, gp.extra["wo"], x_rows=sid)
                 g_pre = self._new(b, A, 128)
-                gw_i, gw_j = self._new(b, A, 64), self._new(b, A, 64)
+                gw_j = self._new(b, A, 64)
+                gw_i = None if one_call else self._new(b, A, 64)
+                sp = None
                 if rec is not None:
                     g_p = self._new(b, A, 128)
                     K.bond_conv_bwd(sv["pre"], sv["p"], wbg_s, b.ang_is, b.ang_js, g_agg, gp.w2, gp.ln, g_pre,
                                     gw_i, gw_j, g_p, None)
                     rec["bond"][t] = dict(g_eout=g_e.clone(), g_agg=g_agg, g_p=g_p)
-                elif G is None:
+                elif one_call:
+                    sp = self._new(b, Es, 256)
+                    K.bond_conv_bwd_fused(sv["pre"], sv["p"], wbg_s, b.ang_is, b.ang_js, b.ptr_is, g_agg, gp.w2, gp.ln,
+                                          g_pre, gw_j, sp[:, :128], g_wbg)
+                elif fuse_sums:
+                    sp = self._new(b, Es, 256)
                     K.bond_conv_bwd(sv["pre"], sv["p"], wbg_s, b.ang_is, b.ang_js, g_agg, gp.w2, gp.ln, g_pre,
                                     gw_i, gw_j)
+                    K.segment_sum(g_pre, None, b.ptr_is, 0, sp[:, :128])
+                    K.segment_sum(gw_i, None, b.ptr_is, 1, g_wbg)
                 else:
                     g_p, g_ln = self._new(b, A, 128), ln_acc()
                     K.bond_conv_bwd(sv["pre"], sv["p"], wbg_s, b.ang_is, b.ang_js, g_agg, gp.w2, gp.ln, g_pre,
@@ -632,8 +656,9 @@
                     if gp.extra["bo"] is not None:
                         G[f"bond.{t}.bo"] = self._colsum(b, g_e)
                 g_a = acc(g_a, g_pre, gp.extra["w1a_b"])
-                g_x, g_e = angle_scatter(g_pre, g_x, g_e, gp.extra, f"bond.{t}", sv)
-                K.segment_sum(gw_i, None, b.ptr_is, 1, g_wbg)
+                g_x, g_e = angle_scatter(g_pre, g_x, g_e, gp.extra, f"bond.{t}", sv, sp)
+                if sp is None:
+                    K.segment_sum(gw_i, None, b.ptr_is, 1, g_wbg)
                 K.segment_sum(gw_j, b.perm_js, b.ptr_js, 1, g_wbg)
             g_x, g_e = atom_conv_bwd(t, g_x, g_e)
 
diff --git a/include/chgnet_b200.h b/include/chgnet_b200.h
--- a/include/chgnet_b200.h
+++ b/include/chgnet_b200.h
@@ -102,6 +102,19 @@
 int chg_angle_update_bwd(const float* save_p, const float* g_ang_in, int32_t n_angles,
                          const float* ln, float* g_pre, double* g_ln ,
                          void* stream);
+
+int chg_atom_conv_bwd_fused(const float* pcn, const float* pe, const float* wag, const int32_t* center,
+                            const int32_t* nbr, const int32_t* d2u, const int32_t* ptr_c, int32_t n_edges,
+                            int32_t n_atoms, const float* save_p, const float* g_agg, const float* w2,
+                            const float* ln, float* g_pre, float* g_w, float* sp, int32_t ld_sp, float* work,
+                            void* stream);
+int chg_bond_conv_bwd_fused(const float* save_pre, const float* save_p, const float* wbg, const int32_t* ang_i,
+                            const int32_t* ang_j, const int32_t* ptr_i, int32_t n_angles, int32_t n_slots,
+                            const float* g_agg, const float* w2, const float* ln, float* g_pre, float* gw_j,
+                            float* sp, int32_t ld_sp, float* g_wbg, float* work, void* stream);
+int chg_angle_update_bwd_fused(const float* save_p, const float* g_ang_in, const int32_t* ang_i,
+                               const int32_t* ptr_i, int32_t n_angles, int32_t n_slots, const float* ln,
+                               float* g_pre, float* sp, int32_t ld_sp, float* work, void* stream);
 
 int chg_readout(const float* x, const int32_t* z, const int32_t* atom_owner, int32_t n_atoms,
                 const float* ln, const float* mlp_wt, const float* mlp_w, const float* mlp_b,
```

Result: faster. 11300, median of 6 (+3.2%).
